# IrisRainbowNeko/HCP-Diffusion

Hardware: AMD Instinct MI355X
Metric: training images/sec (whole node), SD1.5 LoRA 512px bs=4/GPU (higher is better)
Workload: dtype bf16; 1 GPU; SD1.5 UNet LoRA rank=8 bf16, bs=4/GPU, 512x512 (64x64 latents), 77-token context, random-init weights, cached latents, grad-ckpt off; global_batch=4, parallelism=dp1, rccl_ranks=1, comm=none, hip_graph=True, gradient_checkpointing=False

## Files before the change

hcp_diffusion_amd/_lib.py:

```python
import ctypes
import os
from ctypes import c_int, c_long, c_float, c_void_p, c_size_t, c_char_p
from pathlib import Path

LIB_PATH = Path(__file__).resolve().parent / "libhcp_mi355x.so"

P, I, L, F = c_void_p, c_int, c_long, c_float

_PROTOTYPES = {
    "hcp_last_error": (c_char_p, []),
    "hcp_is_emulated": (I, []),
    "hcp_abi_version": (I, []),
    "hcp_selfcheck_atomics": (I, [P, P, I, I, I, P]),
    "hcp_gemm_bf16": (I, [P, I, P, I, P, I, I, I, I, P, I, P, I, I, P, P, I, I, P, I, P, P, P, F, I, P, c_size_t, P]),
    "hcp_gemm_lora_bf16": (I, [P, I, P, I, P, P, P, I, P, I, I, I, I, P, P, I, P, P, P, P, c_size_t, P]),
    "hcp_gemm_geglu_bwd_bf16": (I, [P, I, P, I, P, P, P, I, P, P, I, I, I, P, c_size_t, P]),
    "hcp_gemm_workspace_bytes": (c_size_t, [I, I]),
    "hcp_conv3x3_bf16": (I, [P, I, P, I, I, I, I, I, I, I, I, I, I, P, I, P, I, P, P, I, P, I, I, P, P, P, c_size_t, P]),
    "hcp_attention_fwd": (I, [P, P, P, P, P, I, I, I, I, I, L, I, L, I, L, I, L, I, F, P, L, I, P]),
    "hcp_attention_bwd": (I, [P, P, P, P, P, P, P, P, P, P, I, I, I, I, I, L, I, L, I, L, I, L, I, F, P, L, I, P, c_size_t, P]),
    "hcp_groupnorm_workspace_bytes": (c_size_t, [I, I, I, I]),
    "hcp_groupnorm_silu_fwd": (I, [P, P, P, P, P, P, I, I, I, I, F, I, P]),
    "hcp_groupnorm_silu_bwd": (I, [P, P, P, P, P, P, P, P, I, I, I, I, I, P]),
    "hcp_layernorm_fwd": (I, [P, P, P, P, P, P, I, I, F, P]),
    "hcp_layernorm_bwd": (I, [P, P, P, P, P, P, P, P, P, I, I, P]),
    "hcp_geglu_fwd": (I, [P, P, L, I, P]),
    "hcp_geglu_bwd": (I, [P, P, P, L, I, P]),
    "hcp_add_bf16": (I, [P, P, P, L, P]),
    "hcp_copy2d_bf16": (I, [P, I, P, I, L, I, P]),
    "hcp_concat2_bf16": (I, [P, I, P, I, P, L, I, P]),
    "hcp_silu_fwd": (I, [P, P, L, P]),
    "hcp_silu_bwd": (I, [P, P, P, L, P]),
    "hcp_nchw_to_nhwc_bf16": (I, [P, I, P, I, I, I, I, P]),
    "hcp_nhwc_to_nchw_f32": (I, [P, P, I, I, I, I, P]),
    "hcp_upsample2x_bwd": (I, [P, P, I, I, I, I, P]),
    "hcp_timestep_embedding": (I, [P, P, I, I, F, P]),
    "hcp_timestep_embedding_f32": (I, [P, P, I, I, F, P]),
    "hcp_wgrad_linear_bf16": (I, [P, I, P, I, P, I, I, I, I, P, c_size_t, P]),
    "hcp_wgrad_conv3x3_bf16": (I, [P, I, P, I, P, I, P, I, I, I, I, I, I, I, I, I, P, c_size_t, P]),
    "hcp_colsum_bf16": (I, [P, I, P, I, I, I, I, P]),
    "hcp_ema_update": (I, [P, P, L, P, F, F, F, P]),
    "hcp_cast_f32_bf16": (I, [P, P, L, F, I, P]),
    "hcp_cast_bf16_f32": (I, [P, P, L, P]),
    "hcp_pack_piece_bytes": (I, []),
    "hcp_pack_weights": (I, [P, I, I, P]),
    "hcp_groupnorm_affine_grad": (I, [P, P, P, P, P, P, P, I, I, I, I, I, P]),
    "hcp_layernorm_affine_grad": (I, [P, P, P, P, P, I, I, P]),
    "hcp_add_noise": (I, [P, P, P, P, P, I, L, P]),
    "hcp_cfg_ddim_step": (I, [P, P, P, L, I, F, F, F, P]),
    "hcp_snr_loss_weight": (I, [P, P, P, I, I, F, P]),
    "hcp_quick_gelu": (I, [P, P, P, L, P]),
    "hcp_embedding_bf16": (I, [P, P, P, P, P, L, I, I, P]),
    "hcp_embedding_pt_fwd_bf16": (I, [P, I, I, I, I, P, I, P, P, I, P, I, P, I, P, P, I, P]),
    "hcp_embedding_pt_bwd_f32": (I, [P, P, L, I, P, I, I, P]),
    "hcp_transpose_bf16": (I, [P, P, I, I, I, P]),
    "hcp_softmax_rows": (I, [P, L, P, L, I, I, F, P]),
    "hcp_vae_latent_sample": (I, [P, P, P, P, P, I, I, L, F, P]),
    "hcp_mse_masked_mean": (I, [P, P, P, I, P, P, P, I, I, I, F, P]),
    "hcp_lora_wgrad": (I, [P, I, I, P, I, P, I, I, I, I, F, I, P, c_size_t, P]),
    "hcp_lora_wgrad_pair": (I, [P, I, P, I, I, P, P, I, P, I, I, P, I, I, F, P, c_size_t, P]),
    "hcp_split_hi_lo_bf16": (I, [P, P, c_long, I, P]),
    "hcp_lora_wgrad_group_geometry": (I, [I, I, I, I, I, P, P, P, P]),
    "hcp_lora_wgrad_group_desc_bytes": (I, []),
    "hcp_lora_wgrad_grouped": (I, [P, I, I, I, c_long, P, c_size_t, P]),
    "hcp_lora_pack": (I, [P, I, P]),
    "hcp_lora_pack_desc_bytes": (I, []),
    "hcp_sumsq_f32": (I, [P, L, P, P]),
    "hcp_adamw_clip_fused": (I, [P, P, P, P, L, P, F, F, F, F, P, F, F, P, P]),
    "hcp_comm_unique_id": (I, [P]),
    "hcp_comm_init": (I, [I, I, P, ctypes.POINTER(P)]),
    "hcp_comm_destroy": (I, [P]),
    "hcp_comm_rank": (I, [P]),
    "hcp_comm_world": (I, [P]),
    "hcp_allreduce_flat": (I, [P, P, c_size_t, I, P]),
    "hcp_reduce_scatter_flat": (I, [P, P, P, c_size_t, I, P]),
    "hcp_allgather_flat": (I, [P, P, P, c_size_t, I, P]),
}

_TOOLS_PROTOTYPES = {
    "hcp_debug_set_gemm_config": (I, [I]),
    "hcp_debug_set_gemm_glds": (I, [I]),
    "hcp_debug_set_gemm_loaders": (I, [I]),
    "hcp_debug_set_gemm_epilogue": (I, [I]),
    "hcp_debug_set_conv_patch": (I, [I]),
    "hcp_debug_set_gn_target": (I, [I]),
    "hcp_debug_set_gemm_ablation": (I, [I]),
    "hcp_debug_set_attention_config": (I, [I]),
    "hcp_debug_set_wgrad_tile": (I, [I]),
    "hcp_debug_gemm_table_stats": (I, [P, P]),
}

EXPORTED_SYMBOLS = tuple(_PROTOTYPES)
TOOLS_SYMBOLS = tuple(_TOOLS_PROTOTYPES)
TOOLS_LIB_PATH = Path(__file__).resolve().parent / "libhcp_mi355x_tools.so"


ABI_VERSION = 4


class HcpError(RuntimeError):
    pass


def bind(cdll):
    cdll.hcp_abi_version.restype = I
    cdll.hcp_abi_version.argtypes = []
    got = cdll.hcp_abi_version()
    if got != ABI_VERSION:
        raise HcpError(f"{getattr(cdll, '_name', 'library')}: hcp_abi_version() = {got}, these bindings are for ABI {ABI_VERSION} "
                       "(rebuild with `python -m hcp_diffusion_amd.build`)")
    for name, (res, args) in _PROTOTYPES.items():
        fn = getattr(cdll, name)
        fn.restype = res
        fn.argtypes = args
    for name, (res, args) in _TOOLS_PROTOTYPES.items():
        fn = getattr(cdll, name, None)
        if fn is not None:
            fn.restype = res
            fn.argtypes = args
    return cdll


_tools = None


def load_tools():
    global _tools
    if _tools is None:
        import torch
        if not TOOLS_LIB_PATH.exists():
            raise HcpError(f"{TOOLS_LIB_PATH} not found: build it with `python -m hcp_diffusion_amd.build`")
        _tools = ctypes.CDLL(str(TOOLS_LIB_PATH))
        for name in _TOOLS_PROTOTYPES:
            getattr(_tools, name)
    return _tools


_lib = None


def load():
    global _lib
    if _lib is None:
        import torch
        if not LIB_PATH.exists():
            raise HcpError(
                f"{LIB_PATH} not found: build it with `python -m hcp_diffusion_amd.build` "
                "(hipcc, gfx950). hcp_diffusion_amd has no CPU/PyTorch fallback path.")
        _lib = bind(ctypes.CDLL(str(LIB_PATH)))
    return _lib


def check(rc, what=""):
    if rc != 0:
        msg = load().hcp_last_error() if _lib is not None else b""
        raise HcpError(f"{what} failed: {msg.decode() if msg else rc}")
```

hcp_diffusion_amd/csrc/gemm.hip:

```cpp
#include "hcp_common.h"
#include "gemm_params.h"

extern "C" int hcp_geglu_fwd(const void* h, void* y, long M, int F, hipStream_t stream);

namespace {

using namespace hcp_gemm;


HCP_DEVICE void epilogue_store(const GemmParams& p, int m, int n, hcp_f32x4 v) {
    if (p.geglu_hg) { epilogue_geglu_bwd(p, m, n, v); return; }
    v = v * p.alpha;
    if (p.bias) v += *(const hcp_f32x4*)(p.bias + n);
    if (p.rowbias) v += *(const hcp_f32x4*)(p.rowbias + (size_t)(m / p.rows_per_group) * p.rowbias_ld + n);
    if (p.residual) {
        hcp_bf16x4 r = *(const hcp_bf16x4*)(p.residual + (size_t)m * p.ldr + n);
#pragma unroll
        for (int q = 0; q < 4; ++q) v[q] += hcp_bf2f((unsigned short)r[q]);
        add_residual_lo(p, m, n, v);
    }
    if (p.out_f32) *(hcp_f32x4*)((float*)p.D + (size_t)m * p.ldd + n) = v;
    else store_hi_lo(p, m, n, v);
}

// ... 666 lines not shown
    }
    if (p.epi_tile) {
        if (!EARLY) load_epilogue_operands();
        if (LORA) HCP_SYNC();
        float* const tile = (float*)lds;
#pragma unroll
        for (int i = 0; i < TM; ++i) {
            const int ml = wm * WTM + i * 16 + fr, m = m0 + ml;
            const float* rbp = (p.rowbias && m < p.M) ? p.rowbias + (size_t)(m / p.rows_per_group) * p.rowbias_ld : nullptr;
#pragma unroll
            for (int j = 0; j < TN; ++j) {
                const int nl = wn * WTN + j * 16 + 4 * fg;
                hcp_f32x4 v = acc[i][j] * p.alpha + bias_v[j];
                if (rbp && n0 + nl < p.N) v += *(const hcp_f32x4*)(rbp + n0 + nl);
                *(hcp_f32x4*)(tile + ml * epi_tile_ld(BN) + nl) = v;
            }
        }
        HCP_SYNC();
        epi_tile_store<BM, BN, NTC>(p, tile, m0, n0, tid_all);
        return;
    }
    if (!EARLY) load_epilogue_operands();
#pragma unroll
    for (int i = 0; i < TM; ++i) {
        const int m = m0 + wm * WTM + i * 16 + fr;
        if (m >= p.M) continue;
        hcp_f32x4 rb_v[TN];
        if (p.rowbias) {
            const float* rbp = p.rowbias + (size_t)(m / p.rows_per_group) * p.rowbias_ld;
#pragma unroll
            for (int j = 0; j < TN; ++j) {
                const int n = n0 + wn * WTN + j * 16 + 4 * fg;
                hcp_f32x4 z = {0.f, 0.f, 0.f, 0.f};
                rb_v[j] = n < p.N ? *(const hcp_f32x4*)(rbp + n) : z;
            }
        }
#pragma unroll
        for (int j = 0; j < TN; ++j) {
            const int n = n0 + wn * WTN + j * 16 + 4 * fg;
            if (n >= p.N) continue;
            hcp_f32x4 v = acc[i][j] * p.alpha + bias_v[j];
            if (p.rowbias) v += rb_v[j];
            if (p.residual) {
#pragma unroll
                for (int q = 0; q < 4; ++q) v[q] += hcp_bf2f((unsigned short)res_v[i][j][q]);
                add_residual_lo(p, m, n, v);
            }
#if defined(HCP_TOOLS)
            if ((p.dbg & 64) && v[0] != 12345.678f) continue;
#endif
            if (p.out_f32) *(hcp_f32x4*)((float*)p.D + (size_t)m * p.ldd + n) = v;
            else store_hi_lo(p, m, n, v);
        }
    }
}

HCP_KERNEL(256) splitk_reduce_kernel(GemmParams p) {
    const unsigned nv = (unsigned)p.N / 4;
    const unsigned total = (unsigned)p.M * nv;
    const size_t slab = (size_t)p.M * p.N;
    const int ns = p.nsplit;
    const bool plain = !p.geglu_hg;
    for (unsigned i = blockIdx.x * 256u + threadIdx.x; i < total; i += gridDim.x * 256u) {
        const int m = (int)(i / nv), n = (int)(i - (unsigned)m * nv) * 4;
        const float* src = p.slabs + (size_t)i * 4;
        hcp_f32x4 v = *(const hcp_f32x4*)src;
        const void* const zp = g_zero_page;
        const hcp_f32x4 bias = *(const hcp_f32x4*)(plain && p.bias ? (const void*)(p.bias + n) : zp);
        const hcp_f32x4 rowb = *(const hcp_f32x4*)(plain && p.rowbias ? (const void*)(p.rowbias + (size_t)(m / p.rows_per_group) * p.rowbias_ld + n) : zp);
        const hcp_bf16x4 res = *(const hcp_bf16x4*)(plain && p.residual ? (const void*)(p.residual + (size_t)m * p.ldr + n) : zp);
        const hcp_bf16x4 res_lo = *(const hcp_bf16x4*)(plain && p.residual && p.residual_lo ? (const void*)(p.residual_lo + (size_t)m * p.ldr + n) : zp);
        int s = 1;
        for (; s + 4 <= ns; s += 4) {
            const hcp_f32x4 a = *(const hcp_f32x4*)(src + (size_t)s * slab), b = *(const hcp_f32x4*)(src + (size_t)(s + 1) * slab);
            const hcp_f32x4 c = *(const hcp_f32x4*)(src + (size_t)(s + 2) * slab), d = *(const hcp_f32x4*)(src + (size_t)(s + 3) * slab);
            v += a; v += b; v += c; v += d;
        }
        if (s + 2 <= ns) {
            const hcp_f32x4 a = *(const hcp_f32x4*)(src + (size_t)s * slab), b = *(const hcp_f32x4*)(src + (size_t)(s + 1) * slab);
            v += a; v += b;
            s += 2;
        }
        if (s < ns) v += *(const hcp_f32x4*)(src + (size_t)s * slab);
        if (!plain) { epilogue_geglu_bwd(p, m, n, v); continue; }
        v = v * p.alpha;
        if (p.bias) v += bias;
        if (p.rowbias) v += rowb;
        if (p.residual) {
#pragma unroll
            for (int q = 0; q < 4; ++q) v[q] += hcp_bf2f((unsigned short)res[q]);
            if (p.residual_lo) {
#pragma unroll
                for (int q = 0; q < 4; ++q) v[q] += hcp_bf2f((unsigned short)res_lo[q]);
            }
        }
        if (p.out_f32) *(hcp_f32x4*)((float*)p.D + (size_t)m * p.ldd + n) = v;
        else store_hi_lo(p, m, n, v);
    }
}

HCP_TUNABLE(int, g_force_cfg, -1);
inline int forced_id(int v) { return v >= 1024 ? (v - 1024) % 64 : v % 16; }
inline int forced_split(int v) { const int s = v >= 1024 ? (v - 1024) / 64 : v / 16; return s > 0 ? s : 1; }
HCP_TUNABLE(int, g_dbg_ablate, 0);
HCP_TUNABLE(int, g_use_glds, 1);
HCP_TUNABLE(int, g_use_v2, 1);

HCP_TUNABLE(int, g_conv_patch, 1);
HCP_TUNABLE(int, g_epi_tile, -1);
HCP_TUNABLE(int, g_force_loaders, -1);

bool want_epi_tile(const GemmParams& p, int mode) {
    if (p.nsplit != 1 || p.out_f32 || p.geglu_hg || p.geglu_out || p.N % 8 || p.ldd % 8 || (p.residual && p.ldr % 8)) return false;
    if ((((size_t)p.D) | ((size_t)p.D_lo) | ((size_t)p.residual) | ((size_t)p.residual_lo)) & 15) return false;
    if (g_epi_tile >= 0) return g_epi_tile == 1;
    return mode == 0 && p.residual != nullptr;
}

template <int BM, int BN, int WGM, int WGN, int MODE, bool FAST, bool LORA = false, int NSTAGE = 2, int NLD = 0>
int launch_cfg(GemmParams& p, hipStream_t stream) {
    p.tiles_m = hcp_cdiv(p.M, BM);
    const int tiles_n = hcp_cdiv(p.N, BN);
    p.dbg = g_dbg_ablate;
    if constexpr (NSTAGE == 2 && (MODE == 0 || FAST)) {
        if (g_use_v2 && g_use_glds && !(p.dbg & 7) && p.K % BK == 0 && (p.K2 == 0 || p.K2 == 32) &&
            (size_t)p.M * p.lda * 2 < (1ul << 31) && (size_t)p.N * p.ldb * 2 < (1ul << 31)) {
            constexpr size_t stage = (size_t)(BM + BN + (LORA ? 32 : 0)) * BK * sizeof(hcp_bf16);
            constexpr size_t eimg = (LORA && NLD > 0) ? (size_t)BN * 32 * sizeof(hcp_bf16) : 0;
            if (p.geglu_out) {
                if (MODE == 0 && WGN % 2 == 0 && p.nsplit == 1 && (p.N / 2) % (BN / 2) == 0) p.geglu_fused = 1;
                else p.geglu_out = nullptr;
            }
            constexpr size_t tile_bytes = (size_t)BM * epi_tile_ld(BN) * sizeof(float);
            p.epi_tile = want_epi_tile(p, MODE) && tile_bytes <= 160 * 1024 - eimg ? 1 : 0;
            size_t smem = 2 * stage;
            const size_t tail = (size_t)(2 * BM + BN) * 40 * sizeof(hcp_bf16);
            if (LORA && smem < tail) smem = tail;
            if (p.epi_tile && smem < tile_bytes) smem = tile_bytes;
            [[maybe_unused]] const dim3 grid(p.tiles_m * tiles_n, p.nsplit);
            if constexpr (NLD > 0) {
                const size_t tb = p.epi_tile ? tile_bytes : 0;
                if (p.loaders == 4 && 4 * stage + eimg <= 160 * 1024) {
                    HCP_LAUNCH((gemm_v2_kernel<BM, BN, WGM, WGN, MODE, LORA, NLD, (4 * stage + eimg <= 160 * 1024 ? 4 : 2)>), grid, dim3(64 * (WGM * WGN + NLD)), (4 * stage > tb ? 4 * stage : tb) + eimg, stream, p);
                } else if (p.loaders >= 3 && 3 * stage + eimg <= 160 * 1024) {
                    HCP_LAUNCH((gemm_v2_kernel<BM, BN, WGM, WGN, MODE, LORA, NLD, (3 * stage + eimg <= 160 * 1024 ? 3 : 2)>), grid, dim3(64 * (WGM * WGN + NLD)), (3 * stage > tb ? 3 * stage : tb) + eimg, stream, p);
                } else if (p.loaders) {
                    HCP_LAUNCH((gemm_v2_kernel<BM, BN, WGM, WGN, MODE, LORA, NLD>), grid, dim3(64 * (WGM * WGN + NLD)), smem + eimg, stream, p);
                } else {
                    HCP_LAUNCH((gemm_v2_kernel<BM, BN, WGM, WGN, MODE, LORA>), grid, dim3(64 * WGM * WGN), smem, stream, p);
                }
            } else {
                HCP_LAUNCH((gemm_v2_kernel<BM, BN, WGM, WGN, MODE, LORA>), dim3(p.tiles_m * tiles_n, p.nsplit), dim3(64 * WGM * WGN), smem, stream, p);
            }
            if (p.nsplit > 1) {
                long nv = (long)p.M * (p.N / 4);
                int g = (int)((nv + 255) / 256); if (g > 2048) g = 2048;
                HCP_LAUNCH(splitk_reduce_kernel, dim3(g), dim3(256), 0, stream, p);
            }
            HCP_LAUNCH_CHECK("gemm_v2_kernel");
        }
    }
    {
        p.epi_tile = 0;
        p.geglu_out = nullptr;
        size_t smem = (size_t)NSTAGE * (BM + BN + (LORA ? 32 : 0)) * BK * sizeof(hcp_bf16);
        const size_t tail = (size_t)(2 * BM + BN) * 40 * sizeof(hcp_bf16);
        if (LORA && smem < tail) smem = tail;
        HCP_LAUNCH((gemm_glds_kernel<BM, BN, WGM, WGN, MODE, FAST, LORA, NSTAGE>), dim3(p.tiles_m * tiles_n, p.nsplit),
                   dim3(64 * WGM * WGN), smem, stream, p);
    }
    if (p.nsplit > 1) {
        long nv = (long)p.M * (p.N / 4);
        int g = (int)((nv + 255) / 256); if (g > 2048) g = 2048;
        HCP_LAUNCH(splitk_reduce_kernel, dim3(g), dim3(256), 0, stream, p);
    }
    HCP_LAUNCH_CHECK("gemm_kernel");
}

struct TileCfg { int bm, bn; };
constexpr TileCfg kCfgs[] = {{128, 128}, {128, 64}, {64, 64}, {128, 160}, {64, 160}, {256, 128}, {256, 160}, {128, 320},
                             {128, 160}, {128, 160}, {256, 160},
                             {128, 320}, {256, 160}, {128, 160}, {64, 160}, {128, 128},
                             {32, 160}};
constexpr int kNumCfgs = sizeof(kCfgs) / sizeof(kCfgs[0]);

int try_pp(int id, int mode, bool fast_or_plain, bool lora, GemmParams& p, hipStream_t stream) {
    if (p.loaders < 8 || !fast_or_plain || !g_use_v2 || (g_dbg_ablate & 7)) return -2;
    if (p.K % BK != 0 || !(p.K2 == 0 || p.K2 == 32) || (size_t)p.M * p.lda * 2 >= (1ul << 31) || (size_t)p.N * p.ldb * 2 >= (1ul << 31)) return -2;
    const int bm = kCfgs[id].bm, bn = kCfgs[id].bn;
    p.tiles_m = hcp_cdiv(p.M, bm);
    p.dbg = g_dbg_ablate;
    p.epi_tile = want_epi_tile(p, mode) ? 1 : 0;
    hcp_bf16* const gout = p.geglu_out;
    if (gout) {
        if (mode == 0 && p.nsplit == 1 && (p.N / 2) % (bn / 2) == 0) p.geglu_fused = 1;
        else p.geglu_out = nullptr;
    }
    int r = -2;
    if (mode != 0 && !lora && (g_conv_patch == 2 || (g_conv_patch == 1 && (mode == 2 || p.nsplit > 1))))
        r = conv_patch_launch(p, bm, bn, mode, p.loaders - 8, stream);
    if (r == -2) r = gemm_pp_launch(p, bm, bn, mode, lora, p.loaders - 8, stream);
    if (r == -2) { p.geglu_out = gout; p.geglu_fused = 0; }
    if (r != 0 || p.nsplit <= 1) return r;
    long nv = (long)p.M * (p.N / 4);
    int g = (int)((nv + 255) / 256); if (g > 2048) g = 2048;
    HCP_LAUNCH(splitk_reduce_kernel, dim3(g), dim3(256), 0, stream, p);
    HCP_LAUNCH_CHECK("splitk_reduce_kernel");
}

template <int MODE, bool FAST>
int launch_by_id(int id, GemmParams& p, hipStream_t stream) {
    if (id >= 0 && id < kNumCfgs) { const int r = try_pp(id, MODE, MODE == 0 || FAST, false, p, stream); if (r != -2) return r; }
    switch (id) {
        case 0: return launch_cfg<128, 128, 2, 2, MODE, FAST>(p, stream);
        case 1: return launch_cfg<128, 64, 2, 2, MODE, FAST>(p, stream);
        case 2: return launch_cfg<64, 64, 2, 2, MODE, FAST>(p, stream);
        case 3: return launch_cfg<128, 160, 2, 2, MODE, FAST>(p, stream);
        case 4: return launch_cfg<64, 160, 2, 2, MODE, FAST>(p, stream);
        case 5: return launch_cfg<256, 128, 4, 2, MODE, FAST>(p, stream);
        case 6: return launch_cfg<256, 160, 4, 2, MODE, FAST>(p, stream);
        case 8: return launch_cfg<128, 160, 4, 2, MODE, FAST, false, 3>(p, stream);
        case 9: return launch_cfg<128, 160, 2, 2, MODE, FAST, false, 3>(p, stream);
        case 10: return launch_cfg<256, 160, 4, 2, MODE, FAST, false, 3>(p, stream);
        case 11: return launch_cfg<128, 320, 4, 4, MODE, FAST>(p, stream);
        case 12: return launch_cfg<256, 160, 8, 2, MODE, FAST>(p, stream);
        case 13: return launch_cfg<128, 160, 4, 2, MODE, FAST, false, 2, 4>(p, stream);
        case 14: return launch_cfg<64, 160, 4, 2, MODE, FAST, false, 2, 4>(p, stream);
        case 15: return launch_cfg<128, 128, 4, 2, MODE, FAST, false, 2, 4>(p, stream);
        case 16: return launch_cfg<64, 160, 4, 2, MODE, FAST, false, 2, 4>(p, stream);
        default: return launch_cfg<128, 320, 2, 4, MODE, FAST>(p, stream);
    }
}

int launch_lora_by_id(int id, GemmParams& p, hipStream_t stream) {
    if (id >= 0 && id < kNumCfgs) { const int r = try_pp(id, 0, true, true, p, stream); if (r != -2) return r; }
    switch (id) {
        case 0: return launch_cfg<128, 128, 2, 2, 0, false, true>(p, stream);
        case 1: return launch_cfg<128, 64, 2, 2, 0, false, true>(p, stream);
        case 2: return launch_cfg<64, 64, 2, 2, 0, false, true>(p, stream);
        case 3: return launch_cfg<128, 160, 2, 2, 0, false, true>(p, stream);
        case 5: return launch_cfg<256, 128, 4, 2, 0, false, true>(p, stream);
        case 6: return launch_cfg<256, 160, 4, 2, 0, false, true>(p, stream);
        case 8: return launch_cfg<128, 160, 4, 2, 0, false, true, 3>(p, stream);
        case 9: return launch_cfg<128, 160, 2, 2, 0, false, true, 3>(p, stream);
        case 12: return launch_cfg<256, 160, 8, 2, 0, false, true>(p, stream);
        case 13: return launch_cfg<128, 160, 4, 2, 0, false, true, 2, 4>(p, stream);
        case 14: return launch_cfg<64, 160, 4, 2, 0, false, true, 2, 4>(p, stream);
        case 15: return launch_cfg<128, 128, 4, 2, 0, false, true, 2, 4>(p, stream);
        case 16: return launch_cfg<64, 160, 4, 2, 0, false, true, 2, 4>(p, stream);
        default: return launch_cfg<64, 160, 2, 2, 0, false, true>(p, stream);
    }
}

int choose_cfg(const GemmParams& p, int* nsplit_out) {
    const int nk1 = hcp_cdiv(p.K, BK);
    int id;
    if (p.N <= 64) id = 2;
    else if (p.N % 160 == 0) id = ((long)p.M * p.N >= (long)4096 * 2560) ? 6 : 4;
    else id = ((long)p.M * p.N >= (long)4096 * 2048) ? 0 : 2;
    const long tiles = (long)hcp_cdiv(p.M, kCfgs[id].bm) * hcp_cdiv(p.N, kCfgs[id].bn);
    int s = 1;
    while (s < 16 && tiles * s < 1024 && nk1 / (s * 2) >= 4) s *= 2;
    *nsplit_out = s;
    return id;
}

struct TunedEntry { int mode, M, N, K, has_k2, stride, up, cfg, split, loaders; };
const TunedEntry kTuned[] = {
#include "gemm_tuned_loaders.inc"
#include "gemm_tuned.inc"
};

#if defined(HCP_TOOLS)
long g_table_hits = 0, g_table_misses = 0;
#endif

bool lookup_tuned(const GemmParams& p, int mode, int* cfg, int* split, int* loaders = nullptr) {
    bool hit = false;
    for (const TunedEntry& e : kTuned) {
        if (g_force_loaders == 0 && e.loaders) continue;
        if (e.mode == mode && e.M == p.M && e.N == p.N && e.K == p.K && e.has_k2 == (p.K2 > 0) &&
            (mode == 0 || mode == 3 || (e.stride == p.cv.stride && e.up == p.cv.up))) {
            *cfg = e.cfg; *split = e.split; if (loaders) *loaders = e.loaders; hit = true; break;
        }
    }
#if defined(HCP_TOOLS)
    (hit ? g_table_hits : g_table_misses) += 1;
#endif
    return hit;
}

inline int deepest_ring(int ld) { return ld == 3 ? 4 : ld; }

template <int MODE, bool FAST>
int dispatch_gemm(GemmParams& p, float* ws, size_t ws_bytes, hipStream_t stream) {
    int nsplit = 1;
    int id = 0, ld = 0;
    if (!lookup_tuned(p, MODE, &id, &nsplit, &ld)) id = choose_cfg(p, &nsplit);
    if (g_force_cfg >= 0) { id = forced_id(g_force_cfg); nsplit = forced_split(g_force_cfg); }
    p.loaders = g_force_loaders >= 0 ? g_force_loaders : deepest_ring(ld);
    if (nsplit > 1 && (size_t)nsplit * p.M * p.N * sizeof(float) > ws_bytes) nsplit = 1;
    if (p.geglu_out) nsplit = 1;
    const int nk1 = hcp_cdiv(p.K, BK);
    p.nsplit = nsplit;
    p.kt_per_split = hcp_cdiv(nk1, nsplit);
    p.nsplit = hcp_cdiv(nk1, p.kt_per_split);
    p.slabs = ws;
    return launch_by_id<MODE, FAST>(id, p, stream);
}

int check_common(const GemmParams& p) {
    HCP_REQUIRE(p.M > 0 && p.N > 0 && p.K > 0, "gemm: empty problem M=%d N=%d K=%d", p.M, p.N, p.K);
    HCP_REQUIRE(p.K % 8 == 0 && p.K2 % 8 == 0, "gemm: K (%d) and K2 (%d) must be multiples of 8", p.K, p.K2);
    HCP_REQUIRE(p.N % 4 == 0 && p.ldd % 4 == 0, "gemm: N (%d) and ldd (%d) must be multiples of 4", p.N, p.ldd);
    HCP_REQUIRE(p.ldb % 8 == 0, "gemm: ldb (%d) must be a multiple of 8", p.ldb);
    HCP_REQUIRE(p.K2 == 0 || (p.A2 && p.B2 && p.lda2 % 8 == 0 && p.ldb2 % 8 == 0), "gemm: bad K-extension operands");
    HCP_REQUIRE(!p.residual || p.ldr % 4 == 0, "gemm: ldr must be a multiple of 4");
    HCP_REQUIRE(!p.rowbias || p.rows_per_group > 0, "gemm: rows_per_group must be > 0");
    return 0;
}

int check_gact(GemmParams& p, void* gact, const char* who) {
    if (!gact) return 0;
    HCP_REQUIRE(!p.out_f32 && !p.residual && !p.rowbias && !p.D_lo && p.alpha == 1.0f && p.N % 16 == 0 && p.ldd == p.N,
                "%s: the GEGLU output needs a contiguous bf16 (h | g) [M, N] (N %% 16 == 0) with no residual / row bias / alpha", who);
    p.geglu_out = (hcp_bf16*)gact; p.geglu_fused = 0;
    return 0;
}
int finish_gact(const GemmParams& p, void* gact, hipStream_t stream) {
    if (!gact || p.geglu_fused) return 0;
    return hcp_geglu_fwd(p.D, gact, p.M, p.N / 2, stream);
}

int launch_lora_dispatched(GemmParams& p, void* workspace, size_t workspace_bytes, hipStream_t stream) {
    int id = 4, nsplit = 1, ld = 0;
    GemmParams q = p; q.K2 = 32;
    if (!lookup_tuned(q, 3, &id, &nsplit, &ld)) {
        if (p.K >= 4096 && p.M <= 4096) id = -1;
        else if ((long)p.M * p.N >= (long)4096 * 2560 && p.N % 160 == 0) id = 6;
        else if (p.N % 160 == 0 && (long)p.M * p.N >= (long)4096 * 640) id = 4;
        else id = 2;
    }
    if (g_force_cfg >= 0) id = forced_id(g_force_cfg);
    p.loaders = g_force_loaders >= 0 ? g_force_loaders : deepest_ring(ld);
    if (id == 7 || id == 10 || id == 11) id = 6;
    if (id < 0) {
        HCP_REQUIRE(p.Tout, "hcp_gemm_lora_bf16: this shape runs as two launches and needs the T buffer");
        const int ldt = p.ldt == 64 ? 64 : 32;
        if (ldt == 64 && hcp_memset_async(p.Tout, 0, (size_t)p.M * 64 * sizeof(hcp_bf16), stream)) return hcp_set_error("hcp_gemm_lora_bf16: memset failed");
        GemmParams t = {};
        t.A = p.A; t.lda = p.lda; t.B = p.L; t.ldb = p.K; t.M = p.M; t.N = 32; t.K = p.K; t.D = p.Tout; t.ldd = ldt; t.alpha = 1.0f;
        if (int e2 = dispatch_gemm<0, false>(t, (float*)workspace, workspace ? workspace_bytes : 0, stream)) return e2;
        p.A2 = (const hcp_bf16*)p.Tout; p.lda2 = ldt; p.B2 = p.E; p.ldb2 = 32; p.K2 = 32;
        p.L = nullptr; p.E = nullptr; p.Tout = nullptr; p.ldt = 0;
        return dispatch_gemm<0, false>(p, (float*)workspace, workspace ? workspace_bytes : 0, stream);
    }
    p.nsplit = 1; p.kt_per_split = hcp_cdiv(p.K, BK); p.slabs = nullptr;
    return launch_lora_by_id(id, p, stream);
}

}

#if defined(HCP_TOOLS)
HCP_API int hcp_debug_gemm_table_stats(long* hits, long* misses) {
    if (hits) *hits = g_table_hits;
    if (misses) *misses = g_table_misses;
    g_table_hits = 0; g_table_misses = 0;
    return 0;
}
HCP_API int hcp_debug_set_gemm_config(int cfg) { g_force_cfg = cfg; return 0; }
HCP_API int hcp_debug_set_gemm_glds(int on) { g_use_glds = 1; g_use_v2 = on == 1; return 0; }
HCP_API int hcp_debug_set_gemm_ablation(int flags) { g_dbg_ablate = flags; return 0; }
HCP_API int hcp_debug_set_gemm_loaders(int mode) { g_force_loaders = mode; return 0; }
HCP_API int hcp_debug_set_gemm_epilogue(int mode) { g_epi_tile = mode; return 0; }
HCP_API int hcp_debug_set_conv_patch(int on) { g_conv_patch = on; return 0; }
#endif

HCP_API size_t hcp_gemm_workspace_bytes(int M, int N) { return (size_t)16 * M * N * sizeof(float); }

HCP_API int hcp_gemm_bf16(const void* A, int lda, const void* B, int ldb, void* D, int ldd, int M, int N, int K,
                          const void* A2, int lda2, const void* B2, int ldb2, int K2, const float* bias,
                          const float* rowbias, int rowbias_ld, int rows_per_group, const void* residual, int ldr,
                          const void* residual_lo, void* D_lo, void* gact, float alpha, int out_f32, void* workspace,
                          size_t workspace_bytes, hipStream_t stream) {
    GemmParams p = {};
    p.A = (const hcp_bf16*)A; p.lda = lda; p.B = (const hcp_bf16*)B; p.ldb = ldb;
    p.A2 = (const hcp_bf16*)A2; p.lda2 = lda2; p.B2 = (const hcp_bf16*)B2; p.ldb2 = ldb2; p.K2 = K2;
    p.M = M; p.N = N; p.K = K; p.D = D; p.ldd = ldd; p.out_f32 = out_f32;
    p.bias = bias; p.rowbias = rowbias; p.rowbias_ld = rowbias_ld; p.rows_per_group = rows_per_group;
    p.residual = (const hcp_bf16*)residual; p.ldr = ldr; p.alpha = alpha;
    p.residual_lo = (const hcp_bf16*)residual_lo; p.D_lo = (hcp_bf16*)D_lo;
    HCP_REQUIRE(A && B && D, "hcp_gemm_bf16: null operand");
    HCP_REQUIRE((!residual_lo || residual) && (!D_lo || !out_f32), "hcp_gemm_bf16: residual_lo needs residual; D_lo needs a bf16 output");
    HCP_REQUIRE(lda % 8 == 0, "hcp_gemm_bf16: lda (%d) must be a multiple of 8", lda);
    if (int e = check_common(p)) return e;
    if (int e = check_gact(p, gact, "hcp_gemm_bf16")) return e;
    if (int e = dispatch_gemm<0, false>(p, (float*)workspace, workspace ? workspace_bytes : 0, stream)) return e;
    return finish_gact(p, gact, stream);
}

HCP_API int hcp_conv3x3_bf16(const void* X1, int C1, const void* X2, int C2, int Bn, int Hs, int Ws, int Ho, int Wo,
                             int mode, int stride, int upsample, int pad, const void* Wp, int Cout, void* D, int ldd,
                             const float* bias, const float* rowbias, int rowbias_ld, const void* residual, int ldr,
                             int out_f32, const void* A2, const void* B2, void* workspace, size_t workspace_bytes,
                             hipStream_t stream) {
    GemmParams p = {};
    HCP_REQUIRE(X1 && Wp && D, "hcp_conv3x3_bf16: null operand");
    HCP_REQUIRE((A2 == nullptr) == (B2 == nullptr), "hcp_conv3x3_bf16: the rank-32 K-extension needs both A2 and B2");
    if (A2) { p.A2 = (const hcp_bf16*)A2; p.lda2 = 32; p.B2 = (const hcp_bf16*)B2; p.ldb2 = 32; p.K2 = 32; }
    HCP_REQUIRE(C1 % 8 == 0 && C2 % 8 == 0 && (C2 == 0 || X2), "hcp_conv3x3_bf16: channels must be multiples of 8");
    HCP_REQUIRE(stride == 1 || stride == 2, "hcp_conv3x3_bf16: stride must be 1 or 2");
    HCP_REQUIRE(mode == 0 || (mode == 1 && upsample == 0 && C2 == 0), "hcp_conv3x3_bf16: bad mode/options");
    HCP_REQUIRE(pad == 1 || (pad == 0 && mode == 0 && !upsample), "hcp_conv3x3_bf16: pad must be 1 (or 0 for a forward conv without upsampling)");
    HCP_REQUIRE(Ho <= 1024 && Wo <= 1024 && Bn < 2048, "hcp_conv3x3_bf16: dims too large for packed pixel ids (10 bits per output axis)");
    HCP_REQUIRE((long)Bn * Hs * Ws * (C1 > C2 ? C1 : C2) < (1L << 31), "hcp_conv3x3_bf16: source tensor too large for 32-bit offsets");
    p.cv.X1 = (const hcp_bf16*)X1; p.cv.C1 = C1; p.cv.X2 = (const hcp_bf16*)X2; p.cv.C2 = C2;
    p.cv.Hs = Hs; p.cv.Ws = Ws; p.cv.Ho = Ho; p.cv.Wo = Wo; p.cv.stride = stride; p.cv.up = upsample ? 1 : 0; p.cv.pad = pad;
    p.M = Bn * Ho * Wo; p.N = Cout; p.K = 9 * (C1 + C2);
    p.B = (const hcp_bf16*)Wp; p.ldb = p.K;
    p.D = D; p.ldd = ldd; p.out_f32 = out_f32; p.bias = bias;
    p.rowbias = rowbias; p.rowbias_ld = rowbias_ld; p.rows_per_group = Ho * Wo;
    p.residual = (const hcp_bf16*)residual; p.ldr = ldr; p.alpha = 1.0f;
    if (int e = check_common(p)) return e;
    float* ws = (float*)workspace; size_t wb = workspace ? workspace_bytes : 0;
    const bool fast = (C1 % 64 == 0) && (C2 % 64 == 0) && !upsample && !(mode == 1 && stride == 2);
    if (mode == 0) return fast ? dispatch_gemm<1, true>(p, ws, wb, stream) : dispatch_gemm<1, false>(p, ws, wb, stream);
    return fast ? dispatch_gemm<2, true>(p, ws, wb, stream) : dispatch_gemm<2, false>(p, ws, wb, stream);
}

HCP_API int hcp_gemm_geglu_bwd_bf16(const void* A, int lda, const void* B, int ldb, const void* L, const void* E, void* Tout, int ldt,
                                    const void* HG, void* DHG, int M, int F, int K, void* workspace, size_t workspace_bytes,
                                    hipStream_t stream) {
    GemmParams p = {};
    p.A = (const hcp_bf16*)A; p.lda = lda; p.B = (const hcp_bf16*)B; p.ldb = ldb;
    p.M = M; p.N = F; p.K = K; p.D = DHG; p.ldd = 2 * F; p.out_f32 = 0; p.alpha = 1.0f;
    p.geglu_hg = (const hcp_bf16*)HG; p.geglu_ld = 2 * F;
    HCP_REQUIRE(A && B && HG && DHG, "hcp_gemm_geglu_bwd_bf16: null operand");
    HCP_REQUIRE((L == nullptr) == (E == nullptr), "hcp_gemm_geglu_bwd_bf16: L and E come together");
    HCP_REQUIRE(lda % 8 == 0 && F % 8 == 0, "hcp_gemm_geglu_bwd_bf16: lda (%d) and F (%d) must be multiples of 8", lda, F);
    if (int e = check_common(p)) return e;
    if (!L) return dispatch_gemm<0, false>(p, (float*)workspace, workspace ? workspace_bytes : 0, stream);
    HCP_REQUIRE(ldt == 32 || ldt == 64, "hcp_gemm_geglu_bwd_bf16: ldt (%d) is 32 (bf16 U) or 64 (split U: hi | lo)", ldt);
    p.L = (const hcp_bf16*)L; p.E = (const hcp_bf16*)E; p.Tout = (hcp_bf16*)Tout; p.ldt = ldt;
    return launch_lora_dispatched(p, workspace, workspace_bytes, stream);
}

HCP_API int hcp_gemm_lora_bf16(const void* A, int lda, const void* B, int ldb, const void* L, const void* E, void* Tout, int ldt, void* D,
                               int ldd, int M, int N, int K, const float* bias, const void* residual, int ldr, const void* residual_lo,
                               void* D_lo, void* gact, void* workspace, size_t workspace_bytes, hipStream_t stream) {
    GemmParams p = {};
    p.A = (const hcp_bf16*)A; p.lda = lda; p.B = (const hcp_bf16*)B; p.ldb = ldb;
    p.M = M; p.N = N; p.K = K; p.D = D; p.ldd = ldd; p.out_f32 = 0;
    p.bias = bias; p.residual = (const hcp_bf16*)residual; p.ldr = ldr; p.alpha = 1.0f;
    p.L = (const hcp_bf16*)L; p.E = (const hcp_bf16*)E; p.Tout = (hcp_bf16*)Tout; p.ldt = ldt;
    p.residual_lo = (const hcp_bf16*)residual_lo; p.D_lo = (hcp_bf16*)D_lo;
    HCP_REQUIRE(A && B && D && L && E, "hcp_gemm_lora_bf16: null operand");
    HCP_REQUIRE(!residual_lo || residual, "hcp_gemm_lora_bf16: residual_lo needs residual");
    HCP_REQUIRE(ldt == 32 || ldt == 64, "hcp_gemm_lora_bf16: ldt (%d) is 32 (bf16 T) or 64 (split T: hi | lo)", ldt);
    HCP_REQUIRE(lda % 8 == 0, "hcp_gemm_lora_bf16: lda (%d) must be a multiple of 8", lda);
    if (int e = check_common(p)) return e;
    if (int e = check_gact(p, gact, "hcp_gemm_lora_bf16")) return e;
    if (int e = launch_lora_dispatched(p, workspace, workspace_bytes, stream)) return e;
    return finish_gact(p, gact, stream);
}
```

hcp_diffusion_amd/csrc/gemm_params.h:

```cpp
#pragma once
#include "hcp_common.h"

namespace hcp_gemm {

struct ConvDesc {
    const hcp_bf16* X1; int C1;
    const hcp_bf16* X2; int C2;
    int Hs, Ws;
    int Ho, Wo;
    int stride;
    int up;
    int pad;
};

struct GemmParams {
    const hcp_bf16* A; int lda;
    const hcp_bf16* A2; int lda2; int K2;
    const hcp_bf16* B; int ldb;
    const hcp_bf16* B2; int ldb2;
    int M, N, K;
    void* D; int ldd; int out_f32;
    const float* bias;
    const float* rowbias; int rowbias_ld; int rows_per_group;
    const hcp_bf16* residual; int ldr;
    const hcp_bf16* residual_lo; hcp_bf16* D_lo;
    float alpha;
    int tiles_m;
    int nsplit; int kt_per_split;
    float* slabs;
    const hcp_bf16* L; const hcp_bf16* E; hcp_bf16* Tout; int ldt;
    const hcp_bf16* geglu_hg; int geglu_ld;
    hcp_bf16* geglu_out; int geglu_fused;
    int epi_tile;
    int loaders;
    int dbg;
    ConvDesc cv;
};

constexpr int BK = 64;

HCP_DEVICE void lora_t_split(const hcp_f32x4& t, hcp_bf16x4& hi, hcp_bf16x4& lo) {
#pragma unroll
    for (int q = 0; q < 4; ++q) {
        const unsigned short h = hcp_f2bf(t[q]);
        hi[q] = (short)h;
        lo[q] = (short)hcp_f2bf(t[q] - hcp_bf2f(h));
    }
}

HCP_DEVICE void store_hi_lo(const GemmParams& p, int m, int n, const hcp_f32x4& v) {
    hcp_bf16x4 o;
#pragma unroll
    for (int q = 0; q < 4; ++q) o[q] = (short)hcp_f2bf(v[q]);
    *(hcp_bf16x4*)((hcp_bf16*)p.D + (size_t)m * p.ldd + n) = o;
    if (p.D_lo) {
        hcp_bf16x4 l;
#pragma unroll
        for (int q = 0; q < 4; ++q) l[q] = (short)hcp_f2bf(v[q] - hcp_bf2f((unsigned short)o[q]));
        *(hcp_bf16x4*)(p.D_lo + (size_t)m * p.ldd + n) = l;
    }
}
HCP_DEVICE void add_residual_lo(const GemmParams& p, int m, int n, hcp_f32x4& v) {
    if (!p.residual_lo) return;
    const hcp_bf16x4 r = *(const hcp_bf16x4*)(p.residual_lo + (size_t)m * p.ldr + n);
#pragma unroll
    for (int q = 0; q < 4; ++q) v[q] += hcp_bf2f((unsigned short)r[q]);
}

constexpr int epi_tile_ld(int BN) { return BN + 4; }
template <int BM, int BN, int NTHREADS>
HCP_DEVICE void epi_tile_store(const GemmParams& p, const float* tile, int m0, int n0, int tid) {
    constexpr int LD = epi_tile_ld(BN), PIECES = BN / 8;
    for (int idx = tid; idx < BM * PIECES; idx += NTHREADS) {
        const int row = idx / PIECES, c8 = (idx - row * PIECES) * 8;
        const int m = m0 + row, n = n0 + c8;
        if (m >= p.M || n >= p.N) continue;
        const hcp_f32x4 a = *(const hcp_f32x4*)(tile + row * LD + c8), b = *(const hcp_f32x4*)(tile + row * LD + c8 + 4);
        float v[8] = {a[0], a[1], a[2], a[3], b[0], b[1], b[2], b[3]};
        if (p.residual) {
            const hcp_bf16x8 r = *(const hcp_bf16x8*)(p.residual + (size_t)m * p.ldr + n);
#pragma unroll
            for (int q = 0; q < 8; ++q) v[q] += hcp_bf2f((unsigned short)r[q]);
            if (p.residual_lo) {
                const hcp_bf16x8 rl = *(const hcp_bf16x8*)(p.residual_lo + (size_t)m * p.ldr + n);
#pragma unroll
                for (int q = 0; q < 8; ++q) v[q] += hcp_bf2f((unsigned short)rl[q]);
            }
        }
        hcp_bf16x8 o;
#pragma unroll
        for (int q = 0; q < 8; ++q) o[q] = (short)hcp_f2bf(v[q]);
        *(hcp_bf16x8*)((hcp_bf16*)p.D + (size_t)m * p.ldd + n) = o;
        if (p.D_lo) {
            hcp_bf16x8 l;
#pragma unroll
            for (int q = 0; q < 8; ++q) l[q] = (short)hcp_f2bf(v[q] - hcp_bf2f((unsigned short)o[q]));
            *(hcp_bf16x8*)(p.D_lo + (size_t)m * p.ldd + n) = l;
        }
    }
}

HCP_DEVICE int geglu_col(const GemmParams& p, int BN, int nl) {
    if (!p.geglu_out) return nl;
    const int half = BN >> 1, j = nl / BN, c = nl - j * BN;
    return c < half ? j * half + c : (p.N >> 1) + j * half + (c - half);
}
template <int TI, int TJ, typename SYNC>
HCP_DEVICE void geglu_fwd_pair(hcp_f32x4 (&v)[TI][TJ], bool is_g, int slot, int lane, hcp_f32x4* xg, SYNC&& sync,
                               hcp_bf16* out, int F, const int (&rows)[TI], int M, const int (&cols)[TJ]) {
    hcp_f32x4* mine = xg + (size_t)slot * TI * TJ * 64 + lane;
    if (is_g) {
#pragma unroll
        for (int i = 0; i < TI; ++i)
#pragma unroll
            for (int j = 0; j < TJ; ++j) {
                hcp_f32x4 ge;
#pragma unroll
                for (int q = 0; q < 4; ++q) ge[q] = hcp_gelu_erf(v[i][j][q]);
                mine[(i * TJ + j) * 64] = ge;
            }
    }
    sync();
    if (!is_g) {
#pragma unroll
        for (int i = 0; i < TI; ++i) {
            if (rows[i] >= M) continue;
#pragma unroll
            for (int j = 0; j < TJ; ++j) {
                const hcp_f32x4 ge = mine[(i * TJ + j) * 64];
                hcp_bf16x4 o;
#pragma unroll
                for (int q = 0; q < 4; ++q) o[q] = (short)hcp_f2bf(v[i][j][q] * ge[q]);
                *(hcp_bf16x4*)(out + (size_t)rows[i] * F + cols[j]) = o;
            }
        }
    }
}

HCP_DEVICE void epilogue_geglu_bwd(const GemmParams& p, int m, int n, hcp_f32x4 v) {
    const hcp_bf16* hp = p.geglu_hg + (size_t)m * p.geglu_ld + n;
    const hcp_bf16x4 h = *(const hcp_bf16x4*)hp, g = *(const hcp_bf16x4*)(hp + p.N);
    hcp_bf16x4 dh, dg;
#pragma unroll
    for (int q = 0; q < 4; ++q) {
        const float hf = hcp_bf2f((unsigned short)h[q]), gf = hcp_bf2f((unsigned short)g[q]);
        const float d = hcp_bf2f(hcp_f2bf(v[q] * p.alpha));
        dh[q] = (short)hcp_f2bf(d * hcp_gelu_erf(gf));
        dg[q] = (short)hcp_f2bf(d * hf * hcp_gelu_erf_grad(gf));
    }
    hcp_bf16* dp = (hcp_bf16*)p.D + (size_t)m * p.ldd + n;
    *(hcp_bf16x4*)dp = dh;
    *(hcp_bf16x4*)(dp + p.N) = dg;
}

constexpr int geglu_tile_ld(int BN) { return BN + 8; }
HCP_DEVICE void geglu_tile_put(hcp_bf16* tile, int ld, int row, int col, hcp_f32x4 v, float alpha) {
    hcp_bf16x4 o;
#pragma unroll
    for (int q = 0; q < 4; ++q) o[q] = (short)hcp_f2bf(v[q] * alpha);
    *(hcp_bf16x4*)(tile + row * ld + col) = o;
}
template <int BM, int BN, int NTHREADS>
HCP_DEVICE void geglu_tile_apply(const GemmParams& p, const hcp_bf16* tile, int m0, int n0, int tid) {
    constexpr int LD = geglu_tile_ld(BN), PIECES = BN / 8;
    for (int idx = tid; idx < BM * PIECES; idx += NTHREADS) {
        const int row = idx / PIECES, c8 = (idx - row * PIECES) * 8;
        const int m = m0 + row, n = n0 + c8;
        if (m >= p.M || n >= p.N) continue;
        const hcp_bf16x8 d = *(const hcp_bf16x8*)(tile + row * LD + c8);
        const hcp_bf16* hp = p.geglu_hg + (size_t)m * p.geglu_ld + n;
        const hcp_bf16x8 h = *(const hcp_bf16x8*)hp, g = *(const hcp_bf16x8*)(hp + p.N);
        hcp_bf16x8 dh, dg;
#pragma unroll
        for (int q = 0; q < 8; ++q) {
            const float df = hcp_bf2f((unsigned short)d[q]), hf = hcp_bf2f((unsigned short)h[q]), gf = hcp_bf2f((unsigned short)g[q]);
            dh[q] = (short)hcp_f2bf(df * hcp_gelu_erf(gf));
            dg[q] = (short)hcp_f2bf(df * hf * hcp_gelu_erf_grad(gf));
        }
        hcp_bf16* dp = (hcp_bf16*)p.D + (size_t)m * p.ldd + n;
        *(hcp_bf16x8*)dp = dh;
        *(hcp_bf16x8*)(dp + p.N) = dg;
    }
// ... 7 lines not shown
```

hcp_diffusion_amd/csrc/norm.hip:

```cpp
#include "hcp_common.h"

namespace {

struct GNGeom { int TX, R, threads, nchunk, rows_per_chunk; };

HCP_TUNABLE(int, g_gn_target_wgs, 512);
HCP_TUNABLE(int, g_gn_slab, 1);
GNGeom gn_geom(int B, int HW, int C) {
    GNGeom g;
    g.TX = C / 8;
    g.R = 256 / g.TX; if (g.R < 1) g.R = 1;
    g.threads = g.TX * g.R;
    long rows = ((long)HW * B + g_gn_target_wgs - 1) / g_gn_target_wgs;
    rows = (rows + g.R - 1) / g.R * g.R;
    if (rows < 4 * g.R) rows = 4 * g.R;
    g.rows_per_chunk = (int)rows;
    g.nchunk = (HW + g.rows_per_chunk - 1) / g.rows_per_chunk;
    return g;
}

inline size_t gn_merge_smem(int threads, int G) { return ((size_t)2 * G + (size_t)(threads / G) * G * 3) * sizeof(float); }

HCP_KERNEL(1024) gn_fwd_partial(const hcp_bf16* x, float* ws, int HW, int C, int G, int TX, int R, int rows_per_chunk) {
    HCP_DYN_SMEM(smem);
// ... 115 lines not shown
    auto row = [&](const hcp_bf16x8& v, int r) {
        hcp_bf16x8 o;
#pragma unroll
        for (int i = 0; i < 8; ++i) {
            float z = hcp_bf2f((unsigned short)v[i]) * a8[i] + b8[i];
            if (silu) z = hcp_silu(z);
            o[i] = (short)hcp_f2bf(z);
        }
        *(hcp_bf16x8*)(y + base + (size_t)r * C) = o;
    };
    int r = r0 + ry;
    for (; r + 3 * R < r1; r += 4 * R) {
        hcp_bf16x8 v[4];
#pragma unroll
        for (int u = 0; u < 4; ++u) v[u] = *(const hcp_bf16x8*)(x + base + (size_t)(r + u * R) * C);
#pragma unroll
        for (int u = 0; u < 4; ++u) row(v[u], r + u * R);
    }
    for (; r < r1; r += R) row(*(const hcp_bf16x8*)(x + base + (size_t)r * C), r);
}

HCP_KERNEL(1024) gn_bwd_partial(const hcp_bf16* x, const hcp_bf16* dy, const float* gamma, const float* beta,
                                const float* stats, float* ws, int HW, int C, int G, int TX, int R, int rows_per_chunk, int silu) {
    HCP_DYN_SMEM(smem);
    float* s_1 = (float*)smem;
    float* s_2 = s_1 + R * C;
    const int tid = threadIdx.x;
    const int cx = tid % TX, ry = tid / TX;
    const int chunk = blockIdx.x, b = blockIdx.y;
    const int Cg = C / G;
    const int r0 = chunk * rows_per_chunk;
    int r1 = r0 + rows_per_chunk; if (r1 > HW) r1 = HW;
    float mean8[8], rstd8[8], g8[8], be8[8], s1[8], s2[8];
#pragma unroll
    for (int i = 0; i < 8; ++i) {
        int c = cx * 8 + i; int g = c / Cg;
        mean8[i] = stats[((size_t)b * G + g) * 2]; rstd8[i] = stats[((size_t)b * G + g) * 2 + 1];
        g8[i] = gamma[c]; be8[i] = beta[c]; s1[i] = 0.f; s2[i] = 0.f;
    }
    const size_t base = (size_t)b * HW * C + cx * 8;
    auto row = [&](const hcp_bf16x8& v, const hcp_bf16x8& d) {
#pragma unroll
        for (int i = 0; i < 8; ++i) {
            float xh = (hcp_bf2f((unsigned short)v[i]) - mean8[i]) * rstd8[i];
            float dz = hcp_bf2f((unsigned short)d[i]);
            if (silu) { float z = xh * g8[i] + be8[i]; float sg = hcp_sigmoid(z); dz *= sg * (1.f + z * (1.f - sg)); }
            float dxh = dz * g8[i];
            s1[i] += dxh; s2[i] += dxh * xh;
        }
    };
    int r = r0 + ry;
    for (; r + 1 * R < r1; r += 2 * R) {
        hcp_bf16x8 v[2], d[2];
#pragma unroll
        for (int u = 0; u < 2; ++u) {
            v[u] = *(const hcp_bf16x8*)(x + base + (size_t)(r + u * R) * C);
            d[u] = *(const hcp_bf16x8*)(dy + base + (size_t)(r + u * R) * C);
        }
#pragma unroll
        for (int u = 0; u < 2; ++u) row(v[u], d[u]);
    }
    for (; r < r1; r += R) row(*(const hcp_bf16x8*)(x + base + (size_t)r * C), *(const hcp_bf16x8*)(dy + base + (size_t)r * C));
#pragma unroll
    for (int i = 0; i < 8; ++i) { s_1[ry * C + cx * 8 + i] = s1[i]; s_2[ry * C + cx * 8 + i] = s2[i]; }
    HCP_SYNC();
    float a = 0.f, bq = 0.f;
    {
        const int g = tid >> 2, sub = tid & 3;
        if (g < G)
            for (int j = sub; j < R * Cg; j += 4) {
                int rr = j / Cg, c = j - rr * Cg;
                a += s_1[rr * C + g * Cg + c]; bq += s_2[rr * C + g * Cg + c];
            }
        a += hcp_shfl_xor(a, 1); a += hcp_shfl_xor(a, 2);
        bq += hcp_shfl_xor(bq, 1); bq += hcp_shfl_xor(bq, 2);
    }
    if ((tid & 3) == 0 && (tid >> 2) < G) {
        float* o = ws + (((size_t)b * gridDim.x + chunk) * G + (tid >> 2)) * 2;
        o[0] = a; o[1] = bq;
    }
}

HCP_KERNEL(1024) gn_bwd_apply(const hcp_bf16* x, const hcp_bf16* dy, const float* gamma, const float* beta,
                              const float* stats, const float* ws, const hcp_bf16* addend, hcp_bf16* dx, int HW, int C, int G,
                              int TX, int R, int rows_per_chunk, int silu) {
    HCP_DYN_SMEM(smem);
    float* s_c12 = (float*)smem;
    const int tid = threadIdx.x;
    const int chunk = blockIdx.x, b = blockIdx.y;
    const int Cg = C / G;
    gn_merge(ws + (size_t)b * gridDim.x * G * 2, s_c12, G, gridDim.x, rows_per_chunk, HW, Cg, 0.f, 1, tid, blockDim.x);
    const int cx = tid % TX, ry = tid / TX;
    const int r0 = chunk * rows_per_chunk;
    int r1 = r0 + rows_per_chunk; if (r1 > HW) r1 = HW;
    float mean8[8], rstd8[8], g8[8], be8[8], c1[8], c2[8];
#pragma unroll
    for (int i = 0; i < 8; ++i) {
        int c = cx * 8 + i; int g = c / Cg;
        mean8[i] = stats[((size_t)b * G + g) * 2]; rstd8[i] = stats[((size_t)b * G + g) * 2 + 1];
        g8[i] = gamma[c]; be8[i] = beta[c]; c1[i] = s_c12[g * 2]; c2[i] = s_c12[g * 2 + 1];
    }
    const size_t base = (size_t)b * HW * C + cx * 8;
    auto row = [&](const hcp_bf16x8& v, const hcp_bf16x8& d, const hcp_bf16x8& ad, int r) {
        hcp_bf16x8 o;
#pragma unroll
        for (int i = 0; i < 8; ++i) {
            float xh = (hcp_bf2f((unsigned short)v[i]) - mean8[i]) * rstd8[i];
            float dz = hcp_bf2f((unsigned short)d[i]);
            if (silu) { float z = xh * g8[i] + be8[i]; float sg = hcp_sigmoid(z); dz *= sg * (1.f + z * (1.f - sg)); }
            float dxh = dz * g8[i];
            o[i] = (short)hcp_f2bf(rstd8[i] * (dxh - c1[i] - xh * c2[i]) + (addend ? hcp_bf2f((unsigned short)ad[i]) : 0.f));
        }
        *(hcp_bf16x8*)(dx + base + (size_t)r * C) = o;
    };
    const hcp_bf16* const adp = addend ? addend : dy;
    int r = r0 + ry;
    for (; r + 1 * R < r1; r += 2 * R) {
        hcp_bf16x8 v[2], d[2], ad[2];
#pragma unroll
        for (int u = 0; u < 2; ++u) {
            v[u] = *(const hcp_bf16x8*)(x + base + (size_t)(r + u * R) * C);
            d[u] = *(const hcp_bf16x8*)(dy + base + (size_t)(r + u * R) * C);
            ad[u] = *(const hcp_bf16x8*)(adp + base + (size_t)(r + u * R) * C);
        }
#pragma unroll
        for (int u = 0; u < 2; ++u) row(v[u], d[u], ad[u], r + u * R);
    }
    for (; r < r1; r += R)
        row(*(const hcp_bf16x8*)(x + base + (size_t)r * C), *(const hcp_bf16x8*)(dy + base + (size_t)r * C),
            *(const hcp_bf16x8*)(adp + base + (size_t)r * C), r);
}

HCP_DEVICE float gn_block_sum(float v, float* s_red, int tid, int nthreads) {
#pragma unroll
    for (int off = 1; off < 64; off <<= 1) v += hcp_shfl_xor(v, off);
    HCP_SYNC();
    if ((tid & 63) == 0) s_red[tid >> 6] = v;
    HCP_SYNC();
    float t = 0.f;
    for (int w = 0; w < nthreads / 64; ++w) t += s_red[w];
    return t;
}
template <int CE>
HCP_DEVICE size_t gn_slab_off(int c, int cpr, unsigned cpr_magic, int C, int* ch_in_group) {
    const int row = cpr_magic ? (int)(((unsigned long long)(unsigned)c * cpr_magic) >> 32) : c;
    *ch_in_group = (c - row * cpr) * CE;
    return (size_t)row * C + (size_t)*ch_in_group;
}
template <int CE> struct GNChunk;
typedef float hcp_f32x2 __attribute__((ext_vector_type(2)));
template <> struct GNChunk<4> { typedef hcp_bf16x4 T; typedef hcp_f32x4 F; };
template <> struct GNChunk<2> { typedef hcp_bf16x2 T; typedef hcp_f32x2 F; };

template <int NCH, int CE>
HCP_KERNEL(1024) gn_slab_fwd(const hcp_bf16* x, const float* gamma, const float* beta, float* stats, hcp_bf16* y, int HW, int C,
                             int G, int cpr, unsigned cpr_magic, int silu, float eps) {
    typedef typename GNChunk<CE>::T V;
    typedef typename GNChunk<CE>::F FV;
    HCP_DYN_SMEM(smem);
    float* s_red = (float*)smem;
    const int tid = threadIdx.x, NT = blockDim.x;
    const int g = blockIdx.x, b = blockIdx.y;
    const int Cg = C / G, total = HW * cpr;
    float* s_ga = s_red + 32;
    float* s_be = s_ga + Cg;
    for (int j = tid; j < Cg; j += NT) { s_ga[j] = gamma[g * Cg + j]; s_be[j] = beta[g * Cg + j]; }
    const size_t base = (size_t)b * HW * C + (size_t)g * Cg;
    V v[NCH];
#pragma unroll
    for (int i = 0; i < NCH; ++i) {
        const int c = tid + i * NT;
        int cg;
        v[i] = *(const V*)(x + base + gn_slab_off<CE>(c < total ? c : 0, cpr, cpr_magic, C, &cg));
        if (NCH > 8 && i % 8 == 7) hcp_sched_fence();
    }
    float s = 0.f;
#pragma unroll
    for (int i = 0; i < NCH; ++i) {
        const bool live = tid + i * NT < total;
#pragma unroll
        for (int e = 0; e < CE; ++e) { v[i][e] = live ? v[i][e] : (short)0; s += hcp_bf2f((unsigned short)v[i][e]); }
    }
    const float n = (float)HW * Cg;
    const float mean = gn_block_sum(s, s_red, tid, NT) / n;
    float q = 0.f;
#pragma unroll
    for (int i = 0; i < NCH; ++i)
        if (tid + i * NT < total) {
#pragma unroll
            for (int e = 0; e < CE; ++e) { const float d = hcp_bf2f((unsigned short)v[i][e]) - mean; q += d * d; }
        }
    const float rstd = 1.0f / sqrtf(gn_block_sum(q, s_red, tid, NT) / n + eps);
    if (tid == 0) { stats[((size_t)b * G + g) * 2] = mean; stats[((size_t)b * G + g) * 2 + 1] = rstd; }
#pragma unroll
    for (int i = 0; i < NCH; ++i) {
        const int c = tid + i * NT;
        if (c >= total) continue;
        int cg;
        const size_t off = gn_slab_off<CE>(c, cpr, cpr_magic, C, &cg);
        const FV ga = *(const FV*)(s_ga + cg), be = *(const FV*)(s_be + cg);
        V o;
#pragma unroll
        for (int e = 0; e < CE; ++e) {
            const float a = rstd * ga[e];
            float z = hcp_bf2f((unsigned short)v[i][e]) * a + (be[e] - mean * a);
            if (silu) z = hcp_silu(z);
            o[e] = (short)hcp_f2bf(z);
        }
        *(V*)(y + base + off) = o;
    }
}

template <int NCH, int CE>
HCP_KERNEL(1024) gn_slab_bwd(const hcp_bf16* x, const hcp_bf16* dy, const float* gamma, const float* beta, const float* stats,
                             const hcp_bf16* addend, hcp_bf16* dx, int HW, int C, int G, int cpr, unsigned cpr_magic, int silu) {
    typedef typename GNChunk<CE>::T V;
    typedef typename GNChunk<CE>::F FV;
    HCP_DYN_SMEM(smem);
    float* s_red = (float*)smem;
    const int tid = threadIdx.x, NT = blockDim.x;
    const int g = blockIdx.x, b = blockIdx.y;
    const int Cg = C / G, total = HW * cpr;
    float* s_ga = s_red + 32;
    float* s_be = s_ga + Cg;
    for (int j = tid; j < Cg; j += NT) { s_ga[j] = gamma[g * Cg + j]; s_be[j] = beta[g * Cg + j]; }
    const size_t base = (size_t)b * HW * C + (size_t)g * Cg;
    const float mean = stats[((size_t)b * G + g) * 2], rstd = stats[((size_t)b * G + g) * 2 + 1];
    constexpr bool EARLY_AD = NCH * CE <= 32;
    constexpr int GB = NCH < 8 ? NCH : 8;
    V v[NCH], d[NCH], ad[EARLY_AD ? NCH : 1];
#pragma unroll
    for (int i = 0; i < NCH; ++i) {
        const int c = tid + i * NT;
        int cg;
        const size_t off = gn_slab_off<CE>(c < total ? c : 0, cpr, cpr_magic, C, &cg);
        v[i] = *(const V*)(x + base + off); d[i] = *(const V*)(dy + base + off);
        if (NCH > 8 && i % 8 == 7) hcp_sched_fence();
    }
    if constexpr (EARLY_AD) {
        if (addend) {
#pragma unroll
            for (int i = 0; i < NCH; ++i) {
                const int c = tid + i * NT;
                int cg;
                ad[i] = *(const V*)(addend + base + gn_slab_off<CE>(c < total ? c : 0, cpr, cpr_magic, C, &cg));
            }
        }
    }
    HCP_SYNC();
    auto terms = [&](int i, int cg, float (&h)[CE], float (&dh)[CE]) {
        const FV ga = *(const FV*)(s_ga + cg), be = *(const FV*)(s_be + cg);
#pragma unroll
        for (int e = 0; e < CE; ++e) {
            h[e] = (hcp_bf2f((unsigned short)v[i][e]) - mean) * rstd;
            float dz = hcp_bf2f((unsigned short)d[i][e]);
            if (silu) { const float z = h[e] * ga[e] + be[e]; const float sg = hcp_sigmoid(z); dz *= sg * (1.f + z * (1.f - sg)); }
            dh[e] = dz * ga[e];
        }
    };
    constexpr bool KEEP = NCH * CE <= 32;
    float dhk[KEEP ? NCH : 1][CE];
    float s1 = 0.f, s2 = 0.f;
#pragma unroll
    for (int i = 0; i < NCH; ++i) {
        int c = tid + i * NT;
        if (NCH > 16) hcp_force_ready(c);
        if (c < total) {
            int cg;
            gn_slab_off<CE>(c, cpr, cpr_magic, C, &cg);
            float h[CE], dh[CE];
            terms(i, cg, h, dh);
#pragma unroll
            for (int e = 0; e < CE; ++e) {
                s1 += dh[e]; s2 += dh[e] * h[e];
                if constexpr (KEEP) dhk[i][e] = dh[e];
            }
        }
        if (NCH > 16 && i % 8 == 7) hcp_sched_fence();
    }
    const float n = (float)HW * Cg;
    const float c1 = gn_block_sum(s1, s_red, tid, NT) / n;
    const float c2 = gn_block_sum(s2, s_red, tid, NT) / n;
#pragma unroll
    for (int i0 = 0; i0 < NCH; i0 += GB) {
        V adg[GB];
        if (addend) {
#pragma unroll
            for (int j = 0; j < GB; ++j) {
                if constexpr (EARLY_AD) adg[j] = ad[i0 + j];
                else {
                    int c = tid + (i0 + j) * NT;
                    if (NCH > 16) hcp_force_ready(c);
                    int cg;
                    adg[j] = *(const V*)(addend + base + gn_slab_off<CE>(c < total ? c : 0, cpr, cpr_magic, C, &cg));
                }
            }
        }
#pragma unroll
        for (int j = 0; j < GB; ++j) {
            const int i = i0 + j;
            int c = tid + i * NT;
            if (NCH > 16) hcp_force_ready(c);
            if (c >= total) continue;
            int cg;
            const size_t off = gn_slab_off<CE>(c, cpr, cpr_magic, C, &cg);
            float h[CE], dh[CE];
            if constexpr (KEEP) {
#pragma unroll
                for (int e = 0; e < CE; ++e) { h[e] = (hcp_bf2f((unsigned short)v[i][e]) - mean) * rstd; dh[e] = dhk[i][e]; }
            } else terms(i, cg, h, dh);
            V o;
#pragma unroll
            for (int e = 0; e < CE; ++e)
                o[e] = (short)hcp_f2bf(rstd * (dh[e] - c1 - h[e] * c2) + (addend ? hcp_bf2f((unsigned short)adg[j][e]) : 0.f));
            *(V*)(dx + base + off) = o;
        }
        if (NCH > 16) hcp_sched_fence();
    }
}

struct GNSlab { int nt, nch, ce, cpr; unsigned magic; };
GNSlab gn_slab_geom(int HW, int C, int G) {
    GNSlab r = {0, 0, 0, 0, 0};
    const int Cg = C / G;
    if (Cg % 2) return r;
    const int ce = Cg % 4 == 0 ? 4 : 2;
    if ((long)HW * Cg > 65536 || Cg > 2048) return r;
    if (ce == 2 && HW > 1024) return r;
    const long total = (long)HW * (Cg / ce);
    r.ce = ce; r.cpr = Cg / ce;
    r.magic = r.cpr == 1 ? 0u : (unsigned)(((1ull << 32) + r.cpr - 1) / r.cpr);
    r.nt = total <= 256 * 8 ? 256 : 1024;
    int nch = 1;
    while ((long)nch * r.nt < total) nch *= 2;
    r.nch = nch;
    return r;
}

#define HCP_GN_SLAB_SWITCH(KERNEL, ...)                                                                              \
    do {                                                                                                             \
        const int key_ = sl.nch * 8 + sl.ce;                                                                         \
        switch (key_) {                                                                                              \
            case 1 * 8 + 4: HCP_LAUNCH((KERNEL<1, 4>), grid, blk, sm, stream, __VA_ARGS__); break;                   \
            case 2 * 8 + 4: HCP_LAUNCH((KERNEL<2, 4>), grid, blk, sm, stream, __VA_ARGS__); break;                   \
            case 4 * 8 + 4: HCP_LAUNCH((KERNEL<4, 4>), grid, blk, sm, stream, __VA_ARGS__); break;                   \
            case 8 * 8 + 4: HCP_LAUNCH((KERNEL<8, 4>), grid, blk, sm, stream, __VA_ARGS__); break;                   \
            case 16 * 8 + 4: HCP_LAUNCH((KERNEL<16, 4>), grid, blk, sm, stream, __VA_ARGS__); break;                 \
            case 1 * 8 + 2: HCP_LAUNCH((KERNEL<1, 2>), grid, blk, sm, stream, __VA_ARGS__); break;                   \
            case 2 * 8 + 2: HCP_LAUNCH((KERNEL<2, 2>), grid, blk, sm, stream, __VA_ARGS__); break;                   \
            case 4 * 8 + 2: HCP_LAUNCH((KERNEL<4, 2>), grid, blk, sm, stream, __VA_ARGS__); break;                   \
            case 8 * 8 + 2: HCP_LAUNCH((KERNEL<8, 2>), grid, blk, sm, stream, __VA_ARGS__); break;                   \
            case 16 * 8 + 2: HCP_LAUNCH((KERNEL<16, 2>), grid, blk, sm, stream, __VA_ARGS__); break;                 \
            default: HCP_LAUNCH((KERNEL<32, 2>), grid, blk, sm, stream, __VA_ARGS__); break;                         \
        }                                                                                                            \
    } while (0)

template <int NV, bool HL>
HCP_KERNEL(256) ln_fwd_kernel(const hcp_bf16* x, const hcp_bf16* x_lo, const float* gamma, const float* beta, hcp_bf16* y, float* stats,
                              int M, int C, float eps) {
    const int lane = threadIdx.x & 63;
    const int row = blockIdx.x * 4 + (threadIdx.x >> 6);
    const bool live = row < M;
    const hcp_bf16* xr = x + (size_t)(live ? row : 0) * C;
    const int nch = C / 8;
    hcp_bf16x8 v[NV], vl[HL ? NV : 1];
#pragma unroll
    for (int u = 0; u < NV; ++u) {
        const int j = lane + 64 * u;
        v[u] = j < nch ? *(const hcp_bf16x8*)(xr + j * 8) : hcp_zero8();
        if (HL) vl[u] = j < nch ? *(const hcp_bf16x8*)(x_lo + (size_t)(live ? row : 0) * C + j * 8) : hcp_zero8();
    }
#define HCP_LN_X(u_, i_) (HL ? hcp_bf2f((unsigned short)v[u_][i_]) + hcp_bf2f((unsigned short)vl[HL ? u_ : 0][i_]) : hcp_bf2f((unsigned short)v[u_][i_]))
    float s = 0.f;
#pragma unroll
    for (int u = 0; u < NV; ++u)
#pragma unroll
        for (int i = 0; i < 8; ++i) s += HCP_LN_X(u, i);
    const float mean = hcp_wave_sum(s) / C;
    float q = 0.f;
#pragma unroll
    for (int u = 0; u < NV; ++u)
        if (lane + 64 * u < nch) {
#pragma unroll
            for (int i = 0; i < 8; ++i) { float d = HCP_LN_X(u, i) - mean; q += d * d; }
        }
    const float rstd = 1.0f / sqrtf(hcp_wave_sum(q) / C + eps);
    if (!live) return;
    if (lane == 0) { stats[(size_t)row * 2] = mean; stats[(size_t)row * 2 + 1] = rstd; }
    hcp_bf16* yr = y + (size_t)row * C;
#pragma unroll
    for (int u = 0; u < NV; ++u) {
        const int j = lane + 64 * u;
        if (j >= nch) continue;
        hcp_f32x4 g0 = *(const hcp_f32x4*)(gamma + j * 8), g1 = *(const hcp_f32x4*)(gamma + j * 8 + 4);
        hcp_f32x4 b0 = *(const hcp_f32x4*)(beta + j * 8), b1 = *(const hcp_f32x4*)(beta + j * 8 + 4);
        hcp_bf16x8 o;
#pragma unroll
        for (int i = 0; i < 8; ++i) {
            float g = i < 4 ? g0[i] : g1[i - 4], bb = i < 4 ? b0[i] : b1[i - 4];
            o[i] = (short)hcp_f2bf((HCP_LN_X(u, i) - mean) * rstd * g + bb);
        }
        *(hcp_bf16x8*)(yr + j * 8) = o;
    }
}

template <int NV, bool HL>
HCP_KERNEL(256) ln_bwd_kernel(const hcp_bf16* x, const hcp_bf16* x_lo, const hcp_bf16* dy, const float* gamma, const float* stats,
                              const hcp_bf16* addend, const hcp_bf16* addend_lo, hcp_bf16* dx, hcp_bf16* dx_lo, int M, int C) {
    const int lane = threadIdx.x & 63;
    const int row = blockIdx.x * 4 + (threadIdx.x >> 6);
    const bool live = row < M;
    const size_t off = (size_t)(live ? row : 0) * C;
    const float mean = stats[(size_t)(live ? row : 0) * 2], rstd = stats[(size_t)(live ? row : 0) * 2 + 1];
    const int nch = C / 8;
    hcp_bf16x8 v[NV], d[NV], ad[NV], vl[HL ? NV : 1], adl[HL ? NV : 1];
#pragma unroll
    for (int u = 0; u < NV; ++u) {
        const int j = lane + 64 * u;
        const bool ok = j < nch;
        v[u] = ok ? *(const hcp_bf16x8*)(x + off + j * 8) : hcp_zero8();
        d[u] = ok ? *(const hcp_bf16x8*)(dy + off + j * 8) : hcp_zero8();
        ad[u] = (ok && addend) ? *(const hcp_bf16x8*)(addend + off + j * 8) : hcp_zero8();
        if (HL) {
            vl[u] = (ok && x_lo) ? *(const hcp_bf16x8*)(x_lo + off + j * 8) : hcp_zero8();
            adl[u] = (ok && addend_lo) ? *(const hcp_bf16x8*)(addend_lo + off + j * 8) : hcp_zero8();
        }
    }
    float s1 = 0.f, s2 = 0.f;
#pragma unroll
    for (int u = 0; u < NV; ++u) {
        const int j = lane + 64 * u;
        if (j >= nch) continue;
#pragma unroll
        for (int i = 0; i < 8; ++i) {
            float xh = (HCP_LN_X(u, i) - mean) * rstd;
            float dxh = hcp_bf2f((unsigned short)d[u][i]) * gamma[j * 8 + i];
            s1 += dxh; s2 += dxh * xh;
        }
    }
    const float c1 = hcp_wave_sum(s1) / C, c2 = hcp_wave_sum(s2) / C;
    if (!live) return;
#pragma unroll
    for (int u = 0; u < NV; ++u) {
        const int j = lane + 64 * u;
        if (j >= nch) continue;
        hcp_bf16x8 o, ol;
#pragma unroll
        for (int i = 0; i < 8; ++i) {
            float xh = (HCP_LN_X(u, i) - mean) * rstd;
            float dxh = hcp_bf2f((unsigned short)d[u][i]) * gamma[j * 8 + i];
            float g = rstd * (dxh - c1 - xh * c2) + hcp_bf2f((unsigned short)ad[u][i]);
            if (HL) g += hcp_bf2f((unsigned short)adl[u][i]);
            o[i] = (short)hcp_f2bf(g);
            if (HL) ol[i] = (short)hcp_f2bf(g - hcp_bf2f((unsigned short)o[i]));
        }
        *(hcp_bf16x8*)(dx + off + j * 8) = o;
        if (HL && dx_lo) *(hcp_bf16x8*)(dx_lo + off + j * 8) = ol;
    }
}
#undef HCP_LN_X

template <bool GROUP>
HCP_KERNEL(256) norm_affine_grad_kernel(const hcp_bf16* x, const hcp_bf16* dy, const float* gamma, const float* beta,
                                        const float* stats, float* dgamma, float* dbeta, int rows, int C, int G, int silu,
                                        int rows_per_block) {
    HCP_DYN_SMEM(smem);
    float (*red)[129] = (float (*)[129])smem;
    const int tid = threadIdx.x;
    const int ch = tid & 7, rl = tid >> 3;
    const int c0 = blockIdx.x * 64 + ch * 8;
    const int b = blockIdx.z;
    const int mb = blockIdx.y * rows_per_block;
    int me = mb + rows_per_block; if (me > rows) me = rows;
    float sg[8], sb[8], mean8[8], rstd8[8], g8[8], be8[8];
#pragma unroll
    for (int i = 0; i < 8; ++i) { sg[i] = 0.f; sb[i] = 0.f; mean8[i] = 0.f; rstd8[i] = 1.f; g8[i] = 1.f; be8[i] = 0.f; }
    if (c0 < C) {
        if (GROUP) {
            const int Cg = C / G;
#pragma unroll
            for (int i = 0; i < 8; ++i) {
                const int g = (c0 + i) / Cg;
                mean8[i] = stats[((size_t)b * G + g) * 2]; rstd8[i] = stats[((size_t)b * G + g) * 2 + 1];
                g8[i] = gamma[c0 + i]; be8[i] = beta[c0 + i];
            }
        }
        const size_t base = (size_t)b * rows * C + c0;
        for (int r = mb + rl; r < me; r += 32) {
            hcp_bf16x8 v = *(const hcp_bf16x8*)(x + base + (size_t)r * C);
            hcp_bf16x8 d = *(const hcp_bf16x8*)(dy + base + (size_t)r * C);
            float mean = 0.f, rstd = 1.f;
            if (!GROUP) { mean = stats[(size_t)r * 2]; rstd = stats[(size_t)r * 2 + 1]; }
#pragma unroll
            for (int i = 0; i < 8; ++i) {
                const float xh = (hcp_bf2f((unsigned short)v[i]) - (GROUP ? mean8[i] : mean)) * (GROUP ? rstd8[i] : rstd);
                float dz = hcp_bf2f((unsigned short)d[i]);
                if (GROUP && silu) { float z = xh * g8[i] + be8[i]; float s = hcp_sigmoid(z); dz *= s * (1.f + z * (1.f - s)); }
                sg[i] += dz * xh; sb[i] += dz;
            }
        }
    }
#pragma unroll
    for (int i = 0; i < 8; ++i) { red[rl][ch * 8 + i] = sg[i]; red[rl][64 + ch * 8 + i] = sb[i]; }
    HCP_SYNC();
    if (tid < 128) {
        float t = 0.f;
        for (int r = 0; r < 32; ++r) t += red[r][tid];
        const int c = blockIdx.x * 64 + (tid & 63);
        if (c < C && mb < me) hcp_atomic_add((tid < 64 ? dgamma : dbeta) + c, t);
    }
}

int affine_grad_blocks(int rows, int col_tiles, int groups, int* rows_per_block) {
    int splits = hcp_cdiv(1024, col_tiles * groups);
    const int max_splits = hcp_cdiv(rows, 128);
    if (splits > max_splits) splits = max_splits;
    if (splits < 1) splits = 1;
    *rows_per_block = hcp_cdiv(hcp_cdiv(rows, splits), 32) * 32;
    return hcp_cdiv(rows, *rows_per_block);
}

int gn_check(int B, int HW, int C, int G) {
    HCP_REQUIRE(B > 0 && HW > 0 && C > 0 && G > 0, "groupnorm: empty problem");
    HCP_REQUIRE(C % 8 == 0 && C % G == 0 && C <= 8192 && G <= 32, "groupnorm: C=%d G=%d unsupported", C, G);
    HCP_REQUIRE(gn_geom(1, HW, C).threads >= 4 * G, "groupnorm: C=%d too small for G=%d", C, G);
    return 0;
}

}

#if defined(HCP_TOOLS)
HCP_API int hcp_debug_set_gn_target(int workgroups) {
    if (workgroups == -1 || workgroups == -2) { g_gn_slab = workgroups == -1 ? 0 : 1; return 0; }
    HCP_REQUIRE(workgroups >= 1 && workgroups <= 65536, "hcp_debug_set_gn_target: bad arguments");
    g_gn_target_wgs = workgroups;
    return 0;
}
#endif

HCP_API size_t hcp_groupnorm_workspace_bytes(int B, int HW, int C, int G) {
    if (B <= 0 || HW <= 0 || C <= 0 || C % 8) return 0;
    GNGeom g = gn_geom(B, HW, C);
    return ((size_t)B * g.nchunk * G * 2 + (size_t)B * G * 2) * sizeof(float);
}

HCP_API int hcp_groupnorm_silu_fwd(const void* x, const float* gamma, const float* beta, void* y, float* stats,
                                   void* workspace, int B, int HW, int C, int G, float eps, int silu, hipStream_t stream) {
    if (int e = gn_check(B, HW, C, G)) return e;
    HCP_REQUIRE(x && gamma && beta && y && stats && workspace, "hcp_groupnorm_silu_fwd: null pointer");
    const GNSlab sl = gn_slab_geom(HW, C, G);
    if (sl.nch && g_gn_slab) {
        const hcp_bf16* xp = (const hcp_bf16*)x; hcp_bf16* yp = (hcp_bf16*)y;
        const dim3 grid(G, B), blk(sl.nt);
        const size_t sm = (32 + 2 * (size_t)(C / G)) * sizeof(float);
        HCP_GN_SLAB_SWITCH(gn_slab_fwd, xp, gamma, beta, stats, yp, HW, C, G, sl.cpr, sl.magic, silu, eps);
        HCP_LAUNCH_CHECK("groupnorm_fwd (slab)");
    }
    GNGeom g = gn_geom(B, HW, C);
    size_t sm1 = (size_t)2 * g.R * C * sizeof(float);
    HCP_LAUNCH(gn_fwd_partial, dim3(g.nchunk, B), dim3(g.threads), sm1, stream, (const hcp_bf16*)x, (float*)workspace, HW, C,
               G, g.TX, g.R, g.rows_per_chunk);
    HCP_LAUNCH(gn_fwd_apply, dim3(g.nchunk, B), dim3(g.threads), gn_merge_smem(g.threads, G), stream, (const hcp_bf16*)x, gamma,
               beta, (const float*)workspace, stats, (hcp_bf16*)y, HW, C, G, g.TX, g.R, g.rows_per_chunk, silu, eps);
    HCP_LAUNCH_CHECK("groupnorm_fwd");
}

HCP_API int hcp_groupnorm_silu_bwd(const void* x, const void* dy, const float* gamma, const float* beta,
                                   const float* stats, const void* addend, void* dx, void* workspace, int B, int HW, int C,
                                   int G, int silu, hipStream_t stream) {
    if (int e = gn_check(B, HW, C, G)) return e;
    HCP_REQUIRE(x && dy && gamma && beta && stats && dx && workspace, "hcp_groupnorm_silu_bwd: null pointer");
    const GNSlab sl = gn_slab_geom(HW, C, G);
    if (sl.nch && g_gn_slab) {
        const hcp_bf16 *xp = (const hcp_bf16*)x, *dp = (const hcp_bf16*)dy, *ap = (const hcp_bf16*)addend; hcp_bf16* op = (hcp_bf16*)dx;
        const dim3 grid(G, B), blk(sl.nt);
        const size_t sm = (32 + 2 * (size_t)(C / G)) * sizeof(float);
        HCP_GN_SLAB_SWITCH(gn_slab_bwd, xp, dp, gamma, beta, stats, ap, op, HW, C, G, sl.cpr, sl.magic, silu);
        HCP_LAUNCH_CHECK("groupnorm_bwd (slab)");
    }
    GNGeom g = gn_geom(B, HW, C);
    size_t sm1 = (size_t)2 * g.R * C * sizeof(float);
    HCP_LAUNCH(gn_bwd_partial, dim3(g.nchunk, B), dim3(g.threads), sm1, stream, (const hcp_bf16*)x, (const hcp_bf16*)dy,
               gamma, beta, stats, (float*)workspace, HW, C, G, g.TX, g.R, g.rows_per_chunk, silu);
    HCP_LAUNCH(gn_bwd_apply, dim3(g.nchunk, B), dim3(g.threads), gn_merge_smem(g.threads, G), stream, (const hcp_bf16*)x,
               (const hcp_bf16*)dy, gamma, beta, stats, (const float*)workspace, (const hcp_bf16*)addend, (hcp_bf16*)dx, HW, C, G,
               g.TX, g.R, g.rows_per_chunk, silu);
    HCP_LAUNCH_CHECK("groupnorm_bwd");
}

HCP_API int hcp_layernorm_fwd(const void* x, const void* x_lo, const float* gamma, const float* beta, void* y, float* stats, int M, int C,
                              float eps, hipStream_t stream) {
    HCP_REQUIRE(M > 0 && C > 0 && C % 8 == 0 && C <= 4096, "hcp_layernorm_fwd: bad shape M=%d C=%d (C: multiple of 8 up to 4096)", M, C);
    HCP_REQUIRE(x && gamma && beta && y && stats, "hcp_layernorm_fwd: null pointer");
#define HCP_LN_FWD(NV_, HL_) HCP_LAUNCH((ln_fwd_kernel<NV_, HL_>), dim3(hcp_cdiv(M, 4)), dim3(256), 0, stream, (const hcp_bf16*)x, \
                                        (const hcp_bf16*)x_lo, gamma, beta, (hcp_bf16*)y, stats, M, C, eps)
    if (x_lo) { if (C <= 512) HCP_LN_FWD(1, true); else if (C <= 1024) HCP_LN_FWD(2, true); else if (C <= 2048) HCP_LN_FWD(4, true); else HCP_LN_FWD(8, true); }
    else { if (C <= 512) HCP_LN_FWD(1, false); else if (C <= 1024) HCP_LN_FWD(2, false); else if (C <= 2048) HCP_LN_FWD(4, false); else HCP_LN_FWD(8, false); }
#undef HCP_LN_FWD
    HCP_LAUNCH_CHECK("layernorm_fwd");
}

HCP_API int hcp_layernorm_bwd(const void* x, const void* x_lo, const void* dy, const float* gamma, const float* stats, const void* addend,
                              const void* addend_lo, void* dx, void* dx_lo, int M, int C, hipStream_t stream) {
    HCP_REQUIRE(M > 0 && C > 0 && C % 8 == 0 && C <= 4096, "hcp_layernorm_bwd: bad shape M=%d C=%d (C: multiple of 8 up to 4096)", M, C);
    HCP_REQUIRE(x && dy && gamma && stats && dx, "hcp_layernorm_bwd: null pointer");
    HCP_REQUIRE(!addend_lo || addend, "hcp_layernorm_bwd: addend_lo needs addend");
#define HCP_LN_BWD(NV_, HL_) HCP_LAUNCH((ln_bwd_kernel<NV_, HL_>), dim3(hcp_cdiv(M, 4)), dim3(256), 0, stream, (const hcp_bf16*)x, \
                                        (const hcp_bf16*)x_lo, (const hcp_bf16*)dy, gamma, stats, (const hcp_bf16*)addend,       \
                                        (const hcp_bf16*)addend_lo, (hcp_bf16*)dx, (hcp_bf16*)dx_lo, M, C)
    if (x_lo || addend_lo || dx_lo) { if (C <= 512) HCP_LN_BWD(1, true); else if (C <= 1024) HCP_LN_BWD(2, true); else if (C <= 2048) HCP_LN_BWD(4, true); else HCP_LN_BWD(8, true); }
    else { if (C <= 512) HCP_LN_BWD(1, false); else if (C <= 1024) HCP_LN_BWD(2, false); else if (C <= 2048) HCP_LN_BWD(4, false); else HCP_LN_BWD(8, false); }
#undef HCP_LN_BWD
    HCP_LAUNCH_CHECK("layernorm_bwd");
}

HCP_API int hcp_groupnorm_affine_grad(const void* x, const void* dy, const float* gamma, const float* beta, const float* stats,
                                      float* dgamma, float* dbeta, int B, int HW, int C, int G, int silu, hipStream_t stream) {
    HCP_REQUIRE(x && dy && gamma && beta && stats && dgamma && dbeta, "hcp_groupnorm_affine_grad: null argument");
    HCP_REQUIRE(B > 0 && HW > 0 && C > 0 && G > 0 && C % 8 == 0 && C % G == 0, "hcp_groupnorm_affine_grad: C=%d G=%d unsupported", C, G);
    const int ct = hcp_cdiv(C, 64);
    int rpb; const int splits = affine_grad_blocks(HW, ct, B, &rpb);
    HCP_LAUNCH((norm_affine_grad_kernel<true>), dim3(ct, splits, B), dim3(256), 32 * 129 * sizeof(float), stream,
               (const hcp_bf16*)x, (const hcp_bf16*)dy, gamma, beta, stats, dgamma, dbeta, HW, C, G, silu, rpb);
    HCP_LAUNCH_CHECK("groupnorm_affine_grad");
}

HCP_API int hcp_layernorm_affine_grad(const void* x, const void* dy, const float* stats, float* dgamma, float* dbeta, int M, int C,
                                      hipStream_t stream) {
    HCP_REQUIRE(x && dy && stats && dgamma && dbeta && M > 0 && C > 0 && C % 8 == 0, "hcp_layernorm_affine_grad: bad arguments");
    const int ct = hcp_cdiv(C, 64);
    int rpb; const int splits = affine_grad_blocks(M, ct, 1, &rpb);
    HCP_LAUNCH((norm_affine_grad_kernel<false>), dim3(ct, splits, 1), dim3(256), 32 * 129 * sizeof(float), stream,
               (const hcp_bf16*)x, (const hcp_bf16*)dy, (const float*)nullptr, (const float*)nullptr, stats, dgamma, dbeta, M, C, 1, 0, rpb);
    HCP_LAUNCH_CHECK("layernorm_affine_grad");
}
```

hcp_diffusion_amd/csrc/runtime.hip:

```cpp
#include "hcp_common.h"

static thread_local char g_err[512] = "";

extern "C" int hcp_set_error(const char* fmt, ...) {
    va_list ap;
    va_start(ap, fmt);
    vsnprintf(g_err, sizeof(g_err), fmt, ap);
    va_end(ap);
    return -1;
}

HCP_API const char* hcp_last_error(void) { return g_err; }

HCP_API int hcp_is_emulated(void) { return HCP_IS_EMULATED; }

HCP_API int hcp_abi_version(void) { return 4; }

namespace {
HCP_KERNEL(256) atomics_selfcheck_kernel(float* line, float* bucket, int nb, int stride) {
    const int tid = threadIdx.x;
    const float v = (float)((tid & 3) + 1);
    hcp_atomic_add(line + (tid & 15), v);
    const int idx = (int)(((long)blockIdx.x * 37 + (long)tid * 101) % nb);
    hcp_atomic_add(bucket + (size_t)idx * stride, v);
}
}

HCP_API int hcp_selfcheck_atomics(float* line, float* bucket, int nb, int stride, int workgroups, hipStream_t stream) {
    HCP_REQUIRE(line && bucket && nb > 0 && stride > 0 && workgroups > 0 && workgroups <= 4096, "hcp_selfcheck_atomics: bad arguments");
    if (hcp_memset_async(line, 0, 16 * sizeof(float), stream) != 0 || hcp_memset_async(bucket, 0, (size_t)nb * stride * sizeof(float), stream) != 0)
        return hcp_set_error("hcp_selfcheck_atomics: clearing the targets failed");
    HCP_LAUNCH(atomics_selfcheck_kernel, dim3(workgroups), dim3(256), 0, stream, line, bucket, nb, stride);
    HCP_LAUNCH_CHECK("atomics_selfcheck");
}
```

hcp_diffusion_amd/kernels.py:

```python
import ctypes
import math
import os
import torch

from . import _lib

_backend = None


def lib():
    global _backend
    if _backend is None:
        _backend = _lib.load()
    return _backend


def _set_backend_for_tests(cdll):
    global _backend
    _backend = _lib.bind(cdll) if cdll is not None else None


def _chk(rc, name):
    if rc != 0:
        raise _lib.HcpError(f"{name}: {lib().hcp_last_error().decode()}")
# ... 18 lines not shown

BF16 = torch.bfloat16

_WS = {}
_WGTAB = {}
_WS_BYTES = 256 << 20
WGRAD_GRID_BLOCKS = 16384


def _workspace(t):
    key = (t.device.type, t.device.index)
    ws = _WS.get(key)
    if ws is None:
        ws = torch.empty(_WS_BYTES if t.is_cuda else (16 << 20), dtype=torch.uint8, device=t.device)
        _WS[key] = ws
    return ws


def atomics_selfcheck(device, workgroups=2048, nb=4099, stride=37):
    dev = torch.device(device)
    line = torch.empty(16, dtype=torch.float32, device=dev)
    bucket = torch.empty(nb * stride, dtype=torch.float32, device=dev)
    _chk(lib().hcp_selfcheck_atomics(_p(line), _p(bucket), nb, stride, workgroups, _stream(line)), "hcp_selfcheck_atomics")
    w = torch.arange(workgroups, dtype=torch.int64).view(-1, 1)
    t = torch.arange(256, dtype=torch.int64).view(1, -1)
    want_b = torch.zeros(nb, dtype=torch.int64).index_add_(0, ((37 * w + 101 * t) % nb).flatten(), ((t & 3) + 1).expand(workgroups, 256).flatten())
    want_l = workgroups * 16 * ((torch.arange(16) & 3) + 1)
    got_l, got_b = line.cpu().double(), bucket.cpu()[::stride].double()
    bad_l = int((got_l != want_l.double()).sum()); bad_b = int((got_b != want_b.double()).sum())
    if bad_l or bad_b:
        worst = float(((got_b - want_b.double()).abs() / want_b.double().clamp(min=1)).max())
        raise _lib.HcpError(f"fp32 atomics self-check FAILED on {dev}: {bad_l}/16 words of the shared line and {bad_b}/{nb} strided words differ "
                            f"from the exact integer sums (worst relative error {worst:.3g}); no result of this device can be trusted")
    return True


TRACE = None
LAUNCHES = None


def _launch(kind, **d):
    d["kind"] = kind
    LAUNCHES.append(d)


def _lo_pair(residual, residual_lo, want_lo, M, N, dev):
    if residual_lo is not None:
        assert residual is not None and residual_lo.dtype == BF16 and residual_lo.shape == (M, N) and residual_lo.stride() == residual.stride()
    return torch.empty((M, N), dtype=BF16, device=dev) if want_lo else None


def gemm(a, b, *, a2=None, b2=None, bias=None, rowbias=None, rows_per_group=1, residual=None, alpha=1.0,
         out_f32=False, out=None, residual_lo=None, want_lo=False, want_gact=False):
    _bf16_2d(a, "a"); _bf16_2d(b, "b")
    M, K = a.shape
    N = b.shape[0]
    assert b.shape[1] == K
    K2 = 0
    if a2 is not None:
        _bf16_2d(a2, "a2"); _bf16_2d(b2, "b2")
        K2 = a2.shape[1]
        assert a2.shape[0] == M and b2.shape == (N, K2)
    if TRACE is not None:
        TRACE.append(("gemm", M, N, K, 1 if K2 else 0))
    if out is None:
        out = torch.empty((M, N), dtype=torch.float32 if out_f32 else BF16, device=a.device)
    assert out.stride(1) == 1
    if LAUNCHES is not None:
        _launch("gemm", M=M, N=N, K=K, K2=K2, lda=a.stride(0), ldb=b.stride(0), ldd=out.stride(0),
                lda2=a2.stride(0) if K2 else 0, ldb2=b2.stride(0) if K2 else 0, ldr=residual.stride(0) if residual is not None else 0,
                bias=bias is not None, rowbias=rowbias is not None, rows_per_group=rows_per_group if rowbias is not None else 0,
                residual=residual is not None, residual_lo=residual_lo is not None, want_lo=bool(want_lo), gact=bool(want_gact),
                alpha=float(alpha), out_f32=out.dtype == torch.float32)
    if bias is not None:
        assert bias.dtype == torch.float32 and bias.numel() == N and bias.is_contiguous()
    if rowbias is not None:
        assert rowbias.dtype == torch.float32 and rowbias.shape[1] == N and rowbias.stride(1) == 1
    if residual is not None:
        _bf16_2d(residual, "residual"); assert residual.shape == (M, N)
    ws = _workspace(a)
    assert not want_lo or (out.dtype == BF16 and out.is_contiguous())
    out_lo = _lo_pair(residual, residual_lo, want_lo, M, N, a.device)
    gact = torch.empty((M, N // 2), dtype=BF16, device=a.device) if want_gact else None
    _chk(lib().hcp_gemm_bf16(_p(a), a.stride(0), _p(b), b.stride(0), _p(out), out.stride(0), M, N, K,
                             _p(a2), a2.stride(0) if a2 is not None else 0, _p(b2), b2.stride(0) if b2 is not None else 0,
                             K2, _p(bias), _p(rowbias), rowbias.stride(0) if rowbias is not None else 0, rows_per_group,
                             _p(residual), residual.stride(0) if residual is not None else 0, _p(residual_lo), _p(out_lo), _p(gact), float(alpha),
                             1 if out.dtype == torch.float32 else 0, _p(ws), ws.numel(), _stream(a)), "hcp_gemm_bf16")
    if want_gact:
        return out, gact
    return (out, out_lo) if want_lo else out


T_SPLIT = os.environ.get("HCP_T_SPLIT") == "1"


def t_lo(t):
    return 32 if (t is not None and T_SPLIT and t.shape[1] == 64 and t.stride(0) == 64) else 0


def gemm_lora(a, b, l, e, *, bias=None, residual=None, want_t=True, residual_lo=None, want_lo=False, want_gact=False):
    _bf16_2d(a, "a"); _bf16_2d(b, "b"); _bf16_2d(l, "l"); _bf16_2d(e, "e")
    M, Kd = a.shape
    N = b.shape[0]
    assert b.shape[1] == Kd and l.shape == (32, Kd) and e.shape == (N, 32) and l.is_contiguous() and e.is_contiguous()
    if TRACE is not None:
        TRACE.append(("lora", M, N, Kd))
    out = torch.empty((M, N), dtype=BF16, device=a.device)
    ldt = 64 if T_SPLIT else 32
    if LAUNCHES is not None:
        _launch("gemm_lora", M=M, N=N, K=Kd, lda=a.stride(0), ldb=b.stride(0), ldd=N, ldt=ldt, want_t=bool(want_t),
                ldr=residual.stride(0) if residual is not None else 0, bias=bias is not None, residual=residual is not None,
                residual_lo=residual_lo is not None, want_lo=bool(want_lo), gact=bool(want_gact))
    t = torch.empty((M, ldt), dtype=BF16, device=a.device) if want_t else None
    if bias is not None:
        assert bias.dtype == torch.float32 and bias.numel() == N and bias.is_contiguous()
    if residual is not None:
        _bf16_2d(residual, "residual"); assert residual.shape == (M, N)
    ws = _workspace(a)
    out_lo = _lo_pair(residual, residual_lo, want_lo, M, N, a.device)
    gact = torch.empty((M, N // 2), dtype=BF16, device=a.device) if want_gact else None
    _chk(lib().hcp_gemm_lora_bf16(_p(a), a.stride(0), _p(b), b.stride(0), _p(l), _p(e), _p(t), ldt, _p(out), N, M, N, Kd, _p(bias),
                                  _p(residual), residual.stride(0) if residual is not None else 0, _p(residual_lo), _p(out_lo), _p(gact),
                                  _p(ws), ws.numel(), _stream(a)),
         "hcp_gemm_lora_bf16")
    if want_gact:
        return (out, gact), t
    return ((out, out_lo) if want_lo else out), t


def gemm_geglu_bwd(dy, wt, hg, *, l=None, e=None, want_t=True):
    _bf16_2d(dy, "dy"); _bf16_2d(wt, "wt"); _bf16_2d(hg, "hg")
    M, C = dy.shape
    Fd = wt.shape[0]
    assert wt.shape[1] == C and hg.shape == (M, 2 * Fd) and hg.is_contiguous()
    if TRACE is not None:
        TRACE.append(("lora", M, Fd, C) if l is not None else ("gemm", M, Fd, C, 0))
    if LAUNCHES is not None:
        _launch("gemm_geglu_bwd", M=M, N=Fd, K=C, lda=dy.stride(0), ldb=wt.stride(0), ldd=2 * Fd, lora=l is not None,
                ldt=(64 if T_SPLIT else 32) if l is not None else 0, want_t=bool(want_t) and l is not None)
    dhg = torch.empty((M, 2 * Fd), dtype=BF16, device=dy.device)
    u = None
    if l is not None:
        _bf16_2d(l, "l"); _bf16_2d(e, "e")
        assert l.shape == (32, C) and e.shape == (Fd, 32) and l.is_contiguous() and e.is_contiguous()
        u = torch.empty((M, 64 if T_SPLIT else 32), dtype=BF16, device=dy.device) if want_t else None
    ws = _workspace(dy)
    _chk(lib().hcp_gemm_geglu_bwd_bf16(_p(dy), dy.stride(0), _p(wt), wt.stride(0), _p(l), _p(e), _p(u), 64 if T_SPLIT else 32, _p(hg), _p(dhg), M, Fd, C,
                                       _p(ws), ws.numel(), _stream(dy)), "hcp_gemm_geglu_bwd_bf16")
    return dhg, u


def conv3x3(x1, wp, cout, *, x2=None, stride=1, upsample=False, mode=0, out_hw=None, bias=None, rowbias=None,
            residual=None, out_f32=False, a2=None, b2=None, pad=1, out=None):
    assert x1.dtype == BF16 and x1.dim() == 4 and x1.is_contiguous()
    B, Hs, Ws, C1 = x1.shape
    C2 = 0
    if x2 is not None:
        assert x2.dtype == BF16 and x2.is_contiguous() and x2.shape[:3] == x1.shape[:3]
        C2 = x2.shape[3]
    assert wp.dtype == BF16 and wp.is_contiguous() and wp.numel() == cout * 9 * (C1 + C2)
    if mode == 0:
        up = 2 if upsample else 1
        Ho = (Hs * up + (2 if pad else 1) - 3) // stride + 1
        Wo = (Ws * up + (2 if pad else 1) - 3) // stride + 1
    else:
        Ho, Wo = out_hw
    if TRACE is not None:
        TRACE.append(("conv", mode, B, Hs, Ws, C1, C2, cout, stride, 1 if upsample else 0, Ho, Wo, 1 if a2 is not None else 0))
    if LAUNCHES is not None:
        _launch("conv3x3", M=B * Ho * Wo, N=cout, K=9 * (C1 + C2), K2=32 if a2 is not None else 0, mode=mode, B=B, Hs=Hs, Ws=Ws, C1=C1, C2=C2,
                Cout=cout, stride=stride, upsample=1 if upsample else 0, pad=pad, Ho=Ho, Wo=Wo, ldd=cout, ldr=cout if residual is not None else 0,
                bias=bias is not None, rowbias=rowbias is not None, rows_per_group=Ho * Wo if rowbias is not None else 0,
                residual=residual is not None, out_f32=bool(out_f32))
    if out is None:
        out = torch.empty((B, Ho, Wo, cout), dtype=torch.float32 if out_f32 else BF16, device=x1.device)
    assert out.dtype == (torch.float32 if out_f32 else BF16) and out.is_contiguous() and tuple(out.shape) == (B, Ho, Wo, cout)
    if residual is not None:
        assert residual.dtype == BF16 and residual.is_contiguous() and residual.numel() == out.numel()
    if rowbias is not None:
        assert rowbias.dtype == torch.float32 and rowbias.shape == (B, cout) and rowbias.stride(1) == 1
    if bias is not None:
        assert bias.dtype == torch.float32 and bias.numel() == cout and bias.is_contiguous()
    if a2 is not None:
        assert a2.dtype == BF16 and b2.dtype == BF16 and a2.is_contiguous() and b2.is_contiguous()
        assert a2.numel() == B * Ho * Wo * 32 and tuple(b2.shape) == (cout, 32)
    ws = _workspace(x1)
    _chk(lib().hcp_conv3x3_bf16(_p(x1), C1, _p(x2), C2, B, Hs, Ws, Ho, Wo, mode, stride, 1 if upsample else 0, pad, _p(wp),
                                cout, _p(out), cout, _p(bias), _p(rowbias), rowbias.stride(0) if rowbias is not None else 0,
                                _p(residual), cout, 1 if out_f32 else 0, _p(a2), _p(b2), _p(ws), ws.numel(), _stream(x1)),
         "hcp_conv3x3_bf16")
    return out


def wgrad_linear(dy, x, dw):
    assert dy.dtype == BF16 and x.dtype == BF16 and dw.dtype == torch.float32 and dy.dim() == 2 and x.dim() == 2
    assert dy.stride(1) == 1 and x.stride(1) == 1 and dw.stride(1) == 1 and dy.shape[0] == x.shape[0]
    M, N = dy.shape
    K = x.shape[1]
    assert tuple(dw.shape) == (N, K)
    if LAUNCHES is not None:
        _launch("wgrad_linear", M=M, N=N, K=K, ldy=dy.stride(0), ldx=x.stride(0), ldw=dw.stride(0))
    ws = _workspace(x)
    _chk(lib().hcp_wgrad_linear_bf16(_p(dy), dy.stride(0), _p(x), x.stride(0), _p(dw), dw.stride(0), M, N, K, _p(ws), ws.numel(),
                                     _stream(x)), "hcp_wgrad_linear_bf16")


def wgrad_conv3x3(dy, x1, dw, *, x2=None, stride=1, upsample=False, cout=None, col0=0):
    assert dy.dtype == BF16 and x1.dtype == BF16 and dw.dtype == torch.float32 and dy.is_contiguous() and x1.is_contiguous()
    B, Hs, Ws, C1 = x1.shape
    C2 = 0
    if x2 is not None:
        assert x2.dtype == BF16 and x2.is_contiguous() and x2.shape[:3] == x1.shape[:3]
        C2 = x2.shape[3]
    _, Ho, Wo, ldy = dy.shape
    cout = cout or ldy
    cw = dw.numel() // (cout * 9)
    assert dw.numel() == cout * 9 * cw and cw <= C1 + C2
    ws = _workspace(x1)
    assert col0 % 8 == 0 and col0 + (cout + 7) // 8 * 8 <= ldy
    if LAUNCHES is not None:
        _launch("wgrad_conv3x3", M=B * Ho * Wo, N=cout, K=9 * (C1 + C2), B=B, Hs=Hs, Ws=Ws, C1=C1, C2=C2, Cout=cout, Cw=cw, stride=stride,
                upsample=1 if upsample else 0, Ho=Ho, Wo=Wo, ldy=ldy, col0=col0)
    dyp = ctypes.c_void_p(dy.data_ptr() + 2 * col0)
    _chk(lib().hcp_wgrad_conv3x3_bf16(dyp, ldy, _p(x1), C1, _p(x2), C2, _p(dw), cw, B, Hs, Ws, Ho, Wo, cout, stride,
                                      1 if upsample else 0, _p(ws), ws.numel(), _stream(x1)), "hcp_wgrad_conv3x3_bf16")


def colsum(y, out, rows_per_group=None):
    assert y.dtype == BF16 and y.dim() == 2 and y.stride(1) == 1 and out.dtype == torch.float32
    M, N = y.shape
    rpg = rows_per_group or M
    ldo = out.stride(0) if out.dim() == 2 else N
    _chk(lib().hcp_colsum_bf16(_p(y), y.stride(0), _p(out), ldo, M, N, rpg, _stream(y)), "hcp_colsum_bf16")


def _attn_strides(t):
    assert t.dtype == BF16 and t.dim() == 3 and t.stride(2) == 1
    return t.stride(0), t.stride(1)


def _key_bias(key_bias, B, Nk):
    if key_bias is None:
        return None, 0
    assert key_bias.dtype == torch.float32 and tuple(key_bias.shape) == (B, Nk) and key_bias.stride(1) == 1
    return key_bias, key_bias.stride(0)


def attention_fwd(q, k, v, heads, scale=None, key_bias=None, causal=False, q_prescaled=False):
    B, Nq, C = q.shape
    Nk = k.shape[1]
    D = C // heads
    scale = scale if scale is not None else 1.0 / math.sqrt(D)
    o = torch.empty((B, Nq, C), dtype=BF16, device=q.device)
    lse = torch.empty((B, heads, Nq), dtype=torch.float32, device=q.device)
    qb, qr = _attn_strides(q); kb, kr = _attn_strides(k); vb, vr = _attn_strides(v); ob, orr = _attn_strides(o)
    kbt, kbs = _key_bias(key_bias, B, Nk)
    _chk(lib().hcp_attention_fwd(_p(q), _p(k), _p(v), _p(o), _p(lse), B, heads, Nq, Nk, D, qb, qr, kb, kr, vb, vr, ob, orr,
                                 float(scale), _p(kbt), kbs, (1 if causal else 0) | (2 if q_prescaled else 0), _stream(q)), "hcp_attention_fwd")
    return o, lse


def attention_bwd(q, k, v, o, do, lse, heads, scale=None, out=None, key_bias=None, causal=False, q_prescaled=False):
    B, Nq, C = q.shape
    Nk = k.shape[1]
    D = C // heads
    scale = scale if scale is not None else 1.0 / math.sqrt(D)
    assert o.is_contiguous() and do.is_contiguous()
    if out is None:
        assert q.is_contiguous() and k.is_contiguous() and v.is_contiguous(), "strided q/k/v need matching `out` buffers"
        dq = torch.empty_like(q); dk = torch.empty_like(k); dv = torch.empty_like(v)
    else:
        dq, dk, dv = out
        assert dq.stride() == q.stride() and dk.stride() == k.stride() and dv.stride() == v.stride()
    delta = torch.empty((B, heads, Nq), dtype=torch.float32, device=q.device)
    qb, qr = _attn_strides(q); kb, kr = _attn_strides(k); vb, vr = _attn_strides(v); ob, orr = _attn_strides(o)
    ws = _workspace(q)
    kbt, kbs = _key_bias(key_bias, B, Nk)
    _chk(lib().hcp_attention_bwd(_p(q), _p(k), _p(v), _p(o), _p(do), _p(lse), _p(delta), _p(dq), _p(dk), _p(dv), B, heads,
                                 Nq, Nk, D, qb, qr, kb, kr, vb, vr, ob, orr, float(scale), _p(kbt), kbs,
                                 (1 if causal else 0) | (2 if q_prescaled else 0), _p(ws),
                                 ws.numel(), _stream(q)), "hcp_attention_bwd")
    return dq, dk, dv


def _gn_ws(x, B, HW, C, G):
    n = lib().hcp_groupnorm_workspace_bytes(B, HW, C, G)
    return torch.empty((max(n, 4) // 4,), dtype=torch.float32, device=x.device)


def groupnorm_fwd(x, gamma, beta, groups, eps, silu):
    assert x.dtype == BF16 and x.is_contiguous()
    B, C = x.shape[0], x.shape[-1]
    HW = x.numel() // (B * C)
    y = torch.empty_like(x)
    stats = torch.empty((B, groups, 2), dtype=torch.float32, device=x.device)
    ws = _gn_ws(x, B, HW, C, groups)
    _chk(lib().hcp_groupnorm_silu_fwd(_p(x), _p(gamma), _p(beta), _p(y), _p(stats), _p(ws), B, HW, C, groups, float(eps),
                                      1 if silu else 0, _stream(x)), "hcp_groupnorm_silu_fwd")
    return y, stats


def groupnorm_bwd(x, dy, gamma, beta, stats, groups, silu, addend=None):
    assert x.dtype == BF16 and x.is_contiguous() and dy.dtype == BF16 and dy.is_contiguous()
    assert addend is None or (addend.dtype == BF16 and addend.is_contiguous() and addend.numel() == x.numel())
    B, C = x.shape[0], x.shape[-1]
    HW = x.numel() // (B * C)
    dx = torch.empty_like(x)
    ws = _gn_ws(x, B, HW, C, groups)
    _chk(lib().hcp_groupnorm_silu_bwd(_p(x), _p(dy), _p(gamma), _p(beta), _p(stats), _p(addend), _p(dx), _p(ws), B, HW, C, groups,
                                      1 if silu else 0, _stream(x)), "hcp_groupnorm_silu_bwd")
    return dx


def groupnorm_affine_grad(x, dy, gamma, beta, stats, groups, silu, dgamma, dbeta):
    B, C = x.shape[0], x.shape[-1]
    HW = x.numel() // (B * C)
    assert x.is_contiguous() and dy.is_contiguous() and dgamma.dtype == torch.float32 and dbeta.dtype == torch.float32
    _chk(lib().hcp_groupnorm_affine_grad(_p(x), _p(dy), _p(gamma), _p(beta), _p(stats), _p(dgamma), _p(dbeta), B, HW, C, groups,
                                         1 if silu else 0, _stream(x)), "hcp_groupnorm_affine_grad")


def layernorm_affine_grad(x, dy, stats, dgamma, dbeta):
    C = x.shape[-1]
    M = x.numel() // C
    assert x.is_contiguous() and dy.is_contiguous() and dgamma.dtype == torch.float32 and dbeta.dtype == torch.float32
    _chk(lib().hcp_layernorm_affine_grad(_p(x), _p(dy), _p(stats), _p(dgamma), _p(dbeta), M, C, _stream(x)),
         "hcp_layernorm_affine_grad")


def _lo_like(t, ref):
    assert t is None or (t.dtype == BF16 and t.is_contiguous() and t.numel() == ref.numel())
    return t


def layernorm_fwd(x, gamma, beta, eps, x_lo=None):
    assert x.dtype == BF16 and x.is_contiguous()
    C = x.shape[-1]; M = x.numel() // C
    y = torch.empty_like(x)
    stats = torch.empty((M, 2), dtype=torch.float32, device=x.device)
    _chk(lib().hcp_layernorm_fwd(_p(x), _p(_lo_like(x_lo, x)), _p(gamma), _p(beta), _p(y), _p(stats), M, C, float(eps), _stream(x)), "hcp_layernorm_fwd")
    return y, stats


def layernorm_bwd(x, dy, gamma, stats, addend=None, x_lo=None, addend_lo=None, want_lo=False):
    assert x.is_contiguous() and dy.is_contiguous() and dy.dtype == BF16
    assert addend is None or (addend.dtype == BF16 and addend.is_contiguous() and addend.numel() == x.numel())
    C = x.shape[-1]; M = x.numel() // C
    dx = torch.empty_like(x)
    dx_lo = torch.empty_like(x) if want_lo else None
    _chk(lib().hcp_layernorm_bwd(_p(x), _p(_lo_like(x_lo, x)), _p(dy), _p(gamma), _p(stats), _p(addend), _p(_lo_like(addend_lo, x)), _p(dx),
                                 _p(dx_lo), M, C, _stream(x)), "hcp_layernorm_bwd")
    return (dx, dx_lo) if want_lo else dx


def geglu_fwd(h):
    assert h.dtype == BF16 and h.is_contiguous()
    F2 = h.shape[-1]; F = F2 // 2; M = h.numel() // F2
    y = torch.empty(h.shape[:-1] + (F,), dtype=BF16, device=h.device)
    _chk(lib().hcp_geglu_fwd(_p(h), _p(y), M, F, _stream(h)), "hcp_geglu_fwd")
    return y


def geglu_bwd(h, dy):
    assert h.is_contiguous() and dy.is_contiguous() and dy.dtype == BF16
    F2 = h.shape[-1]; F = F2 // 2; M = h.numel() // F2
    dh = torch.empty_like(h)
    _chk(lib().hcp_geglu_bwd(_p(h), _p(dy), _p(dh), M, F, _stream(h)), "hcp_geglu_bwd")
    return dh


def add(a, b):
    assert a.dtype == BF16 and b.dtype == BF16 and a.is_contiguous() and b.is_contiguous() and a.numel() == b.numel()
    o = torch.empty_like(a)
    _chk(lib().hcp_add_bf16(_p(a), _p(b), _p(o), a.numel(), _stream(a)), "hcp_add_bf16")
    return o


def concat_channels(a, b):
    assert a.dtype == BF16 and b.dtype == BF16 and a.is_contiguous() and b.is_contiguous() and a.shape[:-1] == b.shape[:-1]
    c1, c2 = a.shape[-1], b.shape[-1]
    M = a.numel() // c1
    out = torch.empty(a.shape[:-1] + (c1 + c2,), dtype=BF16, device=a.device)
    o2 = out.view(M, c1 + c2)
    _chk(lib().hcp_concat2_bf16(_p(a), c1, _p(b), c2, _p(o2), M, 0, _stream(a)), "hcp_concat2_bf16")
    return out


def split_channels(d, c1):
    assert d.dtype == BF16 and d.is_contiguous()
    c = d.shape[-1]; c2 = c - c1
    M = d.numel() // c
    d2 = d.view(M, c)
    a = torch.empty(d.shape[:-1] + (c1,), dtype=BF16, device=d.device)
    b = torch.empty(d.shape[:-1] + (c2,), dtype=BF16, device=d.device)
    _chk(lib().hcp_concat2_bf16(_p(a), c1, _p(b), c2, _p(d2), M, 1, _stream(d)), "hcp_concat2_bf16")
    return a, b


def silu_fwd(x):
    assert x.dtype == BF16 and x.is_contiguous()
    y = torch.empty_like(x)
    _chk(lib().hcp_silu_fwd(_p(x), _p(y), x.numel(), _stream(x)), "hcp_silu_fwd")
    return y


def silu_bwd(x, dy):
    dx = torch.empty_like(x)
    _chk(lib().hcp_silu_bwd(_p(x), _p(dy), _p(dx), x.numel(), _stream(x)), "hcp_silu_bwd")
    return dx


def nchw_to_nhwc(x, cpad=None):
    assert x.dim() == 4 and x.is_contiguous() and x.dtype in (torch.float32, BF16)
    B, C, H, W = x.shape
    cp = cpad or C
    y = torch.empty((B, H, W, cp), dtype=BF16, device=x.device)
    _chk(lib().hcp_nchw_to_nhwc_bf16(_p(x), 1 if x.dtype == torch.float32 else 0, _p(y), B, C, H * W, cp, _stream(x)),
         "hcp_nchw_to_nhwc_bf16")
    return y


def nhwc_to_nchw_f32(x, c):
    assert x.dim() == 4 and x.is_contiguous() and x.dtype == torch.float32
    B, H, W, Cs = x.shape
    y = torch.empty((B, c, H, W), dtype=torch.float32, device=x.device)
    _chk(lib().hcp_nhwc_to_nchw_f32(_p(x), _p(y), B, c, H * W, Cs, _stream(x)), "hcp_nhwc_to_nchw_f32")
    return y


def upsample2x_bwd(dup):
    assert dup.dtype == BF16 and dup.is_contiguous()
    B, H2, W2, C = dup.shape
    dx = torch.empty((B, H2 // 2, W2 // 2, C), dtype=BF16, device=dup.device)
    _chk(lib().hcp_upsample2x_bwd(_p(dup), _p(dx), B, H2 // 2, W2 // 2, C, _stream(dup)), "hcp_upsample2x_bwd")
    return dx


def timestep_embedding(t, dim, max_period=10000.0):
    assert t.dtype in (torch.int64, torch.float32) and t.is_contiguous()
    emb = torch.empty((t.numel(), dim), dtype=BF16, device=t.device)
    if t.dtype == torch.int64:
        _chk(lib().hcp_timestep_embedding(_p(t), _p(emb), t.numel(), dim, float(max_period), _stream(t)), "hcp_timestep_embedding")
    else:
        _chk(lib().hcp_timestep_embedding_f32(_p(t), _p(emb), t.numel(), dim, float(max_period), _stream(t)),
             "hcp_timestep_embedding_f32")
    return emb


def add_noise(x0, noise, t, alphas_cumprod):
    assert x0.dtype == torch.float32 and noise.dtype == torch.float32 and x0.is_contiguous() and noise.is_contiguous()
    assert t.dtype == torch.int64 and alphas_cumprod.dtype == torch.float32
    xt = torch.empty_like(x0)
    B = x0.shape[0]
    _chk(lib().hcp_add_noise(_p(x0), _p(noise), _p(t), _p(alphas_cumprod), _p(xt), B, x0.numel() // B, _stream(x0)), "hcp_add_noise")
    return xt


def cfg_ddim_step(x, eps2, a_t, a_prev, guidance_scale=1.0, out=None):
    assert x.dtype == torch.float32 and eps2.dtype == torch.float32 and x.is_contiguous() and eps2.is_contiguous()
    guided = eps2.numel() == 2 * x.numel()
    assert guided or eps2.numel() == x.numel()
    out = torch.empty_like(x) if out is None else out
    _chk(lib().hcp_cfg_ddim_step(_p(x), _p(eps2), _p(out), x.numel(), 1 if guided else 0, float(guidance_scale), float(a_t), float(a_prev),
                                 _stream(x)), "hcp_cfg_ddim_step")
# ... 254 lines not shown
```

hcp_diffusion_amd/ops.py:

```python
import os
import threading
from contextlib import contextmanager

import torch

from . import kernels as K

BF16 = torch.bfloat16



class WgradContext:
    def __init__(self, grouped=False, side_stream=False):
        self.grouped, self.side = bool(grouped), bool(side_stream)
        self.items, self.keep = [], []
        self.stream, self.side_keep = None, []

    def add(self, U, x2, gd, T, dy2, gu, rank, alpha, slot0=0, ulo=0, tlo=0):
        if self.grouped:
            self.items.append((U, x2, gd, T, dy2, gu, rank, alpha, slot0, ulo, tlo))
            return
        if slot0 != 0 or not dy2.is_contiguous() or (ulo != 0) != (U.shape[1] == 64) or (tlo != 0) != (T.shape[1] == 64):
            self.keep = [K.lora_wgrad_grouped([(U, x2, gd, T, dy2, gu, rank, alpha, slot0, ulo, tlo)])]
            return
# ... 264 lines not shown
    outs = _CtxKVFn.apply(x, batch, *params)
    node = outs[0].grad_fn
    if node is not None:
        d3 = node.dkv_all.view(*x.shape[:-1], batch.n_total)
        for kv, g, o in zip(outs, batch.groups, batch.n_off):
            kv._hcp_grad_buf = d3[..., o:o + g.n_total]
    return outs


def linear_group(x, group):
    for h in group.hosts:
        assert _tr(h.weight) is None and _tr(h.bias) is None, "fused projection groups require frozen host weights"
    params = [p for b in group.blocks if b is not None for p in (b.layer.W_down, b.layer.W_up)]
    return _LinearGroupFn.apply(x, group, *params)


class _Conv3x3Fn(torch.autograd.Function):

    @staticmethod
    def forward(ctx, x1, x2, rowbias, residual, host, stride, upsample, hw=None, hb=None, lora=None, w_down=None, w_up=None):
        pk = host.packed()
        T = None
        if lora is not None and getattr(lora, "wide", False):
            lp = lora.packed()
            rp = lora.rank_pad
            T = K.conv3x3(x1, lp.ad, rp, x2=x2, stride=stride, upsample=upsample)
            y0 = K.conv3x3(x1, pk.w, pk.cout, x2=x2, stride=stride, upsample=upsample, bias=pk.bias, rowbias=rowbias, residual=residual)
            y = K.gemm(T.view(-1, rp), lp.bu, residual=y0.view(-1, pk.cout)).view_as(y0)
        elif lora is not None:
            lp = lora.packed()
            T = K.conv3x3(x1, lp.ad, 32, x2=x2, stride=stride, upsample=upsample)
            y = K.conv3x3(x1, pk.w, pk.cout, x2=x2, stride=stride, upsample=upsample, bias=pk.bias, rowbias=rowbias, residual=residual,
                          a2=T, b2=lp.bu)
        else:
            y = K.conv3x3(x1, pk.w, pk.cout, x2=x2, stride=stride, upsample=upsample, bias=pk.bias, rowbias=rowbias, residual=residual)
        ctx.host, ctx.stride, ctx.upsample, ctx.lora = host, stride, upsample, lora
        ctx.in_shape = x1.shape
        ctx.c2 = x2.shape[-1] if x2 is not None else 0
        ctx.has_res = residual is not None
        ctx.train_w, ctx.train_b = hw is not None, hb is not None
        keep_x = hw is not None or lora is not None
        ctx.save_for_backward(x1 if keep_x else None, x2 if keep_x else None, T)
        return y

    @staticmethod
    def backward(ctx, dy):
        pk = ctx.host.packed()
        dy = dy.contiguous()
        B, H, W, C1 = ctx.in_shape
        hw = (H * 2, W * 2) if ctx.upsample else (H, W)
        dx1 = dx2 = None
        x1, x2, T = ctx.saved_tensors
        lora = ctx.lora
        dl1 = dl2 = None
        if lora is not None:
            lp = lora.packed()
            rp = lp.but.shape[0]
            U = K.gemm(dy.view(-1, dy.shape[-1]), lp.but).view(*dy.shape[:-1], rp)
            T2 = T.view(-1, rp)
            for blk, s0 in lora.members():
                gd, gu = blk.grad_views()
                for j in range(0, blk.rank, 32):
                    K.lora_wgrad(T2[:, s0 + j:], dy.view(-1, dy.shape[-1]), gu, min(32, blk.rank - j), blk.alpha_f, True, out_col0=j)
                K.wgrad_conv3x3(U, x1, gd, x2=x2, stride=ctx.stride, upsample=ctx.upsample, cout=blk.rank, col0=s0)
            if ctx.needs_input_grad[0]:
                dl1 = K.conv3x3(U, lp.wdl[:C1], C1, mode=1, stride=ctx.stride, out_hw=hw)
            if ctx.c2 and ctx.needs_input_grad[1]:
                dl2 = K.conv3x3(U, lp.wdl[C1:], ctx.c2, mode=1, stride=ctx.stride, out_hw=hw)
        if ctx.needs_input_grad[0]:
            dx1 = K.conv3x3(dy, pk.wd[:C1], C1, mode=1, stride=ctx.stride, out_hw=hw, residual=dl1)
            if ctx.upsample:
                dx1 = K.upsample2x_bwd(dx1)
        if ctx.c2 and ctx.needs_input_grad[1]:
            dx2 = K.conv3x3(dy, pk.wd[C1:], ctx.c2, mode=1, stride=ctx.stride, out_hw=hw, residual=dl2)
        drb = None
        dy2 = dy.view(-1, dy.shape[-1])
        if ctx.needs_input_grad[2]:
            drb = torch.zeros((B, dy.shape[-1]), dtype=torch.float32, device=dy.device)
            K.colsum(dy2, drb, dy.shape[1] * dy.shape[2])
        if ctx.train_w:
            K.wgrad_conv3x3(dy, x1, grad_buffer(ctx.host.weight, True), x2=x2, stride=ctx.stride, upsample=ctx.upsample)
        if ctx.train_b:
            K.colsum(dy2, grad_buffer(ctx.host.bias))
        return dx1, dx2, drb, (dy if ctx.has_res else None), None, None, None, None, None, None, None, None


def conv3x3(x1, host, *, x2=None, rowbias=None, residual=None, stride=1, upsample=False, lora=None):
    wd = lora.layer.W_down if lora is not None else None
    wu = lora.layer.W_up if lora is not None else None
    return _Conv3x3Fn.apply(x1, x2, rowbias, residual, host, stride, upsample, _tr(host.weight), _tr(host.bias), lora, wd, wu)


def _gn_affine(ctx, x, dy, g, b, stats):
    if ctx.train:
        K.groupnorm_affine_grad(x, dy, g, b, stats, ctx.gn.num_groups, ctx.silu, grad_buffer(ctx.gn.weight), grad_buffer(ctx.gn.bias))


def _norm_tr(m):
    w, b = _tr(m.weight), _tr(m.bias)
    if (w is None) != (b is None):
        raise NotImplementedError("hcp_diffusion_amd: a norm layer's weight and bias must be trainable together")
    return w, b


class _GroupNormFn(torch.autograd.Function):
    @staticmethod
    def forward(ctx, x, gn, silu, hw=None, hb=None):
        g, b = gn.f32_params()
        y, stats = K.groupnorm_fwd(x, g, b, gn.num_groups, gn.eps, silu)
        ctx.save_for_backward(x, stats)
        ctx.gn, ctx.silu, ctx.train = gn, silu, hw is not None
        return y

    @staticmethod
    def backward(ctx, dy):
        x, stats = ctx.saved_tensors
        g, b = ctx.gn.f32_params()
        dy = dy.contiguous()
        _gn_affine(ctx, x, dy, g, b, stats)
        dx = K.groupnorm_bwd(x, dy, g, b, stats, ctx.gn.num_groups, ctx.silu) if ctx.needs_input_grad[0] else None
        return dx, None, None, None, None


def groupnorm(x, gn, silu):
    return _GroupNormFn.apply(x, gn, silu, *_norm_tr(gn))


class _GroupNormForkFn(torch.autograd.Function):

    @staticmethod
    def forward(ctx, x, gn, silu, hw=None, hb=None):
        g, b = gn.f32_params()
        y, stats = K.groupnorm_fwd(x, g, b, gn.num_groups, gn.eps, silu)
        ctx.save_for_backward(x, stats)
        ctx.gn, ctx.silu, ctx.train = gn, silu, hw is not None
        return y, x.view_as(x)

    @staticmethod
    def backward(ctx, dy, dskip):
        x, stats = ctx.saved_tensors
        g, b = ctx.gn.f32_params()
        if dy is None:
            return dskip, None, None, None, None
        dy = dy.contiguous()
        _gn_affine(ctx, x, dy, g, b, stats)
        return K.groupnorm_bwd(x, dy, g, b, stats, ctx.gn.num_groups, ctx.silu,
                               dskip.contiguous() if dskip is not None else None), None, None, None, None


def groupnorm_fork(x, gn, silu):
    return _GroupNormForkFn.apply(x, gn, silu, *_norm_tr(gn))


class _LayerNormFn(torch.autograd.Function):
    @staticmethod
    def forward(ctx, x, ln, hw=None, hb=None):
        g, b = ln.f32_params()
        y, stats = K.layernorm_fwd(x, g, b, ln.eps)
        ctx.save_for_backward(x, stats)
        ctx.ln, ctx.train = ln, hw is not None
        return y

    @staticmethod
    def backward(ctx, dy):
        x, stats = ctx.saved_tensors
        g, _ = ctx.ln.f32_params()
        dy = dy.contiguous()
        if ctx.train:
            K.layernorm_affine_grad(x, dy, stats, grad_buffer(ctx.ln.weight), grad_buffer(ctx.ln.bias))
        return (K.layernorm_bwd(x, dy, g, stats) if ctx.needs_input_grad[0] else None), None, None, None


def layernorm(x, ln):
    return _LayerNormFn.apply(x, ln, *_norm_tr(ln))


class _LayerNormForkFn(torch.autograd.Function):

    @staticmethod
    def forward(ctx, x, ln, hw=None, hb=None, x_lo=None, stream=False):
        g, b = ln.f32_params()
        y, stats = K.layernorm_fwd(x, g, b, ln.eps, x_lo=x_lo)
        ctx.save_for_backward(x, stats, x_lo)
        ctx.ln, ctx.train, ctx.stream = ln, hw is not None, stream
        if stream:
            ctx.set_materialize_grads(False)
            return y, x.view_as(x), (x_lo.view_as(x_lo) if x_lo is not None else None)
        return y, x.view_as(x)

    @staticmethod
    def backward(ctx, dy, dskip, dskip_lo=None):
        x, stats, x_lo = ctx.saved_tensors
        g, _ = ctx.ln.f32_params()
        if dy is None:
            return dskip, None, None, None, dskip_lo, None
        dy = dy.contiguous()
        if ctx.train:
            K.layernorm_affine_grad(x, dy, stats, grad_buffer(ctx.ln.weight), grad_buffer(ctx.ln.bias))
        if ctx.stream:
            want_lo = x_lo is not None
            r = K.layernorm_bwd(x, dy, g, stats, dskip.contiguous() if dskip is not None else None, x_lo=x_lo,
                                addend_lo=dskip_lo.contiguous() if (dskip_lo is not None and dskip is not None) else None, want_lo=want_lo)
            return (r[0], None, None, None, r[1], None) if want_lo else (r, None, None, None, None, None)
        return K.layernorm_bwd(x, dy, g, stats, dskip.contiguous() if dskip is not None else None), None, None, None, None, None


def layernorm_fork(x, ln):
    return _LayerNormForkFn.apply(x, ln, *_norm_tr(ln))


def layernorm_fork_stream(hi, lo, ln):
    return _LayerNormForkFn.apply(hi, ln, *_norm_tr(ln), lo, True)


class _GegluFn(torch.autograd.Function):
    @staticmethod
    def forward(ctx, h):
        ctx.save_for_backward(h)
        return K.geglu_fwd(h)

    @staticmethod
    def backward(ctx, dy):
        (h,) = ctx.saved_tensors
        return K.geglu_bwd(h, dy.contiguous())


geglu = _GegluFn.apply


class _GegluLinearFn(torch.autograd.Function):

    @staticmethod
    def forward(ctx, hg, residual, w_down, w_up, host, lora, hw=None, hb=None, residual_lo=None, stream=False, gact=None):
        shp = hg.shape
        hg2 = hg.reshape(-1, shp[-1])
        x2 = gact.reshape(-1, gact.shape[-1]) if gact is not None else K.geglu_fwd(hg2)
        res2 = residual.reshape(-1, residual.shape[-1]) if residual is not None else None
        lo2 = residual_lo.reshape(-1, residual_lo.shape[-1]) if residual_lo is not None else None
        pk = host.packed()
        T = None
        if lora is not None:
            lp = lora.packed()
            y, T = K.gemm_lora(x2, pk.w, lp.ad, lp.bu, bias=pk.bias, residual=res2, residual_lo=lo2, want_lo=stream)
        else:
            y = K.gemm(x2, pk.w, bias=pk.bias, residual=res2, residual_lo=lo2, want_lo=stream)
        ctx.host, ctx.lora = host, lora
        ctx.wg = current_wgrad()
        ctx.train_w, ctx.train_b = hw is not None, hb is not None
        ctx.save_for_backward(hg2, x2 if (lora is not None or hw is not None) else None, T)
        ctx.hshape = shp
        ctx.has_res = residual is not None
        ctx.has_lo = residual_lo is not None
        if stream:
            ctx.set_materialize_grads(False)
            return y[0].view(*shp[:-1], y[0].shape[-1]), y[1].view(*shp[:-1], y[1].shape[-1])
        return y.view(*shp[:-1], y.shape[-1])

    @staticmethod
    def backward(ctx, dy, dy_lo=None):
        if dy is None:
            assert dy_lo is None
            return (None,) * 11
        hg2, x2, T = ctx.saved_tensors
        host, lora = ctx.host, ctx.lora
        dy2 = dy.reshape(-1, dy.shape[-1])
        if not dy2.is_contiguous():
            dy2 = dy2.contiguous()
        pk = host.packed()
        dhg = None
        if lora is not None:
            lp = lora.packed()
            if ctx.needs_input_grad[0]:
                dhg, U = K.gemm_geglu_bwd(dy2, pk.wt, hg2, l=lp.but, e=lp.adt)
            else:
                U = K.gemm(dy2, lp.but)
            for blk, s0 in lora.members():
                gd, gu = blk.grad_views()
                ctx.wg.add(U, x2, gd, T, dy2, gu, blk.rank, blk.alpha_f, s0, K.t_lo(U), K.t_lo(T))
        elif ctx.needs_input_grad[0]:
            dhg, _ = K.gemm_geglu_bwd(dy2, pk.wt, hg2)
        if ctx.train_w:
            gw = grad_buffer(host.weight)
            K.wgrad_linear(dy2, x2, gw.view(gw.shape[0], -1))
        if ctx.train_b:
            K.colsum(dy2, grad_buffer(host.bias))
        if dhg is not None:
            dhg = dhg.view(ctx.hshape)
        return dhg, (dy if ctx.has_res else None), None, None, None, None, None, None, (dy_lo if ctx.has_lo else None), None, None


def geglu_linear(hg, host, lora=None, residual=None, gact=None):
    wd = lora.layer.W_down if lora is not None else None
    wu = lora.layer.W_up if lora is not None else None
    if isinstance(residual, tuple):
        return _GegluLinearFn.apply(hg, residual[0], wd, wu, host, lora, _tr(host.weight), _tr(host.bias), residual[1], True, gact)
    return _GegluLinearFn.apply(hg, residual, wd, wu, host, lora, _tr(host.weight), _tr(host.bias), None, False, gact)


class _AttentionFn(torch.autograd.Function):
    @staticmethod
    def forward(ctx, q, k, v, heads, key_bias=None, causal=False):
        o, lse = K.attention_fwd(q, k, v, heads, key_bias=key_bias, causal=causal)
        ctx.save_for_backward(q, k, v, o, lse, key_bias)
        ctx.heads, ctx.causal = heads, causal
        return o

# ... 302 lines not shown
```

hcp_diffusion_amd/unet.py:

```python
import os

import torch
from torch import nn

from . import kernels as K
from . import ops
from .layers import HipConv2d, HipConvIn, HipConvOut, HipGroupNorm, HipLayerNorm, HipLinear

BF16 = torch.bfloat16

SD15_CONFIG = dict(
    in_channels=4, out_channels=4, block_out_channels=(320, 640, 1280, 1280), layers_per_block=2,
    down_block_types=("CrossAttnDownBlock2D", "CrossAttnDownBlock2D", "CrossAttnDownBlock2D", "DownBlock2D"),
    up_block_types=("UpBlock2D", "CrossAttnUpBlock2D", "CrossAttnUpBlock2D", "CrossAttnUpBlock2D"),
    num_attention_heads=8, cross_attention_dim=768, norm_num_groups=32, num_train_timesteps=1000,
    transformer_layers_per_block=1, use_linear_projection=False, addition_embed_type=None, addition_time_embed_dim=None,
    projection_class_embeddings_input_dim=None)

SDXL_CONFIG = dict(
    in_channels=4, out_channels=4, block_out_channels=(320, 640, 1280), layers_per_block=2,
    down_block_types=("DownBlock2D", "CrossAttnDownBlock2D", "CrossAttnDownBlock2D"),
    up_block_types=("CrossAttnUpBlock2D", "CrossAttnUpBlock2D", "UpBlock2D"),
    num_attention_heads=(5, 10, 20), cross_attention_dim=2048, norm_num_groups=32, num_train_timesteps=1000,
    transformer_layers_per_block=(1, 2, 10), use_linear_projection=True, addition_embed_type="text_time",
    addition_time_embed_dim=256, projection_class_embeddings_input_dim=2816)


def _per_block(v, i):
    return v[i] if isinstance(v, (tuple, list)) else v


def _call_res(mod, x, residual):
    if isinstance(residual, tuple):
        leaf = _ff_out_leaf(mod)
        if leaf is not None:
            return ops.linear_stream(x, leaf[0], leaf[1], residual[0], residual[1])
        return _call_res(mod, x, residual[0]), None
    if getattr(mod, "supports_fused_residual", False):
        return mod(x, residual=residual)
    return ops.add(mod(x), residual)


def _ckpt(module, fn, *args, **kwargs):
    if getattr(module, "gradient_checkpointing", False) and torch.is_grad_enabled():
        from torch.utils.checkpoint import checkpoint
        wg = ops.current_wgrad()

        def run(*a, **k):
            with ops.wgrad_context(wg):
                return fn(*a, **k)
        return checkpoint(run, *args, use_reentrant=False, preserve_rng_state=False, **kwargs)
    return fn(*args, **kwargs)


def _tb(temb_act, resnet):
    table = getattr(temb_act, "_hcp_tb", None)
    return table.get(id(resnet)) if table is not None else None


class Timesteps(nn.Module):
    def __init__(self, dim):
        super().__init__()
        self.num_channels = dim

    def forward(self, t):
        return K.timestep_embedding(t.contiguous(), self.num_channels)


class SiLU(nn.Module):
    def forward(self, x):
        return ops.silu(x)


class TimestepEmbedding(nn.Module):
    def __init__(self, cin, dim):
        super().__init__()
        self.linear_1 = HipLinear(cin, dim)
        self.act = SiLU()
        self.linear_2 = HipLinear(dim, dim)

    def forward(self, x):
        return self.linear_2(self.act(self.linear_1(x)))


class ResnetBlock2D(nn.Module):
    def __init__(self, cin, cout, temb_dim, groups, eps=1e-5):
        super().__init__()
        self.norm1 = HipGroupNorm(groups, cin, eps=eps)
        self.conv1 = HipConv2d(cin, cout, 3, 1, 1)
        self.time_emb_proj = HipLinear(temb_dim, cout)
        self.norm2 = HipGroupNorm(groups, cout, eps=eps)
        self.dropout = nn.Dropout(0.0)
        self.conv2 = HipConv2d(cout, cout, 3, 1, 1)
        self.nonlinearity = SiLU()
        if cin != cout:
            self.conv_shortcut = HipConv2d(cin, cout, 1)
        self.gradient_checkpointing = False

    def forward(self, x, temb_act, skip=None, temb_bias=None):
        if skip is not None:
            x = ops.concat_channels(x, skip)
        h, x = self.norm1(x, silu=True, fork=True)
        if temb_bias is not None:
            tb = temb_bias
        elif (isinstance(self.time_emb_proj, HipLinear) and not temb_act.requires_grad
              and not self.time_emb_proj.weight.requires_grad):
            tb = self.time_emb_proj(temb_act, out_f32=True)
        else:
            tb = self.time_emb_proj(temb_act).float()
        h = self.conv1(h, rowbias=tb)
        h = self.norm2(h, silu=True)
        sc = self.conv_shortcut(x) if hasattr(self, "conv_shortcut") else x
        return self.conv2(h, residual=sc)


LOG2E = 1.4426950408889634


def _fusable_linear(m):
    from .lora import LoraHipContainer
    host, blk = m, None
    if isinstance(m, LoraHipContainer):
        if type(m) is not LoraHipContainer or len(m.plugin_names) != 1:
            return None
        host, blk = m._host, m[m.plugin_names[0]]
        if m._forward_hooks or m._forward_pre_hooks:
            return None
    if type(host) is not HipLinear or host.bias is not None or host._forward_hooks or host._forward_pre_hooks:
        return None
    if host.weight.requires_grad:
        return None
    if blk is not None and blk.wide:
        return None
    if blk is not None and blk.dropout.p > 0.0:
        return None
    return host, blk




def _ff_out_leaf(m):
    from .lora import LoraHipContainer
    if isinstance(m, LoraHipContainer):
        if (type(m) is not LoraHipContainer or len(m.plugin_names) != 1 or m._forward_hooks or m._forward_pre_hooks or type(m._host) is not HipLinear
                or m._host._forward_hooks or m._host._forward_pre_hooks):
            return None
        blk = m[m.plugin_names[0]]
        if blk.wide or blk.host_type == "conv" or (blk.dropout.p > 0.0 and blk.training):
            return None
        return m._host, blk
    if type(m) is HipLinear and not (m._forward_hooks or m._forward_pre_hooks):
        return m, None
    return None


class CrossAttention(nn.Module):
    def __init__(self, dim, ctx_dim, heads):
        super().__init__()
        self.heads, self.head_dim = heads, dim // heads
        self.to_q = HipLinear(dim, dim, bias=False)
        self.to_k = HipLinear(ctx_dim, dim, bias=False)
        self.to_v = HipLinear(ctx_dim, dim, bias=False)
        self.to_out = nn.ModuleList([HipLinear(dim, dim), nn.Dropout(0.0)])
        self._groups = {}

    def _group(self, mods, scales=None):
        from .lora import FusedLoraGroup
        key = tuple(id(m) for m in mods)
        hit = self._groups.get(key)
        if hit is not None:
            return hit[0]
        pairs = [_fusable_linear(m) for m in mods]
        group = None
        if all(p is not None for p in pairs):
            blocks = [p[1] for p in pairs]
            buckets = {id(b._bucket) for b in blocks if b is not None}
            ok = len(buckets) <= 1 and all(b is None or b._bucket is not None for b in blocks)
            if ok and sum(8 * ((b.rank + 7) // 8) for b in blocks if b is not None) <= 32:
                group = FusedLoraGroup([p[0] for p in pairs], blocks, scales)
                lb = next((b for b in blocks if b is not None), None)
                group.bucket = lb._bucket if lb is not None else None
                if lb is not None:
                    group.bucket.add_group(group)
        if len(self._groups) >= 6:
            self._groups.pop(next(iter(self._groups)))
        self._groups[key] = (group, mods)
        return group

    def forward(self, x, context=None, residual=None, key_bias=None):
        qc = self.head_dim ** -0.5 * LOG2E
        if context is None:
            g = self._group((self.to_q, self.to_k, self.to_v), (qc, 1.0, 1.0))
            gq = gkv = None
            if g is None:
                gkv = self._group((self.to_k, self.to_v))
                gq = self._group((self.to_q,), (qc,)) if gkv is not None else None
            if g is not None:
                o = ops.attention_packed(ops.linear_group(x, g), None, self.heads, q_prescaled=True)
            elif gq is not None:
                o = ops.attention_packed(ops.linear_group(x, gq), ops.linear_group(x, gkv), self.heads, None, q_prescaled=True)
            else:
                o = ops.attention(self.to_q(x), self.to_k(x), self.to_v(x), self.heads)
        else:
            g = self._group((self.to_k, self.to_v))
            gq = self._group((self.to_q,), (qc,)) if (g is not None and key_bias is None) else None
            pre = getattr(context, "_hcp_kv", None)
            kv = pre.get(id(self)) if (pre is not None and g is not None) else None
            if g is not None and kv is None:
                kv = ops.linear_group(context, g)
            if g is not None and gq is not None:
                o = ops.attention_packed(ops.linear_group(x, gq), kv, self.heads, None, q_prescaled=True)
            elif g is not None:
                o = ops.attention_packed(self.to_q(x), kv, self.heads, key_bias)
            else:
                o = ops.attention(self.to_q(x), self.to_k(context), self.to_v(context), self.heads, key_bias)
        return _call_res(self.to_out[0], o, residual) if residual is not None else self.to_out[0](o)


class GEGLU(nn.Module):
    def __init__(self, dim, inner):
        super().__init__()
        self.proj = HipLinear(dim, inner * 2)

    def forward(self, x):
        return ops.geglu(self.proj(x))


class FeedForward(nn.Module):
    geglu_in_epilogue = False

    def __init__(self, dim):
        super().__init__()
        self.net = nn.ModuleList([GEGLU(dim, dim * 4), nn.Dropout(0.0), HipLinear(dim * 4, dim)])

    def forward(self, x, residual=None):
        leaf = _ff_out_leaf(self.net[2]) if not (self.net[0]._forward_hooks or self.net[0]._forward_pre_hooks) and self.net[1].p == 0.0 else None
        if leaf is not None and type(self.net[0]) is GEGLU:
            pleaf = _ff_out_leaf(self.net[0].proj) if self.geglu_in_epilogue else None
            if pleaf is not None:
                hg, act = ops.linear_geglu(x, pleaf[0], pleaf[1])
                return ops.geglu_linear(hg, leaf[0], leaf[1], residual, gact=act)
            return ops.geglu_linear(self.net[0].proj(x), leaf[0], leaf[1], residual)
        h = self.net[0](x)
        return _call_res(self.net[2], h, residual) if residual is not None else self.net[2](h)


class BasicTransformerBlock(nn.Module):
    def __init__(self, dim, ctx_dim, heads):
        super().__init__()
        self.attn1 = CrossAttention(dim, dim, heads)
        self.ff = FeedForward(dim)
        self.attn2 = CrossAttention(dim, ctx_dim, heads)
        self.norm1 = HipLayerNorm(dim)
        self.norm2 = HipLayerNorm(dim)
        self.norm3 = HipLayerNorm(dim)

    def forward(self, x, context):
        context, key_bias = context if isinstance(context, tuple) else (context, None)
        if isinstance(x, tuple):
            h, hi, lo = ops.layernorm_fork_stream(x[0], x[1], self.norm1)
            x = self.attn1(h, residual=(hi, lo))
            h, hi, lo = ops.layernorm_fork_stream(x[0], x[1], self.norm2)
            x = self.attn2(h, context, residual=(hi, lo), key_bias=key_bias)
            h, hi, lo = ops.layernorm_fork_stream(x[0], x[1], self.norm3)
            return self.ff(h, residual=(hi, lo))
        h, x = self.norm1(x, fork=True)
# ... 372 lines not shown
```

include/hcp_mi355x.h:

```cpp
#ifndef HCP_MI355X_H
#define HCP_MI355X_H
#include <stddef.h>

#ifdef __cplusplus
extern "C" {
#endif

typedef struct ihipStream_t* hcpStream_t;

const char* hcp_last_error(void);
int hcp_is_emulated(void);
#define HCP_ABI_VERSION 4
int hcp_abi_version(void);
int hcp_selfcheck_atomics(float* line, float* bucket, int nb, int stride, int workgroups, hcpStream_t stream);

int hcp_gemm_bf16(const void* A, int lda, const void* B, int ldb, void* D, int ldd, int M, int N, int K, const void* A2,
                  int lda2, const void* B2, int ldb2, int K2, const float* bias, const float* rowbias, int rowbias_ld,
                  int rows_per_group, const void* residual, int ldr, const void* residual_lo, void* D_lo, void* gact, float alpha,
                  int out_f32, void* workspace, size_t workspace_bytes, hcpStream_t stream);
int hcp_gemm_lora_bf16(const void* A, int lda, const void* B, int ldb, const void* L, const void* E, void* Tout, int ldt, void* D,
                       int ldd, int M, int N, int K, const float* bias, const void* residual, int ldr, const void* residual_lo, void* D_lo,
                       void* gact, void* workspace, size_t workspace_bytes, hcpStream_t stream);
int hcp_gemm_geglu_bwd_bf16(const void* A, int lda, const void* B, int ldb, const void* L, const void* E, void* Tout, int ldt,
                            const void* HG, void* DHG, int M, int F, int K, void* workspace, size_t workspace_bytes, hcpStream_t stream);
size_t hcp_gemm_workspace_bytes(int M, int N);

int hcp_conv3x3_bf16(const void* X1, int C1, const void* X2, int C2, int B, int Hs, int Ws, int Ho, int Wo, int mode,
                     int stride, int upsample, int pad, const void* Wp, int Cout, void* D, int ldd, const float* bias,
                     const float* rowbias, int rowbias_ld, const void* residual, int ldr, int out_f32, const void* A2,
                     const void* B2, void* workspace, size_t workspace_bytes, hcpStream_t stream);

int hcp_attention_fwd(const void* Q, const void* K, const void* V, void* O, float* lse, int B, int H, int Nq, int Nk, int D,
                      long q_bs, int q_rs, long k_bs, int k_rs, long v_bs, int v_rs, long o_bs, int o_rs, float scale,
                      const float* key_bias, long key_bias_bs, int causal, hcpStream_t stream);
int hcp_attention_bwd(const void* Q, const void* K, const void* V, const void* O, const void* dO, const float* lse,
                      float* delta_ws , void* dQ, void* dK, void* dV, int B, int H, int Nq, int Nk, int D,
                      long q_bs, int q_rs, long k_bs, int k_rs, long v_bs, int v_rs, long o_bs, int o_rs, float scale,
                      const float* key_bias, long key_bias_bs, int causal, void* workspace, size_t workspace_bytes,
                      hcpStream_t stream);


size_t hcp_groupnorm_workspace_bytes(int B, int HW, int C, int G);
int hcp_groupnorm_silu_fwd(const void* x, const float* gamma, const float* beta, void* y, float* stats, void* workspace,
                           int B, int HW, int C, int G, float eps, int silu, hcpStream_t stream);
int hcp_groupnorm_silu_bwd(const void* x, const void* dy, const float* gamma, const float* beta, const float* stats,
                           const void* addend , void* dx,
                           void* workspace, int B, int HW, int C, int G, int silu, hcpStream_t stream);

int hcp_layernorm_fwd(const void* x, const void* x_lo, const float* gamma, const float* beta, void* y, float* stats, int M, int C,
                      float eps, hcpStream_t stream);
int hcp_layernorm_bwd(const void* x, const void* x_lo, const void* dy, const float* gamma, const float* stats, const void* addend,
                      const void* addend_lo, void* dx, void* dx_lo, int M, int C, hcpStream_t stream);

int hcp_geglu_fwd(const void* h, void* y, long M, int F, hcpStream_t stream);
int hcp_geglu_bwd(const void* h, const void* dy, void* dh, long M, int F, hcpStream_t stream);

int hcp_add_bf16(const void* a, const void* b, void* out, long n, hcpStream_t stream);
int hcp_copy2d_bf16(const void* src, int sld, void* dst, int dld, long M, int C, hcpStream_t stream);
int hcp_concat2_bf16(void* a, int c1, void* b, int c2, void* joint, long M, int split, hcpStream_t stream);
int hcp_silu_fwd(const void* x, void* y, long n, hcpStream_t stream);
int hcp_silu_bwd(const void* x, const void* dy, void* dx, long n, hcpStream_t stream);
int hcp_nchw_to_nhwc_bf16(const void* src, int src_is_f32, void* dst, int B, int C, int HW, int Cpad, hcpStream_t stream);
int hcp_nhwc_to_nchw_f32(const float* src, float* dst, int B, int C, int HW, int Csrc, hcpStream_t stream);
int hcp_upsample2x_bwd(const void* dup, void* dx, int B, int H, int W, int C, hcpStream_t stream);

int hcp_wgrad_linear_bf16(const void* dY, int ldy, const void* X, int ldx, float* dW, int ldw, int M, int N, int K,
                          float* workspace, size_t workspace_bytes, hcpStream_t stream);
int hcp_wgrad_conv3x3_bf16(const void* dY, int ldy, const void* X1, int C1, const void* X2, int C2, float* dW, int Cw, int B,
                           int Hs, int Ws, int Ho, int Wo, int Cout, int stride, int upsample, float* workspace,
                           size_t workspace_bytes, hcpStream_t stream);
int hcp_colsum_bf16(const void* Y, int ldy, float* out, int ldo, int M, int N, int rows_per_group, hcpStream_t stream);
int hcp_pack_piece_bytes(void);
int hcp_pack_weights(const void* pieces, int count, int total_tiles, hcpStream_t stream);
int hcp_groupnorm_affine_grad(const void* x, const void* dy, const float* gamma, const float* beta, const float* stats,
                              float* dgamma, float* dbeta, int B, int HW, int C, int G, int silu, hcpStream_t stream);
int hcp_layernorm_affine_grad(const void* x, const void* dy, const float* stats, float* dgamma, float* dbeta, int M, int C,
                              hcpStream_t stream);

int hcp_timestep_embedding(const long long* timesteps, void* emb, int B, int dim, float max_period, hcpStream_t stream);
int hcp_timestep_embedding_f32(const float* values, void* emb, int B, int dim, float max_period, hcpStream_t stream);
int hcp_add_noise(const float* x0, const float* noise, const long long* timesteps, const float* alphas_cumprod, float* xt,
                  int B, long per_sample, hcpStream_t stream);
int hcp_transpose_bf16(const void* src, void* dst, int batch, int R, int C, hcpStream_t stream);
int hcp_softmax_rows(const float* S, long lds, void* P, long ldp, int M, int N, float scale, hcpStream_t stream);
int hcp_vae_latent_sample(const float* moments, const float* Wq, const float* bq, const float* noise, float* latents, int B, int L,
                          long hw, float scale, hcpStream_t stream);
int hcp_quick_gelu(const void* x, const void* dy, void* out, long n, hcpStream_t stream);
int hcp_embedding_bf16(const float* token_table, const long long* ids, const float* position_table, const long long* position_ids,
                       void* out, long n, int C, int L, hcpStream_t stream);
int hcp_embedding_pt_fwd_bf16(const long long* ids, int B, int R, int W, int n_word, const float* token_table, int vocab,
                              const float* position_table, const long long* position_ids, int n_pos, const float* custom_table,
                              int n_custom, const int* custom_map, int n_map, void* out, int* src_map, int C, hcpStream_t stream);
int hcp_embedding_pt_bwd_f32(const void* dX, const int* src_map, long M, int C, float* grad, int n_custom, int beta, hcpStream_t stream);
int hcp_snr_loss_weight(const long long* timesteps, const float* alphas_cumprod, float* w, int B, int kind, float gamma,
                        hcpStream_t stream);
int hcp_mse_masked_mean(const float* pred, const float* target, const float* mask, int mask_channels,
                        const float* sample_weight, float* loss, float* grad, int B, int C, int HW, float weight,
                        hcpStream_t stream);

int hcp_lora_wgrad(const void* L, int ldl, int l_lo, const void* R, int ldr, float* out, int ldo, int M, int P, int Q, float scale,
                   int transpose_out, void* workspace, size_t workspace_bytes, hcpStream_t stream);
int hcp_lora_wgrad_pair(const void* U, int ldu, const void* x, int ldx, int K, float* grad_down, const void* T, int ldt, const void* dY,
                        int ldy, int N, float* grad_up, int M, int r, float scale, void* workspace, size_t workspace_bytes,
                        hcpStream_t stream);
int hcp_split_hi_lo_bf16(const float* src, void* dst, long M, int C, hcpStream_t stream);
int hcp_lora_wgrad_group_geometry(int M, int K, int N, int P, int target_blocks, int* qt_down, int* qt_up, int* splits,
                                  int* rows_per_split);
int hcp_lora_wgrad_group_desc_bytes(void);
int hcp_lora_wgrad_grouped(const void* descs, int count, int total_blocks, int total_tiles, long slab_units, void* workspace,
                           size_t workspace_bytes, hcpStream_t stream);
int hcp_lora_pack(const void* descs, int count, hcpStream_t stream);
int hcp_lora_pack_desc_bytes(void);

int hcp_sumsq_f32(const float* g, long n, float* out, hcpStream_t stream);
int hcp_adamw_clip_fused(float* p, float* g, float* m, float* v, long n, const float* lr, float beta1, float beta2,
                         float eps, float weight_decay, const float* sumsq, float grad_scale, float max_norm, int* step,
                         hcpStream_t stream);
int hcp_ema_update(float* ema, const float* p, long n, const int* step, float inv_gamma, float power, float decay_max,
                   hcpStream_t stream);
int hcp_cast_f32_bf16(float* src, void* dst_bf16, long n, float scale, int zero_src, hcpStream_t stream);
int hcp_cast_bf16_f32(const void* src_bf16, float* dst, long n, hcpStream_t stream);

int hcp_cfg_ddim_step(const float* x, const float* eps2, float* out, long n, int guided, float guidance_scale,
                      float alpha_cumprod_t, float alpha_cumprod_prev, hcpStream_t stream);


#define HCP_COMM_UNIQUE_ID_BYTES 128
int hcp_comm_unique_id(void* out128);
int hcp_comm_init(int rank, int world, const void* unique_id128, void** comm_out);
int hcp_comm_destroy(void* comm);
int hcp_comm_rank(const void* comm);
int hcp_comm_world(const void* comm);
int hcp_allreduce_flat(void* comm, void* buf, size_t count, int dtype, hcpStream_t stream);
int hcp_reduce_scatter_flat(void* comm, const void* send, void* recv, size_t recv_count, int dtype, hcpStream_t stream);
int hcp_allgather_flat(void* comm, const void* send, void* recv, size_t send_count, int dtype, hcpStream_t stream);

#ifdef __cplusplus
}
#endif
#endif
```

Baseline: 209.8 images/sec.

## Fold split-K conv reduction into following GroupNorm kernels in ResNet blocks

Adds a deferred-reduce conv3x3 entry point that leaves split-K partial slabs unreduced. New GroupNorm fwd/bwd slab variants sum the slabs, apply alpha, bias and rowbias, and optionally write the bf16 conv output, all inside the norm kernel. ResNet blocks are routed through new autograd functions that pair conv1 with norm2, and the conv dgrad with the norm backward. The aim is to drop the separate split-K reduce kernel and a round trip of the conv output through memory. The cost is more complex kernels, extra template instances, and a fallback condition that depends on hooks and which parameters are trainable.

```diff
diff --git a/hcp_diffusion_amd/_lib.py b/hcp_diffusion_amd/_lib.py
--- a/hcp_diffusion_amd/_lib.py
+++ b/hcp_diffusion_amd/_lib.py
@@ -17,11 +17,15 @@
     "hcp_gemm_geglu_bwd_bf16": (I, [P, I, P, I, P, P, P, I, P, P, I, I, I, P, c_size_t, P]),
     "hcp_gemm_workspace_bytes": (c_size_t, [I, I]),
     "hcp_conv3x3_bf16": (I, [P, I, P, I, I, I, I, I, I, I, I, I, I, P, I, P, I, P, P, I, P, I, I, P, P, P, c_size_t, P]),
+    "hcp_conv3x3_bf16_deferred": (I, [P, I, P, I, I, I, I, I, I, I, I, I, I, P, I, P, P, P, I, P, c_size_t, P, ctypes.POINTER(c_int)]),
     "hcp_attention_fwd": (I, [P, P, P, P, P, I, I, I, I, I, L, I, L, I, L, I, L, I, F, P, L, I, P]),
     "hcp_attention_bwd": (I, [P, P, P, P, P, P, P, P, P, P, I, I, I, I, I, L, I, L, I, L, I, L, I, F, P, L, I, P, c_size_t, P]),
     "hcp_groupnorm_workspace_bytes": (c_size_t, [I, I, I, I]),
     "hcp_groupnorm_silu_fwd": (I, [P, P, P, P, P, P, I, I, I, I, F, I, P]),
     "hcp_groupnorm_silu_bwd": (I, [P, P, P, P, P, P, P, P, I, I, I, I, I, P]),
+    "hcp_groupnorm_slab_path": (I, [I, I, I]),
+    "hcp_groupnorm_silu_fwd_slabs": (I, [P, I, F, P, P, I, P, P, P, P, P, I, I, I, I, F, I, P]),
+    "hcp_groupnorm_silu_bwd_slabs": (I, [P, P, I, P, P, P, P, P, P, I, I, I, I, I, P]),
     "hcp_layernorm_fwd": (I, [P, P, P, P, P, P, I, I, F, P]),
     "hcp_layernorm_bwd": (I, [P, P, P, P, P, P, P, P, P, I, I, P]),
     "hcp_geglu_fwd": (I, [P, P, L, I, P]),
@@ -95,7 +99,7 @@
 TOOLS_LIB_PATH = Path(__file__).resolve().parent / "libhcp_mi355x_tools.so"
 
 
-ABI_VERSION = 4
+ABI_VERSION = 5
 
 
 class HcpError(RuntimeError):
diff --git a/hcp_diffusion_amd/csrc/gemm.hip b/hcp_diffusion_amd/csrc/gemm.hip
--- a/hcp_diffusion_amd/csrc/gemm.hip
+++ b/hcp_diffusion_amd/csrc/gemm.hip
@@ -842,7 +842,7 @@
             } else {
                 HCP_LAUNCH((gemm_v2_kernel<BM, BN, WGM, WGN, MODE, LORA>), dim3(p.tiles_m * tiles_n, p.nsplit), dim3(64 * WGM * WGN), smem, stream, p);
             }
-            if (p.nsplit > 1) {
+            if (p.nsplit > 1 && !p.defer_reduce) {
                 long nv = (long)p.M * (p.N / 4);
                 int g = (int)((nv + 255) / 256); if (g > 2048) g = 2048;
                 HCP_LAUNCH(splitk_reduce_kernel, dim3(g), dim3(256), 0, stream, p);
@@ -859,7 +859,7 @@
         HCP_LAUNCH((gemm_glds_kernel<BM, BN, WGM, WGN, MODE, FAST, LORA, NSTAGE>), dim3(p.tiles_m * tiles_n, p.nsplit),
                    dim3(64 * WGM * WGN), smem, stream, p);
     }
-    if (p.nsplit > 1) {
+    if (p.nsplit > 1 && !p.defer_reduce) {
         long nv = (long)p.M * (p.N / 4);
         int g = (int)((nv + 255) / 256); if (g > 2048) g = 2048;
         HCP_LAUNCH(splitk_reduce_kernel, dim3(g), dim3(256), 0, stream, p);
@@ -891,7 +891,7 @@
         r = conv_patch_launch(p, bm, bn, mode, p.loaders - 8, stream);
     if (r == -2) r = gemm_pp_launch(p, bm, bn, mode, lora, p.loaders - 8, stream);
     if (r == -2) { p.geglu_out = gout; p.geglu_fused = 0; }
-    if (r != 0 || p.nsplit <= 1) return r;
+    if (r != 0 || p.nsplit <= 1 || p.defer_reduce) return r;
     long nv = (long)p.M * (p.N / 4);
     int g = (int)((nv + 255) / 256); if (g > 2048) g = 2048;
     HCP_LAUNCH(splitk_reduce_kernel, dim3(g), dim3(256), 0, stream, p);
@@ -1089,12 +1089,13 @@
     return finish_gact(p, gact, stream);
 }
 
-HCP_API int hcp_conv3x3_bf16(const void* X1, int C1, const void* X2, int C2, int Bn, int Hs, int Ws, int Ho, int Wo,
-                             int mode, int stride, int upsample, int pad, const void* Wp, int Cout, void* D, int ldd,
-                             const float* bias, const float* rowbias, int rowbias_ld, const void* residual, int ldr,
-                             int out_f32, const void* A2, const void* B2, void* workspace, size_t workspace_bytes,
-                             hipStream_t stream) {
+static int conv3x3_launch(const void* X1, int C1, const void* X2, int C2, int Bn, int Hs, int Ws, int Ho, int Wo,
+                          int mode, int stride, int upsample, int pad, const void* Wp, int Cout, void* D, int ldd,
+                          const float* bias, const float* rowbias, int rowbias_ld, const void* residual, int ldr,
+                          int out_f32, const void* A2, const void* B2, void* workspace, size_t workspace_bytes,
+                          hipStream_t stream, int* nsplit_out) {
     GemmParams p = {};
+    p.defer_reduce = nsplit_out != nullptr;
     HCP_REQUIRE(X1 && Wp && D, "hcp_conv3x3_bf16: null operand");
     HCP_REQUIRE((A2 == nullptr) == (B2 == nullptr), "hcp_conv3x3_bf16: the rank-32 K-extension needs both A2 and B2");
     if (A2) { p.A2 = (const hcp_bf16*)A2; p.lda2 = 32; p.B2 = (const hcp_bf16*)B2; p.ldb2 = 32; p.K2 = 32; }
@@ -1114,8 +1115,28 @@
     if (int e = check_common(p)) return e;
     float* ws = (float*)workspace; size_t wb = workspace ? workspace_bytes : 0;
     const bool fast = (C1 % 64 == 0) && (C2 % 64 == 0) && !upsample && !(mode == 1 && stride == 2);
-    if (mode == 0) return fast ? dispatch_gemm<1, true>(p, ws, wb, stream) : dispatch_gemm<1, false>(p, ws, wb, stream);
-    return fast ? dispatch_gemm<2, true>(p, ws, wb, stream) : dispatch_gemm<2, false>(p, ws, wb, stream);
+    const int rc = mode == 0 ? (fast ? dispatch_gemm<1, true>(p, ws, wb, stream) : dispatch_gemm<1, false>(p, ws, wb, stream))
+                             : (fast ? dispatch_gemm<2, true>(p, ws, wb, stream) : dispatch_gemm<2, false>(p, ws, wb, stream));
+    if (nsplit_out) *nsplit_out = p.nsplit;
+    return rc;
+}
+
+HCP_API int hcp_conv3x3_bf16(const void* X1, int C1, const void* X2, int C2, int Bn, int Hs, int Ws, int Ho, int Wo,
+                             int mode, int stride, int upsample, int pad, const void* Wp, int Cout, void* D, int ldd,
+                             const float* bias, const float* rowbias, int rowbias_ld, const void* residual, int ldr,
+                             int out_f32, const void* A2, const void* B2, void* workspace, size_t workspace_bytes,
+                             hipStream_t stream) {
+    return conv3x3_launch(X1, C1, X2, C2, Bn, Hs, Ws, Ho, Wo, mode, stride, upsample, pad, Wp, Cout, D, ldd, bias, rowbias, rowbias_ld,
+                          residual, ldr, out_f32, A2, B2, workspace, workspace_bytes, stream, nullptr);
+}
+
+HCP_API int hcp_conv3x3_bf16_deferred(const void* X1, int C1, const void* X2, int C2, int Bn, int Hs, int Ws, int Ho, int Wo,
+                                      int mode, int stride, int upsample, int pad, const void* Wp, int Cout, void* D,
+                                      const float* bias, const float* rowbias, int rowbias_ld, void* workspace,
+                                      size_t workspace_bytes, hipStream_t stream, int* nsplit) {
+    HCP_REQUIRE(nsplit, "hcp_conv3x3_bf16_deferred: null nsplit");
+    return conv3x3_launch(X1, C1, X2, C2, Bn, Hs, Ws, Ho, Wo, mode, stride, upsample, pad, Wp, Cout, D, Cout, bias, rowbias, rowbias_ld,
+                          nullptr, 0, 0, nullptr, nullptr, workspace, workspace_bytes, stream, nsplit);
 }
 
 HCP_API int hcp_gemm_geglu_bwd_bf16(const void* A, int lda, const void* B, int ldb, const void* L, const void* E, void* Tout, int ldt,
diff --git a/hcp_diffusion_amd/csrc/gemm_params.h b/hcp_diffusion_amd/csrc/gemm_params.h
--- a/hcp_diffusion_amd/csrc/gemm_params.h
+++ b/hcp_diffusion_amd/csrc/gemm_params.h
@@ -28,6 +28,7 @@
     int tiles_m;
     int nsplit; int kt_per_split;
     float* slabs;
+    int defer_reduce;
     const hcp_bf16* L; const hcp_bf16* E; hcp_bf16* Tout; int ldt;
     const hcp_bf16* geglu_hg; int geglu_ld;
     hcp_bf16* geglu_out; int geglu_fused;
diff --git a/hcp_diffusion_amd/csrc/norm.hip b/hcp_diffusion_amd/csrc/norm.hip
--- a/hcp_diffusion_amd/csrc/norm.hip
+++ b/hcp_diffusion_amd/csrc/norm.hip
@@ -291,8 +291,84 @@
 template <> struct GNChunk<4> { typedef hcp_bf16x4 T; typedef hcp_f32x4 F; };
 template <> struct GNChunk<2> { typedef hcp_bf16x2 T; typedef hcp_f32x2 F; };
 
+struct GNSlabSrc {
+    const float* slabs; size_t slab_elems; int ns;
+    float alpha; const float* bias; const float* rowbias; int rowbias_ld;
+    hcp_bf16* out;
+};
+
+template <int PC, int CE, int NS, int GCH>
+HCP_DEVICE void gn_add_slabs(const float* slabs, size_t slab_elems, int s, int i0, size_t base, int tid, int NT, int total, int cpr,
+                             unsigned cpr_magic, int C, typename GNChunk<CE>::F (&acc)[PC]) {
+    typedef typename GNChunk<CE>::F FV;
+    constexpr int GC = GCH < PC ? GCH : PC;
+    const char* const sbase = (const char*)(slabs + base);
+    const unsigned sbytes = (unsigned)slab_elems * 4u;
+#pragma unroll
+    for (int g0 = 0; g0 < PC; g0 += GC) {
+        FV t[GC][NS];
+#pragma unroll
+        for (int j = 0; j < GC; ++j) {
+            const int c = tid + (i0 + g0 + j) * NT;
+            int cg;
+            const unsigned bo = (unsigned)gn_slab_off<CE>(c < total ? c : 0, cpr, cpr_magic, C, &cg) * 4u;
+#pragma unroll
+            for (int k = 0; k < NS; ++k) t[j][k] = *(const FV*)(sbase + (bo + (unsigned)(s + k) * sbytes));
+        }
+#pragma unroll
+        for (int j = 0; j < GC; ++j) {
+#pragma unroll
+            for (int k = 0; k < NS; ++k) acc[g0 + j] += t[j][k];
+        }
+        if (PC > GC) hcp_sched_fence();
+    }
+}
+
 template <int NCH, int CE>
-HCP_KERNEL(1024) gn_slab_fwd(const hcp_bf16* x, const float* gamma, const float* beta, float* stats, hcp_bf16* y, int HW, int C,
+HCP_DEVICE void gn_sum_slabs(const GNSlabSrc sp, float* s_bi, float* s_rb, size_t base, int b, int g, int Cg, int tid, int NT, int total,
+                             int cpr, unsigned cpr_magic, int C, typename GNChunk<CE>::T (&v)[NCH]) {
+    typedef typename GNChunk<CE>::T V;
+    typedef typename GNChunk<CE>::F FV;
+    constexpr int PC = NCH * CE <= 32 ? NCH : 32 / CE;
+    constexpr int G4 = 8 / CE;
+    for (int j = tid; j < Cg; j += NT) {
+        s_bi[j] = sp.bias ? sp.bias[g * Cg + j] : 0.f;
+        s_rb[j] = sp.rowbias ? sp.rowbias[(size_t)b * sp.rowbias_ld + g * Cg + j] : 0.f;
+    }
+#pragma unroll
+    for (int i0 = 0; i0 < NCH; i0 += PC) {
+        FV acc[PC];
+#pragma unroll
+        for (int i = 0; i < PC; ++i) {
+            const int c = tid + (i0 + i) * NT;
+            int cg;
+            acc[i] = *(const FV*)((const char*)(sp.slabs + base) + (unsigned)gn_slab_off<CE>(c < total ? c : 0, cpr, cpr_magic, C, &cg) * 4u);
+        }
+        int s = 1;
+        for (; s + 4 <= sp.ns; s += 4) gn_add_slabs<PC, CE, 4, G4>(sp.slabs, sp.slab_elems, s, i0, base, tid, NT, total, cpr, cpr_magic, C, acc);
+        if (s + 2 <= sp.ns) { gn_add_slabs<PC, CE, 2, 2 * G4>(sp.slabs, sp.slab_elems, s, i0, base, tid, NT, total, cpr, cpr_magic, C, acc); s += 2; }
+        if (s < sp.ns) gn_add_slabs<PC, CE, 1, 4 * G4>(sp.slabs, sp.slab_elems, s, i0, base, tid, NT, total, cpr, cpr_magic, C, acc);
+        if (i0 == 0) HCP_SYNC();
+#pragma unroll
+        for (int i = 0; i < PC; ++i) {
+            const int c = tid + (i0 + i) * NT;
+            int cg;
+            const size_t off = gn_slab_off<CE>(c < total ? c : 0, cpr, cpr_magic, C, &cg);
+            FV a = acc[i] * sp.alpha;
+            if (sp.bias) a += *(const FV*)(s_bi + cg);
+            if (sp.rowbias) a += *(const FV*)(s_rb + cg);
+            V o;
+#pragma unroll
+            for (int e = 0; e < CE; ++e) o[e] = (short)hcp_f2bf(a[e]);
+            v[i0 + i] = o;
+            if (sp.out && c < total) *(V*)(sp.out + base + off) = o;
+        }
+        if (NCH > PC) hcp_sched_fence();
+    }
+}
+
+template <int NCH, int CE, bool SL>
+HCP_KERNEL(1024) gn_slab_fwd(const hcp_bf16* x, GNSlabSrc sp, const float* gamma, const float* beta, float* stats, hcp_bf16* y, int HW, int C,
                              int G, int cpr, unsigned cpr_magic, int silu, float eps) {
     typedef typename GNChunk<CE>::T V;
     typedef typename GNChunk<CE>::F FV;
@@ -306,12 +382,15 @@
     for (int j = tid; j < Cg; j += NT) { s_ga[j] = gamma[g * Cg + j]; s_be[j] = beta[g * Cg + j]; }
     const size_t base = (size_t)b * HW * C + (size_t)g * Cg;
     V v[NCH];
-#pragma unroll
-    for (int i = 0; i < NCH; ++i) {
-        const int c = tid + i * NT;
-        int cg;
-        v[i] = *(const V*)(x + base + gn_slab_off<CE>(c < total ? c : 0, cpr, cpr_magic, C, &cg));
-        if (NCH > 8 && i % 8 == 7) hcp_sched_fence();
+    if constexpr (SL) gn_sum_slabs<NCH, CE>(sp, s_be + Cg, s_be + 2 * Cg, base, b, g, Cg, tid, NT, total, cpr, cpr_magic, C, v);
+    else {
+#pragma unroll
+        for (int i = 0; i < NCH; ++i) {
+            const int c = tid + i * NT;
+            int cg;
+            v[i] = *(const V*)(x + base + gn_slab_off<CE>(c < total ? c : 0, cpr, cpr_magic, C, &cg));
+            if (NCH > 8 && i % 8 == 7) hcp_sched_fence();
+        }
     }
     float s = 0.f;
 #pragma unroll
@@ -350,8 +429,8 @@
     }
 }
 
-template <int NCH, int CE>
-HCP_KERNEL(1024) gn_slab_bwd(const hcp_bf16* x, const hcp_bf16* dy, const float* gamma, const float* beta, const float* stats,
+template <int NCH, int CE, bool SL>
+HCP_KERNEL(1024) gn_slab_bwd(const hcp_bf16* x, const hcp_bf16* dy, GNSlabSrc sp, const float* gamma, const float* beta, const float* stats,
                              const hcp_bf16* addend, hcp_bf16* dx, int HW, int C, int G, int cpr, unsigned cpr_magic, int silu) {
     typedef typename GNChunk<CE>::T V;
     typedef typename GNChunk<CE>::F FV;
@@ -368,12 +447,14 @@
     constexpr bool EARLY_AD = NCH * CE <= 32;
     constexpr int GB = NCH < 8 ? NCH : 8;
     V v[NCH], d[NCH], ad[EARLY_AD ? NCH : 1];
+    if constexpr (SL) gn_sum_slabs<NCH, CE>(sp, s_be + Cg, s_be + 2 * Cg, base, b, g, Cg, tid, NT, total, cpr, cpr_magic, C, d);
 #pragma unroll
     for (int i = 0; i < NCH; ++i) {
         const int c = tid + i * NT;
         int cg;
         const size_t off = gn_slab_off<CE>(c < total ? c : 0, cpr, cpr_magic, C, &cg);
-        v[i] = *(const V*)(x + base + off); d[i] = *(const V*)(dy + base + off);
+        v[i] = *(const V*)(x + base + off);
+        if constexpr (!SL) d[i] = *(const V*)(dy + base + off);
         if (NCH > 8 && i % 8 == 7) hcp_sched_fence();
     }
     if constexpr (EARLY_AD) {
@@ -476,21 +557,38 @@
     return r;
 }
 
-#define HCP_GN_SLAB_SWITCH(KERNEL, ...)                                                                              \
+#define HCP_GN_SLAB_SWITCH(KERNEL, SL, ...)                                                                             \
     do {                                                                                                             \
         const int key_ = sl.nch * 8 + sl.ce;                                                                         \
         switch (key_) {                                                                                              \
-            case 1 * 8 + 4: HCP_LAUNCH((KERNEL<1, 4>), grid, blk, sm, stream, __VA_ARGS__); break;                   \
-            case 2 * 8 + 4: HCP_LAUNCH((KERNEL<2, 4>), grid, blk, sm, stream, __VA_ARGS__); break;                   \
-            case 4 * 8 + 4: HCP_LAUNCH((KERNEL<4, 4>), grid, blk, sm, stream, __VA_ARGS__); break;                   \
-            case 8 * 8 + 4: HCP_LAUNCH((KERNEL<8, 4>), grid, blk, sm, stream, __VA_ARGS__); break;                   \
-            case 16 * 8 + 4: HCP_LAUNCH((KERNEL<16, 4>), grid, blk, sm, stream, __VA_ARGS__); break;                 \
-            case 1 * 8 + 2: HCP_LAUNCH((KERNEL<1, 2>), grid, blk, sm, stream, __VA_ARGS__); break;                   \
-            case 2 * 8 + 2: HCP_LAUNCH((KERNEL<2, 2>), grid, blk, sm, stream, __VA_ARGS__); break;                   \
-            case 4 * 8 + 2: HCP_LAUNCH((KERNEL<4, 2>), grid, blk, sm, stream, __VA_ARGS__); break;                   \
-            case 8 * 8 + 2: HCP_LAUNCH((KERNEL<8, 2>), grid, blk, sm, stream, __VA_ARGS__); break;                   \
-            case 16 * 8 + 2: HCP_LAUNCH((KERNEL<16, 2>), grid, blk, sm, stream, __VA_ARGS__); break;                 \
-            default: HCP_LAUNCH((KERNEL<32, 2>), grid, blk, sm, stream, __VA_ARGS__); break;                         \
+            case 1 * 8 + 4: HCP_LAUNCH((KERNEL<1, 4, SL>), grid, blk, sm, stream, __VA_ARGS__); break;                   \
+            case 2 * 8 + 4: HCP_LAUNCH((KERNEL<2, 4, SL>), grid, blk, sm, stream, __VA_ARGS__); break;                   \
+            case 4 * 8 + 4: HCP_LAUNCH((KERNEL<4, 4, SL>), grid, blk, sm, stream, __VA_ARGS__); break;                   \
+            case 8 * 8 + 4: HCP_LAUNCH((KERNEL<8, 4, SL>), grid, blk, sm, stream, __VA_ARGS__); break;                   \
+            case 16 * 8 + 4: HCP_LAUNCH((KERNEL<16, 4, SL>), grid, blk, sm, stream, __VA_ARGS__); break;                 \
+            case 1 * 8 + 2: HCP_LAUNCH((KERNEL<1, 2, SL>), grid, blk, sm, stream, __VA_ARGS__); break;                   \
+            case 2 * 8 + 2: HCP_LAUNCH((KERNEL<2, 2, SL>), grid, blk, sm, stream, __VA_ARGS__); break;                   \
+            case 4 * 8 + 2: HCP_LAUNCH((KERNEL<4, 2, SL>), grid, blk, sm, stream, __VA_ARGS__); break;                   \
+            case 8 * 8 + 2: HCP_LAUNCH((KERNEL<8, 2, SL>), grid, blk, sm, stream, __VA_ARGS__); break;                   \
+            case 16 * 8 + 2: HCP_LAUNCH((KERNEL<16, 2, SL>), grid, blk, sm, stream, __VA_ARGS__); break;                 \
+            default: HCP_LAUNCH((KERNEL<32, 2, SL>), grid, blk, sm, stream, __VA_ARGS__); break;                         \
+        }                                                                                                            \
+    } while (0)
+
+constexpr int kGnSumMaxElems = 32;
+#define HCP_GN_SLABSUM_SWITCH(KERNEL, ...)                                                                           \
+    do {                                                                                                             \
+        const int key_ = sl.nch * 8 + sl.ce;                                                                         \
+        switch (key_) {                                                                                              \
+            case 1 * 8 + 4: HCP_LAUNCH((KERNEL<1, 4, true>), grid, blk, sm, stream, __VA_ARGS__); break;             \
+            case 2 * 8 + 4: HCP_LAUNCH((KERNEL<2, 4, true>), grid, blk, sm, stream, __VA_ARGS__); break;             \
+            case 4 * 8 + 4: HCP_LAUNCH((KERNEL<4, 4, true>), grid, blk, sm, stream, __VA_ARGS__); break;             \
+            case 8 * 8 + 4: HCP_LAUNCH((KERNEL<8, 4, true>), grid, blk, sm, stream, __VA_ARGS__); break;             \
+            case 1 * 8 + 2: HCP_LAUNCH((KERNEL<1, 2, true>), grid, blk, sm, stream, __VA_ARGS__); break;             \
+            case 2 * 8 + 2: HCP_LAUNCH((KERNEL<2, 2, true>), grid, blk, sm, stream, __VA_ARGS__); break;             \
+            case 4 * 8 + 2: HCP_LAUNCH((KERNEL<4, 2, true>), grid, blk, sm, stream, __VA_ARGS__); break;             \
+            case 8 * 8 + 2: HCP_LAUNCH((KERNEL<8, 2, true>), grid, blk, sm, stream, __VA_ARGS__); break;             \
+            default: return hcp_set_error("groupnorm (split-K sum): no kernel for %d chunks of %d channels per lane", sl.nch, sl.ce); \
         }                                                                                                            \
     } while (0)
 
@@ -692,7 +790,7 @@
         const hcp_bf16* xp = (const hcp_bf16*)x; hcp_bf16* yp = (hcp_bf16*)y;
         const dim3 grid(G, B), blk(sl.nt);
         const size_t sm = (32 + 2 * (size_t)(C / G)) * sizeof(float);
-        HCP_GN_SLAB_SWITCH(gn_slab_fwd, xp, gamma, beta, stats, yp, HW, C, G, sl.cpr, sl.magic, silu, eps);
+        HCP_GN_SLAB_SWITCH(gn_slab_fwd, false, xp, GNSlabSrc{}, gamma, beta, stats, yp, HW, C, G, sl.cpr, sl.magic, silu, eps);
         HCP_LAUNCH_CHECK("groupnorm_fwd (slab)");
     }
     GNGeom g = gn_geom(B, HW, C);
@@ -714,7 +812,7 @@
         const hcp_bf16 *xp = (const hcp_bf16*)x, *dp = (const hcp_bf16*)dy, *ap = (const hcp_bf16*)addend; hcp_bf16* op = (hcp_bf16*)dx;
         const dim3 grid(G, B), blk(sl.nt);
         const size_t sm = (32 + 2 * (size_t)(C / G)) * sizeof(float);
-        HCP_GN_SLAB_SWITCH(gn_slab_bwd, xp, dp, gamma, beta, stats, ap, op, HW, C, G, sl.cpr, sl.magic, silu);
+        HCP_GN_SLAB_SWITCH(gn_slab_bwd, false, xp, dp, GNSlabSrc{}, gamma, beta, stats, ap, op, HW, C, G, sl.cpr, sl.magic, silu);
         HCP_LAUNCH_CHECK("groupnorm_bwd (slab)");
     }
     GNGeom g = gn_geom(B, HW, C);
@@ -725,6 +823,48 @@
                (const hcp_bf16*)dy, gamma, beta, stats, (const float*)workspace, (const hcp_bf16*)addend, (hcp_bf16*)dx, HW, C, G,
                g.TX, g.R, g.rows_per_chunk, silu);
     HCP_LAUNCH_CHECK("groupnorm_bwd");
+}
+
+HCP_API int hcp_groupnorm_slab_path(int HW, int C, int G) {
+    if (HW <= 0 || C <= 0 || G <= 0 || C % 8 || C % G) return 0;
+    const GNSlab sl = gn_slab_geom(HW, C, G);
+    return sl.nch && sl.nch <= 8 && sl.nch * sl.ce <= kGnSumMaxElems && g_gn_slab ? 1 : 0;
+}
+
+static int gn_slabs_check(const char* who, const float* slabs, int nsplit, int B, int HW, int C, int G) {
+    if (int e = gn_check(B, HW, C, G)) return e;
+    HCP_REQUIRE(slabs && nsplit >= 2 && nsplit <= 64, "%s: needs the slabs of a split launch (nsplit=%d)", who, nsplit);
+    HCP_REQUIRE(hcp_groupnorm_slab_path(HW, C, G), "%s: HW=%d C=%d G=%d has no one-launch slab kernel (reduce first)", who, HW, C, G);
+    HCP_REQUIRE(((size_t)slabs & 15) == 0 && (size_t)nsplit * B * HW * C * sizeof(float) < ((size_t)1 << 31), "%s: slabs misaligned or too large", who);
+    return 0;
+}
+
+HCP_API int hcp_groupnorm_silu_fwd_slabs(const float* slabs, int nsplit, float alpha, const float* bias, const float* rowbias,
+                                         int rowbias_ld, void* h, const float* gamma, const float* beta, void* y, float* stats, int B,
+                                         int HW, int C, int G, float eps, int silu, hipStream_t stream) {
+    if (int e = gn_slabs_check("hcp_groupnorm_silu_fwd_slabs", slabs, nsplit, B, HW, C, G)) return e;
+    HCP_REQUIRE(h && gamma && beta && y && stats, "hcp_groupnorm_silu_fwd_slabs: null pointer");
+    const GNSlab sl = gn_slab_geom(HW, C, G);
+    const GNSlabSrc sp = {slabs, (size_t)B * HW * C, nsplit, alpha, bias, rowbias, rowbias_ld, (hcp_bf16*)h};
+    const hcp_bf16* xp = nullptr; hcp_bf16* yp = (hcp_bf16*)y;
+    const dim3 grid(G, B), blk(sl.nt);
+    const size_t sm = (32 + 4 * (size_t)(C / G)) * sizeof(float);
+    HCP_GN_SLABSUM_SWITCH(gn_slab_fwd, xp, sp, gamma, beta, stats, yp, HW, C, G, sl.cpr, sl.magic, silu, eps);
+    HCP_LAUNCH_CHECK("groupnorm_fwd (slab, split-K sum)");
+}
+
+HCP_API int hcp_groupnorm_silu_bwd_slabs(const void* x, const float* slabs, int nsplit, void* dy_out, const float* gamma,
+                                         const float* beta, const float* stats, const void* addend, void* dx, int B, int HW, int C,
+                                         int G, int silu, hipStream_t stream) {
+    if (int e = gn_slabs_check("hcp_groupnorm_silu_bwd_slabs", slabs, nsplit, B, HW, C, G)) return e;
+    HCP_REQUIRE(x && gamma && beta && stats && dx, "hcp_groupnorm_silu_bwd_slabs: null pointer");
+    const GNSlab sl = gn_slab_geom(HW, C, G);
+    const GNSlabSrc sp = {slabs, (size_t)B * HW * C, nsplit, 1.0f, nullptr, nullptr, 0, (hcp_bf16*)dy_out};
+    const hcp_bf16 *xp = (const hcp_bf16*)x, *dp = nullptr, *ap = (const hcp_bf16*)addend; hcp_bf16* op = (hcp_bf16*)dx;
+    const dim3 grid(G, B), blk(sl.nt);
+    const size_t sm = (32 + 4 * (size_t)(C / G)) * sizeof(float);
+    HCP_GN_SLABSUM_SWITCH(gn_slab_bwd, xp, dp, sp, gamma, beta, stats, ap, op, HW, C, G, sl.cpr, sl.magic, silu);
+    HCP_LAUNCH_CHECK("groupnorm_bwd (slab, split-K sum)");
 }
 
 HCP_API int hcp_layernorm_fwd(const void* x, const void* x_lo, const float* gamma, const float* beta, void* y, float* stats, int M, int C,
diff --git a/hcp_diffusion_amd/csrc/runtime.hip b/hcp_diffusion_amd/csrc/runtime.hip
--- a/hcp_diffusion_amd/csrc/runtime.hip
+++ b/hcp_diffusion_amd/csrc/runtime.hip
@@ -14,7 +14,7 @@
 
 HCP_API int hcp_is_emulated(void) { return HCP_IS_EMULATED; }
 
-HCP_API int hcp_abi_version(void) { return 4; }
+HCP_API int hcp_abi_version(void) { return 5; }
 
 namespace {
 HCP_KERNEL(256) atomics_selfcheck_kernel(float* line, float* bucket, int nb, int stride) {
diff --git a/hcp_diffusion_amd/kernels.py b/hcp_diffusion_amd/kernels.py
--- a/hcp_diffusion_amd/kernels.py
+++ b/hcp_diffusion_amd/kernels.py
@@ -194,7 +194,7 @@
 
 
 def conv3x3(x1, wp, cout, *, x2=None, stride=1, upsample=False, mode=0, out_hw=None, bias=None, rowbias=None,
-            residual=None, out_f32=False, a2=None, b2=None, pad=1, out=None):
+            residual=None, out_f32=False, a2=None, b2=None, pad=1, out=None, _defer=False):
     assert x1.dtype == BF16 and x1.dim() == 4 and x1.is_contiguous()
     B, Hs, Ws, C1 = x1.shape
     C2 = 0
@@ -228,6 +228,13 @@
         assert a2.dtype == BF16 and b2.dtype == BF16 and a2.is_contiguous() and b2.is_contiguous()
         assert a2.numel() == B * Ho * Wo * 32 and tuple(b2.shape) == (cout, 32)
     ws = _workspace(x1)
+    if _defer:
+        assert residual is None and not out_f32 and a2 is None
+        ns = ctypes.c_int(0)
+        _chk(lib().hcp_conv3x3_bf16_deferred(_p(x1), C1, _p(x2), C2, B, Hs, Ws, Ho, Wo, mode, stride, 1 if upsample else 0, pad, _p(wp),
+                                             cout, _p(out), _p(bias), _p(rowbias), rowbias.stride(0) if rowbias is not None else 0,
+                                             _p(ws), ws.numel(), _stream(x1), ctypes.byref(ns)), "hcp_conv3x3_bf16_deferred")
+        return out, ns.value
     _chk(lib().hcp_conv3x3_bf16(_p(x1), C1, _p(x2), C2, B, Hs, Ws, Ho, Wo, mode, stride, 1 if upsample else 0, pad, _p(wp),
                                 cout, _p(out), cout, _p(bias), _p(rowbias), rowbias.stride(0) if rowbias is not None else 0,
                                 _p(residual), cout, 1 if out_f32 else 0, _p(a2), _p(b2), _p(ws), ws.numel(), _stream(x1)),
@@ -353,6 +360,43 @@
     _chk(lib().hcp_groupnorm_silu_bwd(_p(x), _p(dy), _p(gamma), _p(beta), _p(stats), _p(addend), _p(dx), _p(ws), B, HW, C, groups,
                                       1 if silu else 0, _stream(x)), "hcp_groupnorm_silu_bwd")
     return dx
+
+
+def groupnorm_sums_slabs(hw, c, groups):
+    return bool(lib().hcp_groupnorm_slab_path(hw, c, groups))
+
+
+def conv3x3_groupnorm_fwd(x1, wp, cout, gamma, beta, groups, eps, silu, *, x2=None, bias=None, rowbias=None):
+    B, Hs, Ws = x1.shape[:3]
+    if not groupnorm_sums_slabs(Hs * Ws, cout, groups):
+        h = conv3x3(x1, wp, cout, x2=x2, bias=bias, rowbias=rowbias)
+        return (h,) + groupnorm_fwd(h, gamma, beta, groups, eps, silu)
+    h, ns = conv3x3(x1, wp, cout, x2=x2, bias=bias, rowbias=rowbias, _defer=True)
+    if ns == 1:
+        return (h,) + groupnorm_fwd(h, gamma, beta, groups, eps, silu)
+    y = torch.empty_like(h)
+    stats = torch.empty((B, groups, 2), dtype=torch.float32, device=h.device)
+    _chk(lib().hcp_groupnorm_silu_fwd_slabs(_p(_workspace(x1)), ns, 1.0, _p(bias), _p(rowbias), rowbias.stride(0) if rowbias is not None else 0,
+                                            _p(h), _p(gamma), _p(beta), _p(y), _p(stats), B, Hs * Ws, cout, groups, float(eps),
+                                            1 if silu else 0, _stream(h)), "hcp_groupnorm_silu_fwd_slabs")
+    return h, y, stats
+
+
+def conv3x3_dgrad_groupnorm_bwd(dy, wd, cin, x, gamma, beta, stats, groups, silu, *, addend=None, want_dh=False):
+    assert x.dtype == BF16 and x.is_contiguous() and x.shape[-1] == cin
+    assert addend is None or (addend.dtype == BF16 and addend.is_contiguous() and addend.numel() == x.numel())
+    B, H, W = x.shape[:3]
+    if not groupnorm_sums_slabs(H * W, cin, groups):
+        dh = conv3x3(dy, wd, cin, mode=1, out_hw=(H, W))
+        return groupnorm_bwd(x, dh, gamma, beta, stats, groups, silu, addend), (dh if want_dh else None)
+    dh, ns = conv3x3(dy, wd, cin, mode=1, out_hw=(H, W), _defer=True)
+    if ns == 1:
+        return groupnorm_bwd(x, dh, gamma, beta, stats, groups, silu, addend), (dh if want_dh else None)
+    dx = torch.empty_like(x)
+    _chk(lib().hcp_groupnorm_silu_bwd_slabs(_p(x), _p(_workspace(x)), ns, _p(dh) if want_dh else None, _p(gamma), _p(beta), _p(stats),
+                                            _p(addend), _p(dx), B, H * W, cin, groups, 1 if silu else 0, _stream(x)),
+         "hcp_groupnorm_silu_bwd_slabs")
+    return dx, (dh if want_dh else None)
 
 
 def groupnorm_affine_grad(x, dy, gamma, beta, stats, groups, silu, dgamma, dbeta):
diff --git a/hcp_diffusion_amd/ops.py b/hcp_diffusion_amd/ops.py
--- a/hcp_diffusion_amd/ops.py
+++ b/hcp_diffusion_amd/ops.py
@@ -440,6 +440,94 @@
     return _GroupNormForkFn.apply(x, gn, silu, *_norm_tr(gn))
 
 
+RESNET_CONSUMER_REDUCE = True
+
+
+class _ResnetInFn(torch.autograd.Function):
+    @staticmethod
+    def forward(ctx, x, rowbias, n1, c1, n2, *train):
+        g1, b1 = n1.f32_params()
+        g2, b2 = n2.f32_params()
+        pk = c1.packed()
+        h0, st1 = K.groupnorm_fwd(x, g1, b1, n1.num_groups, n1.eps, True)
+        h1, h2, st2 = K.conv3x3_groupnorm_fwd(h0, pk.w, pk.cout, g2, b2, n2.num_groups, n2.eps, True, bias=pk.bias, rowbias=rowbias)
+        ctx.n1, ctx.c1 = n1, c1
+        ctx.train_n1, ctx.train_w, ctx.train_b = train[0] is not None, train[2] is not None, train[3] is not None
+        ctx.save_for_backward(x, st1, h0 if ctx.train_w else None)
+        ctx.mark_non_differentiable(h2, st2)
+        return h1, h2, st2, x.view_as(x)
+
+    @staticmethod
+    def backward(ctx, dh1, _dh2, _dst2, dskip):
+        x, st1, h0 = ctx.saved_tensors
+        n1, c1 = ctx.n1, ctx.c1
+        dskip = dskip.contiguous() if dskip is not None else None
+        if dh1 is None:
+            return (dskip,) + (None,) * (4 + 4)
+        g1, b1 = n1.f32_params()
+        pk = c1.packed()
+        dh1 = dh1.contiguous()
+        dx = None
+        if ctx.needs_input_grad[0]:
+            dx, dh0 = K.conv3x3_dgrad_groupnorm_bwd(dh1, pk.wd, pk.cin, x, g1, b1, st1, n1.num_groups, True, addend=dskip, want_dh=ctx.train_n1)
+        elif ctx.train_n1:
+            dh0 = K.conv3x3(dh1, pk.wd, pk.cin, mode=1, out_hw=tuple(x.shape[1:3]))
+        if ctx.train_n1:
+            K.groupnorm_affine_grad(x, dh0, g1, b1, st1, n1.num_groups, True, grad_buffer(n1.weight), grad_buffer(n1.bias))
+        drb = None
+        dy2 = dh1.view(-1, dh1.shape[-1])
+        if ctx.needs_input_grad[1]:
+            drb = torch.zeros((dh1.shape[0], dh1.shape[-1]), dtype=torch.float32, device=dh1.device)
+            K.colsum(dy2, drb, dh1.shape[1] * dh1.shape[2])
+        if ctx.train_w:
+            K.wgrad_conv3x3(dh1, h0, grad_buffer(c1.weight, True))
+        if ctx.train_b:
+            K.colsum(dy2, grad_buffer(c1.bias))
+        return (dx, drb) + (None,) * (3 + 4)
+
+
+class _ResnetOutFn(torch.autograd.Function):
+    @staticmethod
+    def forward(ctx, h1, h2, st2, sc, n2, c2, *train):
+        pk = c2.packed()
+        ctx.n2, ctx.c2 = n2, c2
+        ctx.train_n2, ctx.train_w, ctx.train_b = train[0] is not None, train[2] is not None, train[3] is not None
+        ctx.save_for_backward(h1, st2, h2 if ctx.train_w else None)
+        return K.conv3x3(h2, pk.w, pk.cout, bias=pk.bias, residual=sc)
+
+    @staticmethod
+    def backward(ctx, dy):
+        h1, st2, h2 = ctx.saved_tensors
+        n2, c2 = ctx.n2, ctx.c2
+        g2, b2 = n2.f32_params()
+        pk = c2.packed()
+        dy = dy.contiguous()
+        dh1 = None
+        if ctx.needs_input_grad[0]:
+            dh1, dh2 = K.conv3x3_dgrad_groupnorm_bwd(dy, pk.wd, pk.cin, h1, g2, b2, st2, n2.num_groups, True, want_dh=ctx.train_n2)
+        elif ctx.train_n2:
+            dh2 = K.conv3x3(dy, pk.wd, pk.cin, mode=1, out_hw=tuple(h1.shape[1:3]))
+        if ctx.train_n2:
+            K.groupnorm_affine_grad(h1, dh2, g2, b2, st2, n2.num_groups, True, grad_buffer(n2.weight), grad_buffer(n2.bias))
+        if ctx.train_w:
+            K.wgrad_conv3x3(dy, h2, grad_buffer(c2.weight, True))
+        if ctx.train_b:
+            K.colsum(dy.view(-1, dy.shape[-1]), grad_buffer(c2.bias))
+        return (dh1, None, None, dy if ctx.needs_input_grad[3] else None) + (None,) * (2 + 4)
+
+
+def _params4(norm, conv):
+    return _norm_tr(norm) + (_tr(conv.weight), _tr(conv.bias))
+
+
+def resnet_in(x, rowbias, norm1, conv1, norm2):
+    return _ResnetInFn.apply(x, rowbias, norm1, conv1, norm2, *_params4(norm1, conv1))
+
+
+def resnet_out(h1, h2, stats2, sc, norm2, conv2):
+    return _ResnetOutFn.apply(h1, h2, stats2, sc, norm2, conv2, *_params4(norm2, conv2))
+
+
 class _LayerNormFn(torch.autograd.Function):
     @staticmethod
     def forward(ctx, x, ln, hw=None, hb=None):
diff --git a/hcp_diffusion_amd/unet.py b/hcp_diffusion_amd/unet.py
--- a/hcp_diffusion_amd/unet.py
+++ b/hcp_diffusion_amd/unet.py
@@ -100,6 +100,8 @@
     def forward(self, x, temb_act, skip=None, temb_bias=None):
         if skip is not None:
             x = ops.concat_channels(x, skip)
+        if ops.RESNET_CONSUMER_REDUCE and self._plain_main_branch(temb_act, temb_bias):
+            return self._forward_consumer_reduce(x, temb_act, temb_bias)
         h, x = self.norm1(x, silu=True, fork=True)
         if temb_bias is not None:
             tb = temb_bias
@@ -112,6 +114,23 @@
         h = self.norm2(h, silu=True)
         sc = self.conv_shortcut(x) if hasattr(self, "conv_shortcut") else x
         return self.conv2(h, residual=sc)
+
+    def _plain_main_branch(self, temb_act, temb_bias):
+        for m, cls in ((self.norm1, HipGroupNorm), (self.norm2, HipGroupNorm), (self.conv1, HipConv2d), (self.conv2, HipConv2d)):
+            if type(m) is not cls or m._forward_hooks or m._forward_pre_hooks or m._backward_hooks or m._backward_pre_hooks:
+                return False
+        if self.conv1.kernel_size != (3, 3) or self.conv2.kernel_size != (3, 3) or self.dropout.p != 0.0:
+            return False
+        if ops.current_wgrad().side:
+            return False
+        return temb_bias is not None or (isinstance(self.time_emb_proj, HipLinear) and not temb_act.requires_grad
+                                         and not self.time_emb_proj.weight.requires_grad)
+
+    def _forward_consumer_reduce(self, x, temb_act, temb_bias):
+        tb = temb_bias if temb_bias is not None else self.time_emb_proj(temb_act, out_f32=True)
+        h1, h2, st2, x = ops.resnet_in(x, tb, self.norm1, self.conv1, self.norm2)
+        sc = self.conv_shortcut(x) if hasattr(self, "conv_shortcut") else x
+        return ops.resnet_out(h1, h2, st2, sc, self.norm2, self.conv2)
 
 
 LOG2E = 1.4426950408889634
diff --git a/include/hcp_mi355x.h b/include/hcp_mi355x.h
--- a/include/hcp_mi355x.h
+++ b/include/hcp_mi355x.h
@@ -10,7 +10,7 @@
 
 const char* hcp_last_error(void);
 int hcp_is_emulated(void);
-#define HCP_ABI_VERSION 4
+#define HCP_ABI_VERSION 5
 int hcp_abi_version(void);
 int hcp_selfcheck_atomics(float* line, float* bucket, int nb, int stride, int workgroups, hcpStream_t stream);
 
@@ -29,6 +29,10 @@
                      int stride, int upsample, int pad, const void* Wp, int Cout, void* D, int ldd, const float* bias,
                      const float* rowbias, int rowbias_ld, const void* residual, int ldr, int out_f32, const void* A2,
                      const void* B2, void* workspace, size_t workspace_bytes, hcpStream_t stream);
+int hcp_conv3x3_bf16_deferred(const void* X1, int C1, const void* X2, int C2, int B, int Hs, int Ws, int Ho, int Wo, int mode,
+                              int stride, int upsample, int pad, const void* Wp, int Cout, void* D, const float* bias,
+                              const float* rowbias, int rowbias_ld, void* workspace, size_t workspace_bytes, hcpStream_t stream,
+                              int* nsplit);
 
 int hcp_attention_fwd(const void* Q, const void* K, const void* V, void* O, float* lse, int B, int H, int Nq, int Nk, int D,
                       long q_bs, int q_rs, long k_bs, int k_rs, long v_bs, int v_rs, long o_bs, int o_rs, float scale,
@@ -46,6 +50,13 @@
 int hcp_groupnorm_silu_bwd(const void* x, const void* dy, const float* gamma, const float* beta, const float* stats,
                            const void* addend , void* dx,
                            void* workspace, int B, int HW, int C, int G, int silu, hcpStream_t stream);
+int hcp_groupnorm_slab_path(int HW, int C, int G);
+int hcp_groupnorm_silu_fwd_slabs(const float* slabs, int nsplit, float alpha, const float* bias, const float* rowbias, int rowbias_ld,
+                                 void* h, const float* gamma, const float* beta, void* y, float* stats, int B, int HW, int C, int G,
+                                 float eps, int silu, hcpStream_t stream);
+int hcp_groupnorm_silu_bwd_slabs(const void* x, const float* slabs, int nsplit, void* dy_out, const float* gamma, const float* beta,
+                                 const float* stats, const void* addend, void* dx, int B, int HW, int C, int G, int silu,
+                                 hcpStream_t stream);
 
 int hcp_layernorm_fwd(const void* x, const void* x_lo, const float* gamma, const float* beta, void* y, float* stats, int M, int C,
                       float eps, hcpStream_t stream);
```

Measured after the change: 208.5 images/sec (median of 2 runs). No clear change (-0.7%).
